# meudnaes/VoronoiRT

Hardware: AMD Instinct MI355X
Metric: formal-solve cell-updates/sec (higher is better)
Workload: dtype f64

## Files before the change

include/voronoirt.h:

```cpp
#ifndef VORONOIRT_H
#define VORONOIRT_H

#include <stdint.h>

#ifdef __cplusplus
extern "C" {
#endif

#define VRT_OK 0
#define VRT_EINVAL (-1)
#define VRT_EGRID (-2)
#define VRT_ENODEVICE (-3)
#define VRT_ENOMEM (-4)
#define VRT_EIO (-5)

typedef struct vrt_grid vrt_grid;
typedef struct vrt_plan vrt_plan;

#define VRT_ALPHA_SITE 0
#define VRT_ALPHA_SITE_LAM 1
#define VRT_ALPHA_ANGLE_SITE_LAM 2
#define VRT_ALPHA_ANGLE_NATIVE 3
#define VRT_ALPHA_SITE_LAM_NATIVE 4

// ... 25 lines not shown
                       int n_sweeps, vrt_plan **out);
void vrt_plan_destroy(vrt_plan *p);
int64_t vrt_plan_num_levels(const vrt_plan *p);
int64_t vrt_plan_num_nodes(const vrt_plan *p);
int vrt_plan_get_upwind(const vrt_plan *p, int64_t angle, int64_t *up, double *dots, double *w,
                        double *r);

int vrt_plan_execute(vrt_plan *p, int64_t nlam, int64_t ld, const double *S, const double *alpha,
                     int alpha_mode, const double *I0_up, const double *I0_down,
                     const double *weights, double *J, double *I_out);
int vrt_plan_execute_dev(vrt_plan *p, int64_t nlam, int64_t ld, const double *dS,
                         const double *dalpha, int alpha_mode, const double *dI0_up,
                         const double *dI0_down, const double *weights_host, double *dJ,
                         double *dI_out, void *stream);
int vrt_grid_get_storage_order(const vrt_grid *g, int dir, int64_t *out);
int64_t vrt_plan_native_alpha_count(const vrt_plan *p, int64_t nlam);
int vrt_plan_native_pair_block(const vrt_plan *p);
int vrt_plan_native_pair_block_f32(const vrt_plan *p);
int vrt_plan_alpha_to_native_dev(vrt_plan *p, int64_t nlam, int64_t ld, const double *dalpha,
                                 double *dalpha_native, void *stream);
int vrt_plan_alpha_to_native_dev_f32(vrt_plan *p, int64_t nlam, int64_t ld, const float *dalpha,
                                     float *dalpha_native, void *stream);

int64_t vrt_plan_native_plane_count(const vrt_plan *p, int64_t nlam);
int vrt_plan_to_native_dev(vrt_plan *p, int64_t nlam, int64_t ld, const double *d_in, double *d_up, double *d_down,
                           void *stream);
int vrt_plan_from_native_dev(vrt_plan *p, int dir, int64_t nlam, int64_t ld, const double *d_native, double *d_out,
                             void *stream);
int vrt_plan_j_from_native_dev(vrt_plan *p, int64_t nlam, int64_t ld, const double *dJ_up, const double *dJ_down,
                               double *dJ, void *stream);
int vrt_plan_execute_native_dev(vrt_plan *p, int64_t nlam, const double *dS_up, const double *dS_down,
                                const double *dalpha, int alpha_mode, const double *dI0_up, const double *dI0_down,
                                const double *weights_host, double *dJ_up, double *dJ_down, void *stream);
int vrt_plan_to_native_dev_f32(vrt_plan *p, int64_t nlam, int64_t ld, const float *d_in, float *d_up, float *d_down,
                               void *stream);
int vrt_plan_from_native_dev_f32(vrt_plan *p, int dir, int64_t nlam, int64_t ld, const float *d_native, float *d_out,
                                 void *stream);
int vrt_plan_j_from_native_dev_f32(vrt_plan *p, int64_t nlam, int64_t ld, const float *dJ_up, const float *dJ_down,
                                   float *dJ, void *stream);
int vrt_plan_execute_native_dev_f32(vrt_plan *p, int64_t nlam, const float *dS_up, const float *dS_down,
                                    const float *dalpha, int alpha_mode, const float *dI0_up, const float *dI0_down,
                                    const double *weights_host, float *dJ_up, float *dJ_down, void *stream);

int vrt_lambda_update_native_dev(vrt_grid *g, int64_t nlam, const double *dJ_up, const double *dJ_down,
                                 const double *dB_up, const double *deps, double *dS_up, double *dS_down,
                                 double *max_rel_change, void *stream);
int vrt_rates_populations_native_dev(vrt_grid *g, int64_t nlam, const double *lambda, const int64_t blocks[6],
                                     const double *dJ_up, const double *dJ_down, const double *planck2,
                                     double lambda0, double c0, const double *d_doppler_width, const double *d_gamma,
                                     double sigma_bb_const, const double *sigma_bf1, const double *sigma_bf2,
                                     const double *d_temperature, const double *d_lte_populations, double hc_over_kB,
                                     double pref_ij, double pref_ji, const double *d_C, const double *d_atom_density,
                                     double *d_R, double *d_populations, void *stream);

int vrt_plan_execute_dev_f32(vrt_plan *p, int64_t nlam, int64_t ld, const float *dS,
                             const float *dalpha, int alpha_mode, const float *dI0_up,
                             const float *dI0_down, const double *weights_host, float *dJ,
                             float *dI_out, void *stream);
int vrt_plan_last_sweep_timing(const vrt_plan *p, double *ms, int64_t *launches);
int vrt_plan_check(vrt_plan *p);
int vrt_plan_last_path(const vrt_plan *p);
int vrt_plan_set_option(vrt_plan *p, const char *name, const char *value);
int vrt_grid_set_option(vrt_grid *g, const char *name, const char *value);

typedef struct vrt_schedule vrt_schedule;
int vrt_schedule_build(const vrt_grid *g, int dir, const int64_t *up, int n_sweeps, vrt_schedule **out);
int64_t vrt_schedule_num_nodes(const vrt_schedule *s);
int64_t vrt_schedule_num_levels(const vrt_schedule *s);
int vrt_schedule_get(const vrt_schedule *s, int64_t *site, int32_t *zflags, int64_t *level_off);
void vrt_schedule_destroy(vrt_schedule *s);
int vrt_layer_schedule(const vrt_grid *g, int dir, const int64_t *up, int n_sweeps, uint32_t *vis,
                       int32_t *nlev, int64_t *n_visits);
int vrt_layer_sorted_slots(const vrt_grid *g, int dir, const uint32_t *vis, int64_t *store, int64_t *self);

typedef struct vrt_patch_schedule vrt_patch_schedule;
int vrt_patch_schedule_build(const vrt_grid *g, int dir, const int64_t *up, int n_sweeps, int own_target,
                             int entry_cap, vrt_patch_schedule **out, int64_t counts[6]);
int vrt_patch_schedule_get(const vrt_patch_schedule *s, int32_t *layer_patch_off, int32_t *patch_own_lo,
                           int32_t *patch_own_cnt, int32_t *patch_nlev, int64_t *patch_ent_off,
                           int32_t *entry_pos, uint32_t *entry_vis, uint32_t *entry_loc);
int vrt_patch_schedule_get_deps(const vrt_patch_schedule *s, int64_t *dep_off, int32_t *dep_list);
int vrt_patch_schedule_get_layers(const vrt_patch_schedule *s, uint32_t *vis, int32_t *nlev, int64_t *n_visits);
void vrt_patch_schedule_destroy(vrt_patch_schedule *s);

int vrt_delaunay_up(vrt_grid *g, const double k[3], const double *S, const double *I0,
                    int64_t nI0, const double *alpha, int n_sweeps, double *I_out);
int vrt_delaunay_down(vrt_grid *g, const double k[3], const double *S, const double *I0,
                      int64_t nI0, const double *alpha, int n_sweeps, double *I_out);

#define VRT_METRIC_EUCLIDEAN   0
#define VRT_METRIC_PERIODIC_XY 1
#define VRT_RASTER_NEAREST     1
#define VRT_RASTER_INV_DIST2   2
int vrt_grid_nearest(vrt_grid *g, int64_t nq, const double *q_zxy, int metric, int k, int64_t *idx, double *dist);
int vrt_grid_to_raster_dev(vrt_grid *g, int64_t nz, int64_t nx, int64_t ny, const double *z, const double *x,
                           const double *y, int metric, int mode, int64_t nf, int64_t ld, const double *d_fields,
                           double *d_raster, void *stream);
int vrt_raster_to_grid_dev(vrt_grid *g, int64_t nz, int64_t nx, int64_t ny, const double *z, const double *x,
                           const double *y, int64_t nf, const double *d_raster, int64_t ld, double *d_fields,
                           void *stream);
int vrt_grid_to_raster(vrt_grid *g, int64_t nz, int64_t nx, int64_t ny, const double *z, const double *x,
                       const double *y, int metric, int mode, int64_t nf, int64_t ld, const double *fields,
                       double *raster);
int vrt_raster_to_grid(vrt_grid *g, int64_t nz, int64_t nx, int64_t ny, const double *z, const double *x,
                       const double *y, int64_t nf, const double *raster, int64_t ld, double *fields);
int vrt_grid_raster_stats(const vrt_grid *g, double *nearest_ms, double *gather_ms, int64_t *queries,
                          int64_t *walk_steps, int64_t *fallbacks);

int vrt_sample_sites(int device, int64_t nz, int64_t nx, int64_t ny, const double *z, const double *x, const double *y,
                     const double *quantity, int64_t n_sites, uint64_t seed, int64_t batch, int64_t max_proposals,
                     double *pos_zxy, int64_t *proposals_used);
int vrt_sample_sites_dev(int device, int64_t nz, int64_t nx, int64_t ny, const double *z, const double *x,
                         const double *y, const double *d_quantity, int64_t n_sites, uint64_t seed, int64_t batch,
                         int64_t max_proposals, double *d_pos_zxy, int64_t *proposals_used, void *stream);

int vrt_lambda_update_dev(vrt_grid *g, int64_t nlam, int64_t ld, const double *dJ, const double *dB,
                          const double *deps, const double *dS_old, double *dS_new,
                          double *max_rel_change, void *stream);

int vrt_line_opacity_dev(vrt_plan *p, int64_t nlam, const double *lambda, double lambda0, double c0,
                         const double *d_velocity, const double *d_doppler_width, const double *d_gamma,
                         const double *d_line_strength, const double *d_alpha_cont, double *d_alpha_native,
                         void *stream);
int vrt_line_opacity_dev_f32(vrt_plan *p, int64_t nlam, const double *lambda, double lambda0, double c0,
                             const double *d_velocity, const double *d_doppler_width, const double *d_gamma,
                             const double *d_line_strength, const double *d_alpha_cont, float *d_alpha_native,
                             void *stream);

int vrt_plan_execute_line(vrt_plan *p, int64_t nlam, int64_t ld, const double *lambda, double lambda0, double c0,
                          const double *velocity, const double *doppler_width, const double *gamma,
                          const double *line_strength, const double *alpha_cont, const double *S, const double *I0_up,
                          const double *I0_down, const double *weights, double *J);

int vrt_line_terms_dev(vrt_grid *g, const double *d_gamma_static, const double *d_gamma_unsold,
                       const double *d_populations, double strength_const, double Bij, double Bji, double *d_gamma,
                       double *d_line_strength, void *stream);

typedef struct vrt_lambda vrt_lambda;
typedef struct vrt_line_case {
    int64_t nlam;
    const double *lambda;
    int64_t blocks[6];
    double lambda0, c0;
    const double *velocity;
    const double *doppler_width;
    const double *gamma_static;
    const double *gamma_unsold;
    const double *alpha_cont;
    const double *eps;
    const double *temperature;
    const double *atom_density;
    const double *B0;
    const double *lte_populations;
    const double *C;
    const double *planck2;
    const double *sigma_bf1, *sigma_bf2;
    double strength_const, Bij, Bji;
    double sigma_bb_const, hc_over_kB, pref_ij, pref_ji;
} vrt_line_case;
int vrt_lambda_create(vrt_plan *p, const vrt_line_case *lc, const double *weights, vrt_lambda **out);
int vrt_lambda_iterate(vrt_lambda *s, double *max_rel_change);
int vrt_lambda_get(vrt_lambda *s, double *J, double *S, double *populations, double *R, double *gamma);
void vrt_lambda_destroy(vrt_lambda *s);

typedef struct vrt_multi vrt_multi;
int vrt_multi_create(int n_devices, const int *devices, int64_t n, const double *pos_zxy, const int64_t *nbr, int64_t D1,
// ... 134 lines not shown
```

voronoirt_amd/_lib.py:

```python
from __future__ import annotations

import ctypes
import os

HERE = os.path.dirname(os.path.abspath(__file__))
LIB_PATH = os.path.join(HERE, "libvrt_hip.so")
if os.environ.get("VRT_LIB_PATH"):
    LIB_PATH = os.environ["VRT_LIB_PATH"]

c_i64 = ctypes.c_int64
c_dbl = ctypes.c_double
p_i64 = ctypes.POINTER(ctypes.c_int64)
p_i32 = ctypes.POINTER(ctypes.c_int32)
p_dbl = ctypes.POINTER(ctypes.c_double)
p_int = ctypes.POINTER(ctypes.c_int)
vp = ctypes.c_void_p

VRT_OK, VRT_EINVAL, VRT_EGRID, VRT_ENODEVICE, VRT_ENOMEM, VRT_EIO = 0, -1, -2, -3, -4, -5
ALPHA_SITE, ALPHA_SITE_LAM, ALPHA_ANGLE_SITE_LAM, ALPHA_ANGLE_NATIVE, ALPHA_SITE_LAM_NATIVE = 0, 1, 2, 3, 4
METRIC_EUCLIDEAN, METRIC_PERIODIC_XY = 0, 1
RASTER_NEAREST, RASTER_INV_DIST2 = 1, 2

class LineCaseStruct(ctypes.Structure):
    _fields_ = [("nlam", c_i64), ("lambda_", p_dbl), ("blocks", c_i64 * 6), ("lambda0", c_dbl), ("c0", c_dbl),
# ... 24 lines not shown
    "vrt_grid_num_layer_offsets": (c_i64, [vp, ctypes.c_int]),
    "vrt_grid_get_layers": (ctypes.c_int, [vp, ctypes.c_int, p_i64]),
    "vrt_grid_get_perm": (ctypes.c_int, [vp, ctypes.c_int, p_i64]),
    "vrt_grid_get_delaunay_lines": (ctypes.c_int, [vp, p_dbl]),
    "vrt_direction": (None, [c_dbl, c_dbl, p_dbl]),
    "vrt_plan_create": (ctypes.c_int, [vp, c_i64, p_dbl, ctypes.c_int, ctypes.POINTER(vp)]),
    "vrt_plan_create_ex": (ctypes.c_int, [vp, c_i64, p_dbl, p_int, ctypes.c_int,
                                          ctypes.POINTER(vp)]),
    "vrt_plan_destroy": (None, [vp]),
    "vrt_plan_num_levels": (c_i64, [vp]),
    "vrt_plan_num_nodes": (c_i64, [vp]),
    "vrt_plan_get_upwind": (ctypes.c_int, [vp, c_i64, p_i64, p_dbl, p_dbl, p_dbl]),
    "vrt_plan_execute": (ctypes.c_int, [vp, c_i64, c_i64, p_dbl, p_dbl, ctypes.c_int, p_dbl, p_dbl,
                                        p_dbl, p_dbl, p_dbl]),
    "vrt_plan_execute_dev": (ctypes.c_int, [vp, c_i64, c_i64, vp, vp, ctypes.c_int, vp, vp, p_dbl,
                                            vp, vp, vp]),
    "vrt_plan_execute_dev_f32": (ctypes.c_int, [vp, c_i64, c_i64, vp, vp, ctypes.c_int, vp, vp, p_dbl,
                                                vp, vp, vp]),
    "vrt_plan_native_plane_count": (c_i64, [vp, c_i64]),
    "vrt_plan_to_native_dev": (ctypes.c_int, [vp, c_i64, c_i64, vp, vp, vp, vp]),
    "vrt_plan_from_native_dev": (ctypes.c_int, [vp, ctypes.c_int, c_i64, c_i64, vp, vp, vp]),
    "vrt_plan_j_from_native_dev": (ctypes.c_int, [vp, c_i64, c_i64, vp, vp, vp, vp]),
    "vrt_plan_execute_native_dev": (ctypes.c_int, [vp, c_i64, vp, vp, vp, ctypes.c_int, vp, vp, p_dbl, vp, vp, vp]),
    "vrt_plan_to_native_dev_f32": (ctypes.c_int, [vp, c_i64, c_i64, vp, vp, vp, vp]),
    "vrt_plan_from_native_dev_f32": (ctypes.c_int, [vp, ctypes.c_int, c_i64, c_i64, vp, vp, vp]),
    "vrt_plan_j_from_native_dev_f32": (ctypes.c_int, [vp, c_i64, c_i64, vp, vp, vp, vp]),
    "vrt_plan_execute_native_dev_f32": (ctypes.c_int, [vp, c_i64, vp, vp, vp, ctypes.c_int, vp, vp, p_dbl, vp, vp, vp]),
    "vrt_plan_check": (ctypes.c_int, [vp]),
    "vrt_lambda_update_native_dev": (ctypes.c_int, [vp, c_i64, vp, vp, vp, vp, vp, vp, p_dbl, vp]),
    "vrt_rates_populations_native_dev": (ctypes.c_int, [vp, c_i64, p_dbl, p_i64, vp, vp, p_dbl, c_dbl, c_dbl, vp, vp,
                                                        c_dbl, p_dbl, p_dbl, vp, vp, c_dbl, c_dbl, c_dbl, vp, vp, vp,
                                                        vp, vp]),
    "vrt_grid_get_storage_order": (ctypes.c_int, [vp, ctypes.c_int, p_i64]),
    "vrt_plan_native_alpha_count": (c_i64, [vp, c_i64]),
    "vrt_plan_native_pair_block": (ctypes.c_int, [vp]),
    "vrt_plan_native_pair_block_f32": (ctypes.c_int, [vp]),
    "vrt_plan_alpha_to_native_dev": (ctypes.c_int, [vp, c_i64, c_i64, vp, vp, vp]),
    "vrt_line_opacity_dev": (ctypes.c_int, [vp, c_i64, p_dbl, c_dbl, c_dbl, vp, vp, vp, vp, vp, vp, vp]),
    "vrt_line_opacity_dev_f32": (ctypes.c_int, [vp, c_i64, p_dbl, c_dbl, c_dbl, vp, vp, vp, vp, vp, vp, vp]),
    "vrt_plan_alpha_to_native_dev_f32": (ctypes.c_int, [vp, c_i64, c_i64, vp, vp, vp]),
    "vrt_plan_execute_line": (ctypes.c_int, [vp, c_i64, c_i64, p_dbl, c_dbl, c_dbl, p_dbl, p_dbl, p_dbl, p_dbl, p_dbl,
                                             p_dbl, p_dbl, p_dbl, p_dbl, p_dbl]),
    "vrt_line_terms_dev": (ctypes.c_int, [vp, vp, vp, vp, c_dbl, c_dbl, c_dbl, vp, vp, vp]),
    "vrt_lambda_create": (ctypes.c_int, [vp, ctypes.POINTER(LineCaseStruct), p_dbl, ctypes.POINTER(vp)]),
    "vrt_lambda_iterate": (ctypes.c_int, [vp, p_dbl]),
    "vrt_lambda_get": (ctypes.c_int, [vp, p_dbl, p_dbl, p_dbl, p_dbl, p_dbl]),
    "vrt_lambda_destroy": (None, [vp]),
    "vrt_multi_create": (ctypes.c_int, [ctypes.c_int, p_int, c_i64, p_dbl, p_i64, c_i64, p_dbl, c_i64, p_dbl, p_int,
                                        ctypes.c_int, ctypes.POINTER(vp)]),
    "vrt_multi_execute": (ctypes.c_int, [vp, c_i64, c_i64, p_dbl, p_dbl, ctypes.c_int, p_dbl, p_dbl, p_dbl, p_dbl]),
    "vrt_multi_set_shard": (ctypes.c_int, [vp, ctypes.c_char_p]),
    "vrt_multi_last_shard": (ctypes.c_int, [vp]),
    "vrt_multi_uses_rccl": (ctypes.c_int, [vp]),
    "vrt_multi_destroy": (None, [vp]),
    "vrt_multi_execute_line": (ctypes.c_int, [vp, c_i64, c_i64, p_dbl, c_dbl, c_dbl, p_dbl, p_dbl, p_dbl, p_dbl, p_dbl, p_dbl,
                                              p_dbl, p_dbl, p_dbl, p_dbl]),
    "vrt_multi_lambda_create": (ctypes.c_int, [vp, ctypes.POINTER(LineCaseStruct), p_dbl, ctypes.POINTER(vp)]),
    "vrt_multi_lambda_iterate": (ctypes.c_int, [vp, p_dbl]),
    "vrt_multi_lambda_get": (ctypes.c_int, [vp, p_dbl, p_dbl, p_dbl, p_dbl, p_dbl]),
    "vrt_multi_lambda_destroy": (None, [vp]),
    "vrt_rates_populations_dev": (ctypes.c_int, [vp, c_i64, c_i64, p_dbl, p_i64, vp, p_dbl, c_dbl, c_dbl, vp, vp,
                                                 c_dbl, p_dbl, p_dbl, vp, vp, c_dbl, c_dbl, c_dbl, vp, vp, vp,
                                                 vp, vp]),
    "vrt_plan_last_sweep_timing": (ctypes.c_int, [vp, p_dbl, p_i64]),
    "vrt_plan_last_path": (ctypes.c_int, [vp]),
    "vrt_plan_set_option": (ctypes.c_int, [vp, ctypes.c_char_p, ctypes.c_char_p]),
    "vrt_grid_set_option": (ctypes.c_int, [vp, ctypes.c_char_p, ctypes.c_char_p]),
    "vrt_schedule_build": (ctypes.c_int, [vp, ctypes.c_int, p_i64, ctypes.c_int,
                                          ctypes.POINTER(vp)]),
    "vrt_schedule_num_nodes": (c_i64, [vp]),
    "vrt_schedule_num_levels": (c_i64, [vp]),
    "vrt_schedule_get": (ctypes.c_int, [vp, p_i64, p_i32, p_i64]),
    "vrt_schedule_destroy": (None, [vp]),
    "vrt_layer_schedule": (ctypes.c_int, [vp, ctypes.c_int, p_i64, ctypes.c_int,
                                          ctypes.POINTER(ctypes.c_uint32), p_i32, p_i64]),
    "vrt_layer_sorted_slots": (ctypes.c_int, [vp, ctypes.c_int, ctypes.POINTER(ctypes.c_uint32), p_i64, p_i64]),
    "vrt_patch_schedule_build": (ctypes.c_int, [vp, ctypes.c_int, p_i64, ctypes.c_int, ctypes.c_int, ctypes.c_int,
                                                ctypes.POINTER(vp), p_i64]),
    "vrt_patch_schedule_get": (ctypes.c_int, [vp, p_i32, p_i32, p_i32, p_i32, p_i64, p_i32,
                                              ctypes.POINTER(ctypes.c_uint32), ctypes.POINTER(ctypes.c_uint32)]),
    "vrt_patch_schedule_get_deps": (ctypes.c_int, [vp, p_i64, p_i32]),
    "vrt_patch_schedule_get_layers": (ctypes.c_int, [vp, ctypes.POINTER(ctypes.c_uint32), p_i32, p_i64]),
    "vrt_patch_schedule_destroy": (None, [vp]),
    "vrt_lambda_update_dev": (ctypes.c_int, [vp, c_i64, c_i64, vp, vp, vp, vp, vp, p_dbl, vp]),
    "vrt_short_characteristics": (ctypes.c_int, [c_i64, c_i64, c_i64, p_dbl, p_dbl, p_dbl, c_i64, p_dbl,
                                                 p_int, p_dbl, c_i64, p_dbl, c_i64, p_dbl, ctypes.c_int,
                                                 ctypes.c_int, p_dbl]),
    "vrt_regular_create": (ctypes.c_int, [c_i64, c_i64, c_i64, p_dbl, p_dbl, p_dbl, ctypes.c_int,
                                          ctypes.POINTER(vp)]),
    "vrt_regular_destroy": (None, [vp]),
    "vrt_regular_execute_dev": (ctypes.c_int, [vp, c_i64, p_dbl, p_int, vp, c_i64, vp, c_i64, c_i64, vp,
                                               ctypes.c_int, vp, vp]),
    "vrt_regular_last_solve_ms": (ctypes.c_int, [vp, p_dbl]),
    "vrt_regular_execute_line": (ctypes.c_int, [vp, c_i64, p_dbl, p_int, p_dbl, c_i64, p_dbl, c_dbl, c_dbl, p_dbl, p_dbl,
                                                p_dbl, p_dbl, p_dbl, p_dbl, p_dbl, ctypes.c_int, p_dbl]),
    "vrt_regular_lambda_create": (ctypes.c_int, [vp, c_i64, p_dbl, p_int, p_dbl, ctypes.POINTER(LineCaseStruct), ctypes.c_int,
                                                 ctypes.POINTER(vp)]),
    "vrt_regular_lambda_iterate": (ctypes.c_int, [vp, p_dbl]),
    "vrt_regular_lambda_get": (ctypes.c_int, [vp, p_dbl, p_dbl, p_dbl, p_dbl, p_dbl]),
    "vrt_regular_lambda_destroy": (None, [vp]),
    "vrt_synth_opacity_dev": (ctypes.c_int, [c_i64, c_i64, c_i64, p_dbl, c_i64, p_dbl, p_dbl, c_dbl, c_dbl, c_dbl, c_dbl,
                                             c_dbl, c_dbl, c_dbl, c_dbl, vp, vp, vp, vp, vp, vp, vp, vp, vp, vp]),
    "vrt_synth_opacity": (ctypes.c_int, [ctypes.c_int, c_i64, c_i64, c_i64, p_dbl, c_i64, p_dbl, p_dbl, c_dbl, c_dbl,
                                         c_dbl, c_dbl, c_dbl, c_dbl, c_dbl, c_dbl, p_dbl, p_dbl, p_dbl, p_dbl, p_dbl,
                                         p_dbl, p_dbl, p_dbl, p_dbl]),
    "vrt_regular_emergent_dev": (ctypes.c_int, [vp, p_dbl, c_i64, vp, vp, ctypes.c_int, vp, vp]),
    "vrt_top_intensity": (ctypes.c_int, [c_i64, c_i64, c_i64, p_dbl, p_dbl, p_dbl, p_dbl, c_i64, p_dbl, p_dbl,
                                         ctypes.c_int, ctypes.c_int, p_dbl]),
    "vrt_tau_unity_dev": (ctypes.c_int, [c_i64, c_i64, c_i64, p_dbl, p_dbl, p_dbl, p_dbl, c_i64, vp, vp, vp]),
    "vrt_tau_unity": (ctypes.c_int, [c_i64, c_i64, c_i64, p_dbl, p_dbl, p_dbl, p_dbl, c_i64, p_dbl, ctypes.c_int,
                                     p_dbl]),
    "vrt_grid_nearest": (ctypes.c_int, [vp, c_i64, p_dbl, ctypes.c_int, ctypes.c_int, p_i64, p_dbl]),
    "vrt_grid_to_raster_dev": (ctypes.c_int, [vp, c_i64, c_i64, c_i64, p_dbl, p_dbl, p_dbl, ctypes.c_int, ctypes.c_int,
                                              c_i64, c_i64, vp, vp, vp]),
    "vrt_raster_to_grid_dev": (ctypes.c_int, [vp, c_i64, c_i64, c_i64, p_dbl, p_dbl, p_dbl, c_i64, vp, c_i64, vp, vp]),
    "vrt_grid_to_raster": (ctypes.c_int, [vp, c_i64, c_i64, c_i64, p_dbl, p_dbl, p_dbl, ctypes.c_int, ctypes.c_int,
                                          c_i64, c_i64, p_dbl, p_dbl]),
    "vrt_raster_to_grid": (ctypes.c_int, [vp, c_i64, c_i64, c_i64, p_dbl, p_dbl, p_dbl, c_i64, p_dbl, c_i64, p_dbl]),
    "vrt_grid_raster_stats": (ctypes.c_int, [vp, p_dbl, p_dbl, p_i64, p_i64, p_i64]),
    "vrt_sample_sites": (ctypes.c_int, [ctypes.c_int, c_i64, c_i64, c_i64, p_dbl, p_dbl, p_dbl, p_dbl, c_i64,
                                        ctypes.c_uint64, c_i64, c_i64, p_dbl, p_i64]),
    "vrt_sample_sites_dev": (ctypes.c_int, [ctypes.c_int, c_i64, c_i64, c_i64, p_dbl, p_dbl, p_dbl, vp, c_i64,
                                            ctypes.c_uint64, c_i64, c_i64, vp, p_i64, vp]),
    "vrt_ng_accelerate_dev": (ctypes.c_int, [c_i64, vp, vp, vp, vp, vp, p_dbl, p_dbl, p_int, vp]),
    "vrt_ng_sums_dev": (ctypes.c_int, [c_i64, vp, vp, vp, vp, p_dbl, vp]),
    "vrt_ng_coefficients": (ctypes.c_int, [p_dbl, p_dbl]),
    "vrt_ng_apply_dev": (ctypes.c_int, [c_i64, c_dbl, c_dbl, vp, vp, vp, vp, p_int, vp]),
    "vrt_lambda_set_acceleration": (ctypes.c_int, [vp, ctypes.c_int, ctypes.c_int, ctypes.c_int]),
    "vrt_regular_lambda_set_acceleration": (ctypes.c_int, [vp, ctypes.c_int, ctypes.c_int, ctypes.c_int]),
    "vrt_lambda_last_acceleration": (ctypes.c_int, [vp, p_int, p_dbl, p_dbl]),
    "vrt_regular_lambda_last_acceleration": (ctypes.c_int, [vp, p_int, p_dbl, p_dbl]),
    "vrt_continuum_case_check": (ctypes.c_int, [ctypes.POINTER(ContinuumCaseStruct), c_i64]),
    "vrt_continuum_create": (ctypes.c_int, [vp, ctypes.POINTER(ContinuumCaseStruct), p_dbl, ctypes.POINTER(vp)]),
    "vrt_continuum_iterate": (ctypes.c_int, [vp, p_dbl]),
    "vrt_continuum_get": (ctypes.c_int, [vp, p_dbl, p_dbl]),
    "vrt_continuum_set_source": (ctypes.c_int, [vp, p_dbl]),
    "vrt_continuum_set_acceleration": (ctypes.c_int, [vp, ctypes.c_int, ctypes.c_int, ctypes.c_int]),
    "vrt_continuum_last_acceleration": (ctypes.c_int, [vp, p_int, p_dbl, p_dbl]),
    "vrt_continuum_destroy": (None, [vp]),
    "vrt_regular_continuum_create": (ctypes.c_int, [vp, c_i64, p_dbl, p_int, p_dbl, ctypes.POINTER(ContinuumCaseStruct),
                                                    ctypes.c_int, ctypes.POINTER(vp)]),
    "vrt_regular_continuum_iterate": (ctypes.c_int, [vp, p_dbl]),
    "vrt_regular_continuum_get": (ctypes.c_int, [vp, p_dbl, p_dbl]),
    "vrt_regular_continuum_set_source": (ctypes.c_int, [vp, p_dbl]),
    "vrt_regular_continuum_set_acceleration": (ctypes.c_int, [vp, ctypes.c_int, ctypes.c_int, ctypes.c_int]),
    "vrt_regular_continuum_last_acceleration": (ctypes.c_int, [vp, p_int, p_dbl, p_dbl]),
    "vrt_regular_continuum_destroy": (None, [vp]),
    "vrt_continuum_update_dev": (ctypes.c_int, [vp, c_i64, c_i64, vp, vp, vp, c_dbl, vp, vp, p_dbl, p_i64, vp]),
    "vrt_plan_lambda_diagonal_dev": (ctypes.c_int, [vp, c_i64, c_i64, vp, p_dbl, vp, vp]),
    "vrt_plan_lambda_diagonal": (ctypes.c_int, [vp, c_i64, c_i64, p_dbl, p_dbl, p_dbl]),
    "vrt_continuum_ali_update_dev": (ctypes.c_int, [vp, c_i64, c_i64, vp, vp, vp, vp, c_dbl, vp, vp, p_dbl, p_i64, vp]),
    "vrt_continuum_set_operator": (ctypes.c_int, [vp, ctypes.c_int]),
    "vrt_continuum_get_operator": (ctypes.c_int, [vp, p_int, p_dbl]),
    "vrt_delaunay_up": (ctypes.c_int, [vp, p_dbl, p_dbl, p_dbl, c_i64, p_dbl, ctypes.c_int, p_dbl]),
    "vrt_delaunay_down": (ctypes.c_int, [vp, p_dbl, p_dbl, p_dbl, c_i64, p_dbl, ctypes.c_int, p_dbl]),
}


class VrtError(RuntimeError):
    def __init__(self, code: int, message: str):
        super().__init__(f"libvrt_hip error {code}: {message}")
        self.code = code
        self.message = message


_lib = None
# ... 33 lines not shown
```

voronoirt_amd/csrc/vrt_api.cpp:

```cpp
#include <algorithm>
#include <atomic>
#include <chrono>
#include <cmath>
#include <cstdio>
#include <cstdlib>
#include <cstring>
#include <memory>
#include <new>
#include <thread>

#include "vrt_internal.h"

namespace vrt {

static thread_local std::string g_err;

void set_error(const std::string &msg) { g_err = msg; }
int fail(int code, const std::string &msg)
{
    g_err = msg;
    return code;
}

void tuning_from_env(Tuning &t)
{
    static const char *names[] = {"VRT_PATH", "VRT_STEP_K", "VRT_STEP_SINGLE", "VRT_STEP_PAIRS", "VRT_STEP_XCD",
                                  "VRT_STEP_STREAMS", "VRT_STEP_LEVEL_MAP", "VRT_STEP_GROUP_DIR", "VRT_TILE_WIDE",
                                  "VRT_TILE_PRE", "VRT_PATCH_K", "VRT_PATCH_NT", "VRT_PATCH_OWN",
                                  "VRT_PATCH_Q", "VRT_PATCH_TARGET", "VRT_PATCH_SPLIT", "VRT_PAIR_BLOCK", "VRT_PATCH_QUAD", "VRT_PATCH_LEAN", "VRT_PATCH_CHAIN", "VRT_CHAIN_PAIRS", "VRT_CHAIN_SPIN", "VRT_CHAIN_DATAFLAG", "VRT_CHAIN_STATIC", "VRT_LAMBDA_NATIVE", "VRT_DEBUG_FLAGS", "VRT_DEBUG_SKIP_LEVELS",
                                  "VRT_TILE_DEBUG"};
    for (const char *nm : names) {
        const char *e = std::getenv(nm);
        if (e && *e && tuning_set(t, nm, e, false) != VRT_OK) {
            static std::mutex mu;
            static std::vector<std::string> said;
            std::lock_guard<std::mutex> lock(mu);
            if (std::find(said.begin(), said.end(), std::string(nm)) == said.end()) {
                said.push_back(nm);
                std::fprintf(stderr, "[libvrt_hip] ignoring %s=%s: %s\n", nm, e, g_err.c_str());
            }
        }
    }
}

int tuning_set(Tuning &t, const char *name, const char *value, bool created)
{
    if (!name || !value) return fail(VRT_EINVAL, "NULL option name or value");
    const std::string nm(name), v(value);
    if (nm == "VRT_PATH") {
        static const char *paths[] = {"auto", "levels", "tiles", "steps", "patches"};
        for (int i = 0; i < 5; i++)
            if (v == paths[i]) { t.path = i; return VRT_OK; }
        if (v.empty()) { t.path = 0; return VRT_OK; }
        return fail(VRT_EINVAL, "VRT_PATH must be auto, levels, tiles, steps or patches");
    }
    char *end = nullptr;
    const long x = std::strtol(value, &end, 10);
    if (end == value || *end != 0) return fail(VRT_EINVAL, "option " + nm + " needs an integer value");
    struct { const char *name; int *field; long lo, hi; bool creation_only; } tab[] = {
        {"VRT_STEP_K", &t.step_K, 0, 18, false}, {"VRT_STEP_SINGLE", &t.step_single, 0, 1, false},
        {"VRT_STEP_PAIRS", &t.step_pairs, 0, 64, false}, {"VRT_STEP_XCD", &t.step_xcd, 0, 2, false},
        {"VRT_STEP_STREAMS", &t.step_streams, 1, 4, false}, {"VRT_STEP_LEVEL_MAP", &t.step_level_map, 0, 1, false},
        {"VRT_STEP_GROUP_DIR", &t.step_group_dir, 0, 1, false}, {"VRT_TILE_WIDE", &t.tile_wide, 0, 1, false},
        {"VRT_TILE_PRE", &t.tile_pre, 0, 1, false},
        {"VRT_PATCH_K", &t.patch_K, 1, 8, true}, {"VRT_PATCH_NT", &t.patch_NT, 64, 1024, true},
        {"VRT_PATCH_OWN", &t.patch_own, 0, 65535, true}, {"VRT_PATCH_Q", &t.patch_Q, 1, 4, false},
        {"VRT_PATCH_TARGET", &t.patch_target, 0, 1 << 20, false}, {"VRT_PATCH_SPLIT", &t.patch_split, 0, 4096, false}, {"VRT_PAIR_BLOCK", &t.pair_block, 1, 16, true},
        {"VRT_PATCH_QUAD", &t.patch_quad, 0, 1, true}, {"VRT_PATCH_LEAN", &t.patch_lean, 0, 1, false},
        {"VRT_PATCH_CHAIN", &t.patch_chain, 0, 2, false}, {"VRT_CHAIN_PAIRS", &t.chain_pairs, 1, 256, false},
        {"VRT_CHAIN_SPIN", &t.chain_spin, 1, 1 << 20, false}, {"VRT_CHAIN_DATAFLAG", &t.chain_dataflag, 0, 2, false},
        {"VRT_LAMBDA_NATIVE", &t.lambda_native, 0, 1, false}, {"VRT_CHAIN_STATIC", &t.chain_static, 0, 1, false}, {"VRT_DEBUG_FLAGS", &t.debug_flags, 0, 1 << 20, false},
        {"VRT_DEBUG_SKIP_LEVELS", &t.debug_skip_levels, 0, 1, false}, {"VRT_TILE_DEBUG", &t.tile_debug, 0, 1, false},
    };
    for (auto &o : tab)
        if (nm == o.name) {
            if (o.creation_only && created)
                return fail(VRT_EINVAL, "option " + nm + " shapes what plan creation builds: preset it in the environment");
            if (x < o.lo || x > o.hi) return fail(VRT_EINVAL, "option " + nm + " out of range");
            *o.field = (int)x;
            return VRT_OK;
        }
    return fail(VRT_EINVAL, "unknown option " + nm);
}

int use_device(int device)
{
    if (device < 0)
        return fail(VRT_ENODEVICE, "host-only grid handle (device < 0): no compute without a HIP device");
    int cnt = 0;
    hipError_t e = hipGetDeviceCount(&cnt);
    if (e != hipSuccess || cnt <= 0)
        return fail(VRT_ENODEVICE, "no HIP device available (libvrt_hip has no CPU fallback)");
    if (device < 0 || device >= cnt) return fail(VRT_EINVAL, "device ordinal out of range");
    VRT_HIP_TRY(hipSetDevice(device));
    (void)hipGetLastError();
    return VRT_OK;
}

int use_current_device()
{
    int cnt = 0;
    if (hipGetDeviceCount(&cnt) != hipSuccess || cnt <= 0)
        return fail(VRT_ENODEVICE, "no HIP device available (libvrt_hip has no CPU fallback)");
    (void)hipGetLastError();
    return VRT_OK;
}

static void free_grid(vrt_grid *g)
{
    if (!g) return;
    for (PlanCacheEntry *c : g->cache) {
        vrt_plan_destroy(c->plan);
        delete c;
    }
    g->cache.clear();
    raster_locator_free(g);
    dev_free(g->d_pos);
    dev_free(g->d_rowptr);
    dev_free(g->d_col);
    dev_free(g->d_lz);
    dev_free(g->d_lx);
    dev_free(g->d_ly);
    dev_free(g->up.d_order);
    dev_free(g->down.d_order);
    dev_free(g->up.d_rank);
    dev_free(g->down.d_rank);
    dev_free(g->up.d_lay);
    dev_free(g->down.d_lay);
    dev_free(g->d_scalars);
    dev_free(g->d_small);
    if (g->small_ev) (void)hipEventDestroy(g->small_ev);
    if (g->small_copy_ev) (void)hipEventDestroy(g->small_copy_ev);
    if (g->h_small) (void)hipHostFree(g->h_small);
    dev_free(g->up.d_store);
    dev_free(g->down.d_store);
    dev_free(g->up.d_srank);
    dev_free(g->down.d_srank);
    if (g->stream) (void)hipStreamDestroy(g->stream);
    delete g;
}

static int upload_grid(vrt_grid *g)
{
    const int64_t n = g->n;
    const size_t nnz = g->col.size();
    int rc;
    if ((rc = dev_alloc(&g->d_pos, (size_t)3 * n))) return rc;
    if ((rc = dev_alloc(&g->d_rowptr, (size_t)n + 1))) return rc;
    if ((rc = dev_alloc(&g->d_col, nnz))) return rc;
    if ((rc = dev_alloc(&g->d_lz, nnz))) return rc;
// ... 9 lines not shown
        std::vector<int32_t> order((size_t)n);
        for (int64_t i = 0; i < n; i++) order[(size_t)i] = (int32_t)(dir.perm[(size_t)i] - 1);
        if ((rc = dev_alloc(&dir.d_order, (size_t)n))) return rc;
        VRT_HIP_TRY(hipMemcpy(dir.d_order, order.data(), sizeof(int32_t) * n, hipMemcpyHostToDevice));
        std::vector<int32_t> rank((size_t)n);
        for (int64_t i = 0; i < n; i++) rank[(size_t)order[(size_t)i]] = (int32_t)i;
        if ((rc = dev_alloc(&dir.d_rank, (size_t)n))) return rc;
        VRT_HIP_TRY(hipMemcpy(dir.d_rank, rank.data(), sizeof(int32_t) * n, hipMemcpyHostToDevice));
        std::vector<int32_t> srank((size_t)n);
        for (int64_t i = 0; i < n; i++) srank[(size_t)dir.store[(size_t)i]] = (int32_t)i;
        if ((rc = dev_alloc(&dir.d_store, (size_t)n))) return rc;
        if ((rc = dev_alloc(&dir.d_srank, (size_t)n))) return rc;
        VRT_HIP_TRY(hipMemcpy(dir.d_store, dir.store.data(), sizeof(int32_t) * n, hipMemcpyHostToDevice));
        VRT_HIP_TRY(hipMemcpy(dir.d_srank, srank.data(), sizeof(int32_t) * n, hipMemcpyHostToDevice));
        std::vector<int32_t> lay(dir.reduced.size());
        for (size_t j = 0; j < lay.size(); j++) lay[j] = (int32_t)(dir.reduced[j] - 1);
        if ((rc = dev_alloc(&dir.d_lay, lay.size()))) return rc;
        VRT_HIP_TRY(hipMemcpy(dir.d_lay, lay.data(), sizeof(int32_t) * lay.size(), hipMemcpyHostToDevice));
    }
    if ((rc = launch_delaunay_lines(g))) return rc;
    VRT_HIP_TRY(hipStreamSynchronize(g->stream));
    return VRT_OK;
}

static int grid_create_impl(int64_t n, const double *pos, const int64_t *nbr, int64_t D1,
                            const double bounds[6], int device, vrt_grid **out)
{
    if (!out) return fail(VRT_EINVAL, "out is NULL");
    *out = nullptr;
    if (!pos || !nbr || !bounds) return fail(VRT_EINVAL, "NULL argument");
    int rc = device >= 0 ? use_device(device) : VRT_OK;
    if (rc) return rc;
    vrt_grid *g = new (std::nothrow) vrt_grid();
    if (!g) return fail(VRT_ENOMEM, "out of host memory");
    g->device = device;
    rc = build_grid_host(g, n, pos, nbr, D1, bounds);
    if (!rc && device >= 0) rc = upload_grid(g);
    if (rc) {
        free_grid(g);
        return rc;
    }
    *out = g;
    return VRT_OK;
}

static const Direction &direction_of(const vrt_grid *g, int dir) { return dir > 0 ? g->up : g->down; }

static void free_plan(vrt_plan *p)
{
    if (!p) return;
    dev_free(p->d_up1);
    dev_free(p->d_up2);
    dev_free(p->d_d1);
    dev_free(p->d_d2);
    dev_free(p->d_w1);
    dev_free(p->d_w2);
    dev_free(p->d_r1);
    dev_free(p->d_r2);
    dev_free(p->d_node_site);
    dev_free(p->d_node_meta);
    dev_free(p->d_node_u1);
    dev_free(p->d_node_u2);
    dev_free(p->d_angles_up);
    dev_free(p->d_angles_down);
    dev_free(p->d_I);
    for (int i = 0; i < 6; i++) dev_free(p->d_stage[i]);
    dev_free(p->t_u1); dev_free(p->t_u2);
    dev_free(p->t_w1); dev_free(p->t_w2); dev_free(p->t_r1); dev_free(p->t_r2);
    dev_free(p->t_vis);
    dev_free(p->t_loc);
    dev_free(p->t_self);
    dev_free(p->t_vis_s);
    dev_free(p->t_loc_s);
    dev_free(p->t_gpos);
    dev_free(p->t_rank_s);
    dev_free(p->t_loc_ss);
    dev_free(p->t_code_ss);
    dev_free(p->d_nlev); dev_free(p->d_angle_dir); dev_free(p->d_task_map);
    for (int d = 0; d < 2; d++) { dev_free(p->ws_S[d]); dev_free(p->ws_A[d]); dev_free(p->ws_J[d]); }
    dev_free(p->ws_AA);
    for (int i = 0; i < 2; i++) dev_free(p->ws_cg[i]);
    dev_free(p->d_step_angles);
    dev_free(p->d_level_map);
    dev_free(p->d_patch_work);
    dev_free(p->d_chain_items); dev_free(p->d_chain_deps); dev_free(p->d_chain_progress); dev_free(p->d_chain_ctrl);
    for (auto &cs : p->chain_cache) { dev_free(cs.items); dev_free(cs.deps); }
    p->chain_cache.clear();
    if (p->h_chain_status) { (void)hipHostFree(p->h_chain_status); p->h_chain_status = nullptr; }
    if (p->d_chain_dev) { (void)hipFree(p->d_chain_dev); p->d_chain_dev = nullptr; }
    if (p->h_chain_dev_pinned) { (void)hipHostFree(p->h_chain_dev_pinned); p->h_chain_dev_pinned = nullptr; }
    if (p->chain_dev_ev) (void)hipEventDestroy(p->chain_dev_ev);
    dev_free(p->e_pos); dev_free(p->e_u1); dev_free(p->e_u2); dev_free(p->e_vis); dev_free(p->e_loc);
    dev_free(p->e_w1); dev_free(p->e_w2); dev_free(p->e_r1); dev_free(p->e_r2);
    if (p->step_fork) (void)hipEventDestroy(p->step_fork);
    for (int i = 0; i < 4; i++) {
        if (p->step_join[i]) (void)hipEventDestroy(p->step_join[i]);
        if (p->step_stream[i]) (void)hipStreamDestroy(p->step_stream[i]);
    }
    for (CopyLane &l : p->copy_lanes) {
        for (int b = 0; b < 2; b++) {
            if (l.pin[b]) (void)hipHostFree(l.pin[b]);
            if (l.ev[b]) (void)hipEventDestroy(l.ev[b]);
        }
        if (l.st) (void)hipStreamDestroy(l.st);
    }
    if (p->copy_done) (void)hipEventDestroy(p->copy_done);
    if (p->ev0) (void)hipEventDestroy(p->ev0);
    if (p->ev1) (void)hipEventDestroy(p->ev1);
    delete p;
}

static int ensure_level_schedule(vrt_plan *p)
{
    if (p->level_ready) return VRT_OK;
    vrt_grid *g = p->g;
    const int64_t n = g->n;
    const int A = p->A;
    const int n_sweeps = p->n_sweeps;
    std::vector<AngleSchedule> sched((size_t)A);
    {
        unsigned hw = std::thread::hardware_concurrency();
        int nthr = (int)std::min<unsigned>(hw ? hw : 4, 16);
        nthr = std::max(1, std::min(nthr, std::max(A, 1)));
        if (!run_workers(nthr, [&](int t) {
                for (int a = t; a < A; a += nthr) {
                    const bool up = p->dir_of_active[(size_t)a] > 0;
                    build_angle_schedule(up ? g->up : g->down, up, n, n_sweeps,
                                         p->h_up1.data() + (size_t)a * n, p->h_up2.data() + (size_t)a * n,
                                         sched[(size_t)a]);
                }
            }))
            return fail(VRT_ENOMEM, "out of host memory while building the level schedule");
    }
    int64_t max_levels = 0, total = 0;
    for (int a = 0; a < A; a++) {
        if (sched[(size_t)a].bad_site >= 0) return fail(VRT_EGRID, "site without an upwind neighbour");
        max_levels = std::max<int64_t>(max_levels, (int64_t)sched[(size_t)a].level_off.size() - 1);
        total += (int64_t)sched[(size_t)a].site.size();
    }
    std::vector<int32_t> srank_up((size_t)n);
    for (int64_t i = 0; i < n; i++) srank_up[(size_t)g->up.store[(size_t)i]] = (int32_t)i;
    std::vector<uint32_t> node_site((size_t)total), node_meta((size_t)total);
    std::vector<int32_t> node_u1((size_t)total), node_u2((size_t)total);
    p->level_off.assign((size_t)max_levels + 1, 0);
    int64_t at = 0;
    for (int64_t t = 0; t < max_levels; t++) {
        p->level_off[(size_t)t] = at;
        for (int a = 0; a < A; a++) {
            const AngleSchedule &s = sched[(size_t)a];
            if (t + 1 >= (int64_t)s.level_off.size()) continue;
            const int64_t x0 = s.level_off[(size_t)t], x1 = s.level_off[(size_t)t + 1];
            std::vector<std::pair<int32_t, int64_t>> keyed((size_t)(x1 - x0));
            for (int64_t x = x0; x < x1; x++)
                keyed[(size_t)(x - x0)] = {srank_up[(size_t)s.site[(size_t)x]], x};
            std::sort(keyed.begin(), keyed.end());
            for (const auto &kv : keyed) {
                const int64_t x = kv.second;
                node_site[(size_t)at] = s.site[(size_t)x];
                node_meta[(size_t)at] = (uint32_t)a | ((uint32_t)s.zflags[(size_t)x] << 8);
                node_u1[(size_t)at] = p->h_up1[(size_t)a * (size_t)n + s.site[(size_t)x]];
                node_u2[(size_t)at] = p->h_up2[(size_t)a * (size_t)n + s.site[(size_t)x]];
                at++;
            }
        }
    }
    p->level_off[(size_t)max_levels] = at;
    p->n_nodes = total;
// ... 773 lines not shown
        return VRT_OK;
    });
}

struct vrt_patch_schedule {
    vrt::PatchSchedule s;
    vrt::LayerSchedule layers;
};

int vrt_patch_schedule_build(const vrt_grid *g, int dir, const int64_t *up, int n_sweeps, int own_target,
                             int entry_cap, vrt_patch_schedule **out, int64_t counts[6])
{
    if (!g || !up || !out || !counts) return fail(VRT_EINVAL, "NULL argument");
    if (n_sweeps < 1 || own_target < 1 || entry_cap < 1 || entry_cap > 65535)
        return fail(VRT_EINVAL, "need n_sweeps >= 1, own_target >= 1 and 1 <= entry_cap <= 65535");
    *out = nullptr;
    return guarded([&] {
        const int64_t n = g->n;
        std::vector<int32_t> u1((size_t)n), u2((size_t)n);
        for (int64_t i = 0; i < n; i++) {
            const int64_t a = up[2 * i], b = up[2 * i + 1];
            if (a > n || b > n) return fail(VRT_EINVAL, "upwind id out of range");
            u1[(size_t)i] = a >= 1 ? (int32_t)(a - 1) : kNoUpwind;
            u2[(size_t)i] = b >= 1 ? (int32_t)(b - 1) : kNoUpwind;
        }
        std::unique_ptr<vrt_patch_schedule> ps(new vrt_patch_schedule());
        int threads = (int)std::max(1u, std::min(8u, std::thread::hardware_concurrency()));
        if (const char *e = std::getenv("VRT_HOST_THREADS")) threads = std::max(1, std::min(64, std::atoi(e)));
        build_patch_schedule(direction_of(g, dir), dir > 0, n, n_sweeps, u1.data(), u2.data(), own_target, entry_cap,
                             ps->s, threads, &ps->layers);
        if (ps->s.bad_site >= 0)
            return fail(VRT_EGRID, "site " + std::to_string(ps->s.bad_site + 1) + " has no upwind neighbour");
        if (!ps->s.ok) return fail(VRT_EINVAL, "schedule does not fit the packed patch encoding");
        counts[0] = (int64_t)ps->s.patch_own_lo.size();
        counts[1] = (int64_t)ps->s.entry_pos.size();
        counts[2] = ps->s.n_visits;
        counts[3] = ps->s.n_live;
        counts[4] = ps->s.max_entries;
        counts[5] = (int64_t)ps->s.layer_patch_off.size();
        *out = ps.release();
        return VRT_OK;
    });
}

int vrt_patch_schedule_get(const vrt_patch_schedule *s, int32_t *layer_patch_off, int32_t *patch_own_lo,
                           int32_t *patch_own_cnt, int32_t *patch_nlev, int64_t *patch_ent_off,
                           int32_t *entry_pos, uint32_t *entry_vis, uint32_t *entry_loc)
{
    if (!s) return fail(VRT_EINVAL, "NULL schedule");
    const PatchSchedule &p = s->s;
    if (layer_patch_off) std::copy(p.layer_patch_off.begin(), p.layer_patch_off.end(), layer_patch_off);
    if (patch_own_lo) std::copy(p.patch_own_lo.begin(), p.patch_own_lo.end(), patch_own_lo);
    if (patch_own_cnt) std::copy(p.patch_own_cnt.begin(), p.patch_own_cnt.end(), patch_own_cnt);
    if (patch_nlev) std::copy(p.patch_nlev.begin(), p.patch_nlev.end(), patch_nlev);
    if (patch_ent_off) std::copy(p.patch_ent_off.begin(), p.patch_ent_off.end(), patch_ent_off);
    if (entry_pos) std::copy(p.entry_pos.begin(), p.entry_pos.end(), entry_pos);
    if (entry_vis) std::copy(p.entry_vis.begin(), p.entry_vis.end(), entry_vis);
    if (entry_loc) std::copy(p.entry_loc.begin(), p.entry_loc.end(), entry_loc);
    return VRT_OK;
}

int vrt_patch_schedule_get_deps(const vrt_patch_schedule *s, int64_t *dep_off, int32_t *dep_list)
{
    if (!s) return fail(VRT_EINVAL, "NULL schedule");
    const PatchSchedule &p = s->s;
    if (dep_off) std::copy(p.dep_off.begin(), p.dep_off.end(), dep_off);
    if (dep_list) std::copy(p.dep_list.begin(), p.dep_list.end(), dep_list);
    return VRT_OK;
}

int vrt_patch_schedule_get_layers(const vrt_patch_schedule *s, uint32_t *vis, int32_t *nlev, int64_t *n_visits)
{
    if (!s) return fail(VRT_EINVAL, "NULL schedule");
    const LayerSchedule &ls = s->layers;
    if (!ls.ok) return fail(VRT_EINVAL, "schedule does not fit the packed layer-tile encoding");
    if (vis) std::copy(ls.vis.begin(), ls.vis.end(), vis);
    if (nlev) std::copy(ls.nlev.begin(), ls.nlev.end(), nlev);
    if (n_visits) *n_visits = ls.n_visits;
    return VRT_OK;
}

void vrt_patch_schedule_destroy(vrt_patch_schedule *s) { delete s; }

int vrt_grid_get_storage_order(const vrt_grid *g, int dir, int64_t *out)
{
    if (!g || !out) return fail(VRT_EINVAL, "NULL argument");
    const Direction &d = direction_of(g, dir);
    for (int64_t i = 0; i < g->n; i++) out[i] = (int64_t)d.store[(size_t)i] + 1;
    return VRT_OK;
}

int vrt_plan_native_pair_block(const vrt_plan *p) { return p ? 1 << native_lg(p, false) : 0; }
int vrt_plan_native_pair_block_f32(const vrt_plan *p) { return p ? 1 << native_lg(p, true) : 0; }

int64_t vrt_plan_native_alpha_count(const vrt_plan *p, int64_t nlam)
{
    if (!p || nlam < 1) return 0;
    return (int64_t)p->A * ((nlam + 1) / 2 * 2) * p->g->n;
}

static int alpha_native_call(vrt_plan *p, int64_t nlam, int64_t ld, const void *dalpha, void *dalpha_native, void *stream,
                             bool f32)
{
    return guarded([&] {
        if (!p || !dalpha || !dalpha_native) return fail(VRT_EINVAL, "NULL argument");
        if (nlam < 1 || ld < nlam) return fail(VRT_EINVAL, "need nlam >= 1 and ld >= nlam");
        if (p->A != (int)p->n_angles_user)
            return fail(VRT_EINVAL, "per-angle alpha needs every angle active (no θ = 90 direction)");
        std::lock_guard<std::mutex> lock(p->mu);
        int rc = use_device(p->g->device);
        return rc ? rc : alpha_to_native(p, nlam, ld, dalpha, dalpha_native, (hipStream_t)stream, f32);
    });
}

int vrt_plan_alpha_to_native_dev(vrt_plan *p, int64_t nlam, int64_t ld, const double *dalpha,
                                 double *dalpha_native, void *stream)
{
    return alpha_native_call(p, nlam, ld, dalpha, dalpha_native, stream, false);
}

int vrt_plan_alpha_to_native_dev_f32(vrt_plan *p, int64_t nlam, int64_t ld, const float *dalpha, float *dalpha_native,
                                     void *stream)
{
    return alpha_native_call(p, nlam, ld, dalpha, dalpha_native, stream, true);
}

int vrt_plan_execute_dev(vrt_plan *p, int64_t nlam, int64_t ld, const double *dS,
                         const double *dalpha, int alpha_mode, const double *dI0_up,
                         const double *dI0_down, const double *weights_host, double *dJ,
                         double *dI_out, void *stream)
{
    return execute_call(p, caller_args(nlam, ld, dS, dalpha, alpha_mode, dI0_up, dI0_down, weights_host, dJ, dI_out,
                                       (hipStream_t)stream, false));
}

int64_t vrt_plan_native_plane_count(const vrt_plan *p, int64_t nlam)
{
    if (!p || nlam < 1) return 0;
    return ((nlam + 1) / 2 * 2) * p->g->n;
}

int vrt_plan_to_native_dev(vrt_plan *p, int64_t nlam, int64_t ld, const double *d_in, double *d_up, double *d_down, void *stream)
{
    return native_call(p, nlam, ld, d_in && (d_up || d_down), false,
                       [&] { return planes_to_native(p, nlam, ld, d_in, d_up, d_down, (hipStream_t)stream); });
}

int vrt_plan_from_native_dev(vrt_plan *p, int dir, int64_t nlam, int64_t ld, const double *d_native, double *d_out, void *stream)
{
    return native_call(p, nlam, ld, d_native && d_out, false,
                       [&] { return plane_from_native(p, dir > 0 ? 0 : 1, nlam, ld, d_native, d_out, (hipStream_t)stream); });
}

int vrt_plan_j_from_native_dev(vrt_plan *p, int64_t nlam, int64_t ld, const double *dJ_up, const double *dJ_down, double *dJ,
                               void *stream)
{
    return native_call(p, nlam, ld, dJ && (dJ_up || dJ_down), false,
                       [&] { return J_from_native(p, nlam, ld, dJ_up, dJ_down, dJ, (hipStream_t)stream); });
}

int vrt_plan_execute_native_dev(vrt_plan *p, int64_t nlam, const double *dS_up, const double *dS_down, const double *dalpha,
                                int alpha_mode, const double *dI0_up, const double *dI0_down, const double *weights_host,
                                double *dJ_up, double *dJ_down, void *stream)
{
    return execute_call(p, native_args(nlam, dS_up, dS_down, dalpha, alpha_mode, dI0_up, dI0_down, weights_host, dJ_up,
                                       dJ_down, (hipStream_t)stream, false));
// ... 384 lines not shown
```

voronoirt_amd/csrc/vrt_internal.h:

```cpp
#pragma once

#include <hip/hip_runtime.h>

#include <algorithm>
#include <cstdint>
#include <mutex>
#include <new>
#include <string>
#include <thread>
#include <vector>

#include "voronoirt.h"

namespace vrt {

void set_error(const std::string &msg);
int fail(int code, const std::string &msg);

#define VRT_HIP_TRY(expr)                                                                  \
    do {                                                                                   \
        hipError_t _e = (expr);                                                            \
        if (_e != hipSuccess)                                                              \
            return ::vrt::fail(VRT_ENODEVICE, std::string(#expr) + ": " + hipGetErrorString(_e)); \
    } while (0)
// ... 65 lines not shown
    ~DevBuf() { dev_free(p); }
    int alloc(size_t count) { dev_free(p); return dev_alloc(&p, count); }
    operator T *() const { return p; }
};

template <typename Body>
inline bool run_workers(int count, Body body)
{
    std::vector<char> threw((size_t)std::max(count, 1), 0);
    auto guarded = [&](int t) {
        try {
            body(t);
        } catch (...) {
            threw[(size_t)t] = 1;
        }
    };
    std::vector<std::thread> pool;
    try {
        pool.reserve((size_t)std::max(count, 1));
    } catch (...) {
    }
    for (int t = 0; t < count; t++) {
        try {
            pool.emplace_back(guarded, t);
        } catch (...) {
            guarded(t);
        }
    }
    for (auto &th : pool) th.join();
    for (int t = 0; t < count; t++)
        if (threw[(size_t)t]) return false;
    return true;
}

constexpr int kMaxAngles = 64;
constexpr int64_t kMaxGuess = 70;
constexpr int32_t kNoUpwind = -1;

struct Direction {
    std::vector<int32_t> layer_of;
    std::vector<int64_t> perm;
    std::vector<int64_t> reduced;
    int64_t n1 = 0;
    int32_t *d_order = nullptr;
    int32_t *d_rank = nullptr;
    int32_t *d_lay = nullptr;
    std::vector<int32_t> store;
    int32_t *d_store = nullptr;
    int32_t *d_srank = nullptr;
};

struct PlanCacheEntry;

struct CopyLane {
    hipStream_t st = nullptr;
    void *pin[2] = {nullptr, nullptr};
    hipEvent_t ev[2] = {nullptr, nullptr};
};
constexpr size_t kCopyChunk = (size_t)8 << 20;

struct Tuning {
    int path = 0;
    int step_K = 0;
    int step_single = 0;
    int step_pairs = 0;
    int step_xcd = 2;
    int step_streams = 2;
    int step_level_map = 1;
    int step_group_dir = 1;
    int tile_wide = 1;
    int tile_pre = 1;
    int patch_K = 1, patch_NT = 512;
    int patch_own = 0;
    int patch_Q = 1;
    int pair_block = 1;
    int patch_quad = 1;
    int patch_lean = 1;
    int patch_chain = 2;
    int chain_pairs = 9;
    int chain_spin = 2048;
    int chain_dataflag = 2;
    int patch_split = 0;
    int patch_target = 0;
    int chain_static = 1;
    int lambda_native = 1;
    int debug_flags = 0, debug_skip_levels = 0, tile_debug = 0;
};
void tuning_from_env(Tuning &t);
int tuning_set(Tuning &t, const char *name, const char *value, bool created);

struct ExecArgs {
    int64_t nlam = 0, ld = 0;
    const void *S = nullptr;
    const void *S_nat[2] = {nullptr, nullptr};
    const void *alpha = nullptr;
    int alpha_mode = 0;
    const void *I0[2] = {nullptr, nullptr};
    const double *weights = nullptr;
    void *J = nullptr;
    void *J_nat[2] = {nullptr, nullptr};
    void *I_out = nullptr;
    bool native = false;
    bool f32 = false;
    hipStream_t st = nullptr;
    bool wants_J() const { return native ? J_nat[0] != nullptr : J != nullptr; }
};
inline ExecArgs caller_args(int64_t nlam, int64_t ld, const void *S, const void *alpha, int alpha_mode, const void *I0_up,
                            const void *I0_down, const double *weights, void *J, void *I_out, hipStream_t st, bool f32)
{
    ExecArgs x;
    x.nlam = nlam; x.ld = ld;
    x.S = S;
    x.alpha = alpha; x.alpha_mode = alpha_mode;
    x.I0[0] = I0_up; x.I0[1] = I0_down;
    x.weights = weights;
    x.J = J; x.I_out = I_out;
    x.f32 = f32;
    x.st = st;
    return x;
}
inline ExecArgs native_args(int64_t nlam, const void *S_up, const void *S_down, const void *alpha, int alpha_mode,
                            const void *I0_up, const void *I0_down, const double *weights, void *J_up, void *J_down,
                            hipStream_t st, bool f32)
{
    ExecArgs x = caller_args(nlam, (nlam + 1) / 2 * 2, nullptr, alpha, alpha_mode, I0_up, I0_down, weights, nullptr, nullptr,
                             st, f32);
    x.S_nat[0] = S_up; x.S_nat[1] = S_down;
    x.J_nat[0] = J_up; x.J_nat[1] = J_down;
    x.native = true;
    return x;
}

}

namespace vrt {
struct RasterLocator;
void raster_locator_free(vrt_grid *g);
}

struct vrt_grid {
    int device = 0;
    int64_t n = 0;
    int64_t D = 0;
    double bounds[6] = {0, 0, 0, 0, 0, 0};
    std::vector<double> pos;
    std::vector<int32_t> rowptr;
    std::vector<int32_t> col;
    vrt::Direction up, down;
    double *d_pos = nullptr;
    int32_t *d_rowptr = nullptr;
    int32_t *d_col = nullptr;
    double *d_lz = nullptr, *d_lx = nullptr, *d_ly = nullptr;
    hipStream_t stream = nullptr;
    unsigned long long *d_scalars = nullptr;
    double *d_small = nullptr;
    size_t small_cap = 0;
    double *h_small = nullptr;
    hipEvent_t small_ev = nullptr;
    bool small_ev_valid = false;
    hipEvent_t small_copy_ev = nullptr;
    bool small_copy_valid = false;
    std::vector<std::pair<std::string, std::string>> options;
    std::mutex mu;
    std::vector<vrt::PlanCacheEntry *> cache;
    vrt::RasterLocator *locator = nullptr;
    int64_t nearest_cells = 0;
};

struct vrt_plan {
    vrt_grid *g = nullptr;
    vrt::Tuning tune;
    int n_sweeps = 3;
    int64_t n_angles_user = 0;
    int A = 0;
    std::vector<int> user_of_active;
    std::vector<int> dir_of_active;
    std::vector<double> k;
    int32_t *d_up1 = nullptr, *d_up2 = nullptr;
    double *d_d1 = nullptr, *d_d2 = nullptr;
    double *d_w1 = nullptr, *d_w2 = nullptr;
    double *d_r1 = nullptr, *d_r2 = nullptr;
    uint32_t *d_node_site = nullptr;
    uint32_t *d_node_meta = nullptr;
    int32_t *d_node_u1 = nullptr, *d_node_u2 = nullptr;
    std::vector<int64_t> level_off;
    bool level_ready = false;
    std::vector<int32_t> h_up1, h_up2;
    int64_t n_nodes = 0;
    int32_t *d_angles_up = nullptr, *d_angles_down = nullptr;
    int n_up = 0, n_down = 0;
    std::vector<int64_t> skip_site;
    double *d_I = nullptr;
    size_t I_cap = 0;
    int64_t I_ld = 0;
    double *d_stage[6] = {nullptr, nullptr, nullptr, nullptr, nullptr, nullptr};
    size_t stage_cap[6] = {0, 0, 0, 0, 0, 0};
    bool tile_ok = false;
    bool step_tables_ready = false;
    int tile_K = 8;
    int tile_max_layers = 0;
    int64_t tile_max_layer_size = 0;
    int64_t tile_visits = 0;
    int32_t *t_u1 = nullptr, *t_u2 = nullptr;
    double *t_w1 = nullptr, *t_w2 = nullptr, *t_r1 = nullptr, *t_r2 = nullptr;
    uint32_t *t_vis = nullptr, *t_loc = nullptr;
    int32_t *t_self = nullptr;
    uint32_t *t_vis_s = nullptr, *t_loc_s = nullptr;
    uint32_t *t_gpos = nullptr;
    int32_t *t_rank_s = nullptr;
    uint32_t *t_loc_ss = nullptr;
    uint32_t *t_code_ss = nullptr;
    int32_t *d_nlev = nullptr, *d_angle_dir = nullptr;
    std::vector<int64_t> angle_visits;
    std::vector<int32_t> h_task_map;
    int32_t *d_task_map = nullptr;
    size_t task_map_cap = 0;
    int task_map_nlam = -1;
    double *ws_S[2] = {nullptr, nullptr}, *ws_A[2] = {nullptr, nullptr}, *ws_J[2] = {nullptr, nullptr};
    size_t ws_S_cap[2] = {0, 0}, ws_A_cap[2] = {0, 0}, ws_J_cap[2] = {0, 0};
    double *ws_AA = nullptr;
    size_t ws_AA_cap = 0;
    double *ws_cg[2] = {nullptr, nullptr};
    size_t ws_cg_cap[2] = {0, 0};
    int step_groups = 0;
    int32_t *d_step_angles = nullptr;
    std::vector<int> step_group_off;
    std::vector<double> angle_mean_levels;
    int32_t *d_level_map = nullptr;
    std::vector<int> level_map_off;
    int level_map_units = 0, level_map_groups = 0;
    std::vector<int32_t> h_step_angles;
    bool patch_ok = false;
    int lg_pair_block = 0;
    int patch_cap = 0, patch_K = 0, patch_NT = 0;
    int64_t n_patches = 0, n_patch_entries = 0, n_patch_visits = 0;
    std::vector<int32_t> h_patch_first;
    std::vector<int4> h_patch_rec;
    int32_t *e_pos = nullptr, *e_u1 = nullptr, *e_u2 = nullptr;
    uint32_t *e_vis = nullptr, *e_loc = nullptr;
    double *e_w1 = nullptr, *e_w2 = nullptr, *e_r1 = nullptr, *e_r2 = nullptr;
    std::vector<int2> h_patch_rec2;
    std::vector<int64_t> h_patch_dep_off;
    std::vector<int32_t> h_patch_deps;
    int4 *d_chain_items = nullptr;
    int32_t *d_chain_deps = nullptr;
    uint32_t *d_chain_progress = nullptr, *d_chain_ctrl = nullptr;
    uint32_t *h_chain_status = nullptr, *d_chain_status = nullptr;
    void *d_chain_dev = nullptr, *h_chain_dev_pinned = nullptr;
    std::vector<char> h_chain_dev;
    hipEvent_t chain_dev_ev = nullptr;
    bool chain_dev_ev_valid = false;
    size_t chain_progress_cap = 0;
    bool chain_progress_fresh = false;
    int chain_q_off[9] = {0, 0, 0, 0, 0, 0, 0, 0, 0};
    int chain_npair = -1, chain_lgB = -1, chain_nsplit = -1, chain_reduce = -1;
    int64_t chain_items = 0;
    struct ChainSet {
        int npair = -1, lgB = -1, nsplit = -1, reduce = -1;
        int4 *items = nullptr;
        int32_t *deps = nullptr;
        int q_off[9] = {0, 0, 0, 0, 0, 0, 0, 0, 0};
        int64_t n_items = 0;
    };
    std::vector<ChainSet> chain_cache;
    uint32_t chain_epoch = 0;
    int4 *d_patch_work = nullptr;
    std::vector<int64_t> patch_work_off;
    int patch_work_groups = 0;
    hipStream_t step_stream[4] = {nullptr, nullptr, nullptr, nullptr};
    hipEvent_t step_fork = nullptr, step_join[4] = {nullptr, nullptr, nullptr, nullptr};
    int last_path = 0;
    hipEvent_t ev0 = nullptr, ev1 = nullptr;
    bool ev_valid = false;
    std::vector<vrt::CopyLane> copy_lanes;
    hipEvent_t copy_done = nullptr;
    int64_t last_launches = 0;
    std::mutex mu;
};

namespace vrt {

struct PlanCacheEntry {
    double k[3];
    int n_sweeps;
    vrt_plan *plan;
    int users;
};

int parse_neighbour_file(const char *path, int64_t n, std::vector<int64_t> &matrix, int64_t &D1);
int build_grid_host(vrt_grid *g, int64_t n, const double *pos, const int64_t *nbr, int64_t D1,
                    const double bounds[6]);

int tessellate_host(int64_t n, const double *pos, const double bounds[6], int64_t D1, int64_t *nbr_out,
                    int64_t *max_count, int nthreads);

struct AngleSchedule {
    std::vector<uint32_t> site;
    std::vector<uint8_t> zflags;
    std::vector<int64_t> level_off;
    int64_t bad_site = -1;
};
void build_angle_schedule(const Direction &dir, bool ascending, int64_t n, int n_sweeps,
                          const int32_t *up1, const int32_t *up2, AngleSchedule &out);
struct LayerSchedule {
    std::vector<uint32_t> vis;
    std::vector<int32_t> nlev;
    int64_t n_visits = 0;
    int64_t max_layer_size = 0;
    int64_t bad_site = -1;
    bool ok = false;
};
void build_layer_schedule(const Direction &dir, bool ascending, int64_t n, int n_sweeps,
                          const int32_t *up1, const int32_t *up2, LayerSchedule &out);
void build_sorted_slots(const Direction &dir, int64_t n, const std::vector<uint32_t> &vis_site,
                        std::vector<int32_t> &self);
struct PatchSchedule {
    std::vector<int32_t> layer_patch_off;
    std::vector<int32_t> patch_own_lo;
    std::vector<int32_t> patch_own_cnt;
    std::vector<int32_t> patch_nlev;
    std::vector<int64_t> patch_ent_off;
    std::vector<int32_t> entry_pos;
    std::vector<uint32_t> entry_vis;
    std::vector<uint32_t> entry_loc;
    std::vector<int64_t> dep_off;
    std::vector<int32_t> dep_list;
    int64_t n_visits = 0;
    int64_t n_live = 0;
    int64_t max_entries = 0;
    int64_t bad_site = -1;
    bool ok = false;
};
void build_patch_schedule(const Direction &dir, bool ascending, int64_t n, int n_sweeps, const int32_t *up1,
                          const int32_t *up2, int own_target, int entry_cap, PatchSchedule &out, int threads = 1,
                          LayerSchedule *layers = nullptr);

int launch_delaunay_lines(vrt_grid *g);
int launch_upwind_table(vrt_plan *p, int a);
struct SweepArgs {
    int64_t n, nlam, ldS, ldA, ldI;
    const void *S, *alpha;
    int alpha_mode;
    void *I;
    bool f32 = false;
};
int launch_boundary(vrt_plan *p, const SweepArgs &sa, const void *dI0_up, const void *dI0_down,
                    hipStream_t st);
int launch_sweep_levels(vrt_plan *p, const SweepArgs &sa, hipStream_t st, int64_t *launches);
int launch_reduce_J(vrt_plan *p, const SweepArgs &sa, const double *weights_active, void *dJ,
                    int64_t ldJ, hipStream_t st);
int launch_copy_I_out(vrt_plan *p, const SweepArgs &sa, void *dI_out, int64_t ldO, hipStream_t st);

constexpr size_t kUpdateWords = 3;
int launch_axpy(size_t count, const double *d_src, double *d_dst, hipStream_t st);
int launch_gather_rows(int64_t rows, int64_t nlam, int64_t ld, const int32_t *d_order, const double *d_src, double *d_dst,
                       hipStream_t st);
int launch_lambda_update(int64_t n, int64_t nlam, int64_t ld, const double *dJ, const double *dB,
                         const double *deps, const double *dS_old, double *dS_new,
                         unsigned long long *d_result, hipStream_t st);
int launch_lambda_update_native(vrt_grid *g, int64_t nlam, const double *dJ_up, const double *dJ_down, const double *dB_up,
                                const double *deps, double *dS_up, double *dS_down, unsigned long long *d_result, hipStream_t st);

int launch_line_opacity(vrt_plan *p, int64_t nlam, const double *d_lambda, double lambda0, double c0,
                        const double *d_velocity, const double *d_doppler, const double *d_gamma,
                        const double *d_strength, const double *d_alpha_cont, void *d_out, hipStream_t st,
                        bool f32_out = false);
int launch_line_terms(int64_t n, const double *d_gamma_static, const double *d_gamma_unsold, const double *d_pops,
                      double strength_const, double Bij, double Bji, double *d_gamma, double *d_strength, hipStream_t st);
int launch_rates_populations(vrt_grid *g, int64_t nlam, int64_t ld, const int64_t blocks[6],
                             const double *d_small, const double *dJ, double lambda0, double c0,
                             const double *d_doppler, const double *d_gamma, double sigma_bb_const,
                             const double *d_temperature, const double *d_lte, double hc_over_kB,
                             double pref_ij, double pref_ji, const double *d_C, const double *d_atom_density,
                             double *d_R, double *d_populations, hipStream_t st,
                             const double *dJ_up = nullptr, const double *dJ_down = nullptr);
int launch_rates_populations(int64_t n, int64_t nlam, int64_t ld, const int64_t blocks[6], const double *d_small,
                             const double *dJ, double lambda0, double c0, const double *d_doppler, const double *d_gamma,
                             double sigma_bb_const, const double *d_temperature, const double *d_lte, double hc_over_kB,
                             double pref_ij, double pref_ji, const double *d_C, const double *d_atom_density, double *d_R,
                             double *d_populations, hipStream_t st);

int launch_rates_partial(vrt_grid *g, int64_t nlam, int64_t l0, int64_t l1, int64_t ld, const int64_t blocks[6],
                         const double *d_small, const double *dJ, double lambda0, double c0, const double *d_doppler,
                         const double *d_gamma, double sigma_bb_const, const double *d_temperature, const double *d_lte,
                         double hc_over_kB, double pref_ij, double pref_ji, double *d_shares, hipStream_t st,
                         const double *dJ_up = nullptr, const double *dJ_down = nullptr);
int launch_populations_from_shares(vrt_grid *g, const double *d_shares, const double *d_C, const double *d_atom_density,
                                   double *d_R, double *d_populations, hipStream_t st);

int execute_locked(vrt_plan *p, const ExecArgs &x);

int ensure_step_tables(vrt_plan *p);
int launch_permute_table(vrt_plan *p, int a, const uint32_t *d_vis_site);
int launch_sorted_tables(vrt_plan *p, int a);
int launch_gpos(vrt_plan *p, int a);
inline int native_lg(const vrt_plan *p, bool f32)
{
    if (!p->patch_ok) return 0;
    return f32 && p->tune.patch_quad != 0 && p->patch_K == 1 ? std::max(p->lg_pair_block, 1) : p->lg_pair_block;
}
int alpha_to_native(vrt_plan *p, int64_t nlam, int64_t ld, const void *dalpha, void *out, hipStream_t st, bool f32);
int native_planes_ok(const vrt_plan *p, bool f32 = false);
int planes_to_native_f32(vrt_plan *p, int64_t nlam, int64_t ld, const float *din, float *out_up, float *out_down, hipStream_t st);
int plane_from_native_f32(vrt_plan *p, int dir_index, int64_t nlam, int64_t ld, const float *din, float *dout, hipStream_t st);
int J_from_native_f32(vrt_plan *p, int64_t nlam, int64_t ld, const float *dJ_up, const float *dJ_down, float *dJ, hipStream_t st);
int planes_to_native(vrt_plan *p, int64_t nlam, int64_t ld, const double *din, double *out_up, double *out_down, hipStream_t st);
int plane_from_native(vrt_plan *p, int dir_index, int64_t nlam, int64_t ld, const double *din, double *dout, hipStream_t st);
int J_from_native(vrt_plan *p, int64_t nlam, int64_t ld, const double *dJ_up, const double *dJ_down, double *dJ, hipStream_t st);
int execute_layers(vrt_plan *p, const ExecArgs &x, int path);
int64_t steps_max_layer(bool f32);

struct TileArgs;
struct PatchReduce;
bool patch_shape_exists(int K, int Q, int NT);
int launch_patch_entries(vrt_plan *p, int a, int64_t first, int64_t count);
int ensure_patch_work(vrt_plan *p, int G, const std::vector<int32_t> &group_angles, const std::vector<int> &group_off);
int launch_patch_layer(vrt_plan *p, const TileArgs &ta, int npair, int layer, int group, int Q, hipStream_t st,
                       bool f32, const PatchReduce *reduce);
bool patch_chain_possible(const vrt_plan *p, int npair, bool f32);
bool patch_chain_dataflag(const vrt_plan *p, int npair, bool f32);
int launch_patch_chain(vrt_plan *p, const TileArgs &ta, int npair, hipStream_t st, bool f32, const PatchReduce *reduce,
                       bool dataflag, bool ctrl_zeroed = false);
int chain_ctrl_words();
int patch_chain_check(vrt_plan *p);

struct NgRange {
    int64_t dense = 0, tail = 0, tstride = 1;
};
struct NgState {
    int order = 0, start = 0, period = 0;
    double *hist[3] = {nullptr, nullptr, nullptr};
    unsigned have = 0;
    double *d_ws = nullptr;
    int last_applied = 0;
    double last_sums[5] = {0, 0, 0, 0, 0}, last_coeffs[2] = {0, 0};
};
int ng_check_settings(int order, int start, int period);
int ng_configure(NgState &ng, int order, int start, int period, size_t alloc_count);
void ng_release(NgState &ng);
int ng_after_iterate(NgState &ng, int64_t iterate, double *&S, size_t alloc_count, const NgRange &rg, hipStream_t st);
int ng_report(const NgState &ng, int *applied, double sums[5], double coeffs[2]);
int launch_ng_mirror(vrt_grid *g, int64_t nlam, const double *dS_up, double *dS_down, hipStream_t st);

}
```

voronoirt_amd/csrc/vrt_layers.hip:

```cpp
#include <hip/hip_runtime.h>

#include <algorithm>
#include <cmath>
#include <cstdio>
#include <cstdlib>
#include <cstring>

#include "vrt_device.h"
#include "vrt_internal.h"

#include "vrt_layout_kernels.h"
#include "vrt_step_kernels.h"
#include "vrt_tile_kernels.h"

namespace vrt {

static int build_task_map(vrt_plan *p, int nlam, hipStream_t st)
{
    const int A = p->A;
    if (p->task_map_nlam == nlam && p->d_task_map) return VRT_OK;
    const int ntask = A * nlam;
    struct Group { int a, l0, l1; double cost; };
    std::vector<Group> groups;
    const int halves = nlam >= 2 ? 2 : 1;
// ... 86 lines not shown
int plane_from_native_f32(vrt_plan *p, int dir_index, int64_t nlam, int64_t ld, const float *din, float *dout, hipStream_t st)
{
    vrt_grid *g = p->g;
    const int64_t n = g->n;
    const dim3 tgrid((unsigned)((n + 63) / 64), (unsigned)((nlam + 63) / 64));
    const Direction &dir = dir_index == 0 ? g->up : g->down;
    hipLaunchKernelGGL(k_from_sweep_order<float>, tgrid, dim3(256), 0, st, n, (int)nlam, ld, 2 << native_lg(p, true), dir.d_store, din, dout);
    VRT_HIP_TRY(hipGetLastError());
    return VRT_OK;
}
int J_from_native_f32(vrt_plan *p, int64_t nlam, int64_t ld, const float *dJ_up, const float *dJ_down, float *dJ, hipStream_t st)
{
    vrt_grid *g = p->g;
    const int64_t n = g->n;
    const dim3 tgrid((unsigned)((n + 63) / 64), (unsigned)((nlam + 63) / 64));
    hipLaunchKernelGGL(k_combine_J<float>, tgrid, dim3(256), 0, st, n, (int)nlam, ld, 2 << native_lg(p, true), g->up.d_store, g->down.d_srank, dJ_up, dJ_down, dJ);
    VRT_HIP_TRY(hipGetLastError());
    return VRT_OK;
}

int planes_to_native(vrt_plan *p, int64_t nlam, int64_t ld, const double *din, double *out_up, double *out_down, hipStream_t st)
{
    vrt_grid *g = p->g;
    const int64_t n = g->n;
    const dim3 tgrid((unsigned)((n + 63) / 64), (unsigned)((nlam + 63) / 64));
    for (int d = 0; d < 2; d++) {
        double *out = d == 0 ? out_up : out_down;
        if (!out) continue;
        const Direction &dir = d == 0 ? g->up : g->down;
        hipLaunchKernelGGL(k_to_sweep_order<double>, tgrid, dim3(256), 0, st, n, (int)nlam, ld, 2, dir.d_store, din, out,
                           (const double *)nullptr, (double *)nullptr);
    }
    VRT_HIP_TRY(hipGetLastError());
    return VRT_OK;
}

int plane_from_native(vrt_plan *p, int dir_index, int64_t nlam, int64_t ld, const double *din, double *dout, hipStream_t st)
{
    vrt_grid *g = p->g;
    const int64_t n = g->n;
    const dim3 tgrid((unsigned)((n + 63) / 64), (unsigned)((nlam + 63) / 64));
    const Direction &dir = dir_index == 0 ? g->up : g->down;
    hipLaunchKernelGGL(k_from_sweep_order<double>, tgrid, dim3(256), 0, st, n, (int)nlam, ld, 2, dir.d_store, din, dout);
    VRT_HIP_TRY(hipGetLastError());
    return VRT_OK;
}

int J_from_native(vrt_plan *p, int64_t nlam, int64_t ld, const double *dJ_up, const double *dJ_down, double *dJ, hipStream_t st)
{
    vrt_grid *g = p->g;
    const int64_t n = g->n;
    const dim3 tgrid((unsigned)((n + 63) / 64), (unsigned)((nlam + 63) / 64));
    hipLaunchKernelGGL(k_combine_J<double>, tgrid, dim3(256), 0, st, n, (int)nlam, ld, 2, g->up.d_store, g->down.d_srank, dJ_up, dJ_down, dJ);
    VRT_HIP_TRY(hipGetLastError());
    return VRT_OK;
}

static int ensure_step_streams(vrt_plan *p, int G)
{
    if (p->step_groups == G && p->d_step_angles) return VRT_OK;
    const int A = p->A;
    std::vector<int32_t> order((size_t)A);
    for (int a = 0; a < A; a++) order[(size_t)a] = a;
    std::stable_sort(order.begin(), order.end(), [&](int32_t x, int32_t y) {
        return p->angle_visits[(size_t)x] > p->angle_visits[(size_t)y];
    });
    std::vector<int32_t> list;
    p->step_group_off.assign((size_t)G + 1, 0);
    const bool by_dir = G == 2 && p->n_up > 0 && std::abs(p->n_up - p->n_down) <= 1 &&
                        p->tune.step_group_dir != 0;
    for (int gi = 0; gi < G; gi++) {
        p->step_group_off[(size_t)gi] = (int)list.size();
        if (by_dir) {
            for (int j = 0; j < A; j++)
                if ((p->dir_of_active[(size_t)order[(size_t)j]] > 0) == (gi == 0)) list.push_back(order[(size_t)j]);
        } else
        for (int j = gi; j < A; j += G) list.push_back(order[(size_t)j]);
    }
    p->step_group_off[(size_t)G] = (int)list.size();
    int rc;
    if (!p->d_step_angles && (rc = dev_alloc(&p->d_step_angles, (size_t)A))) return rc;
    VRT_HIP_TRY(hipMemcpy(p->d_step_angles, list.data(), sizeof(int32_t) * list.size(), hipMemcpyHostToDevice));
    p->h_step_angles = list;
    dev_free(p->d_patch_work);
    if (!p->step_fork) VRT_HIP_TRY(hipEventCreateWithFlags(&p->step_fork, hipEventDisableTiming));
    for (int gi = 0; gi < 4; gi++) {
        if (gi >= 1 && gi < G && !p->step_stream[gi]) {
            VRT_HIP_TRY(hipStreamCreateWithFlags(&p->step_stream[gi], hipStreamNonBlocking));
            VRT_HIP_TRY(hipEventCreateWithFlags(&p->step_join[gi], hipEventDisableTiming));
        }
    }
    p->step_groups = G;
    return VRT_OK;
}

static int build_level_map(vrt_plan *p, int G, int units)
{
    if (p->d_level_map && p->level_map_groups == G && p->level_map_units == units) return VRT_OK;
    dev_free(p->d_level_map);
    double mean_all = 0.0;
    for (double v : p->angle_mean_levels) mean_all += v;
    mean_all = p->angle_mean_levels.empty() ? 1.0 : std::max(1.0, mean_all / (double)p->angle_mean_levels.size());
    std::vector<int32_t> h_angles((size_t)p->A);
    VRT_HIP_TRY(hipMemcpy(h_angles.data(), p->d_step_angles, sizeof(int32_t) * (size_t)p->A, hipMemcpyDeviceToHost));
    std::vector<int32_t> map;
    p->level_map_off.assign((size_t)G + 1, 0);
    for (int gi = 0; gi < G; gi++) {
        p->level_map_off[(size_t)gi] = (int)map.size();
        const int j0 = p->step_group_off[(size_t)gi], n_list = p->step_group_off[(size_t)gi + 1] - j0;
        const int ntask = n_list * units;
        if (ntask == 0) continue;
        std::vector<double> w((size_t)n_list);
        double W = 0.0;
        for (int j = 0; j < n_list; j++) {
            const int a = h_angles[(size_t)(j0 + j)];
            const double lv = (size_t)a < p->angle_mean_levels.size() ? p->angle_mean_levels[(size_t)a] : mean_all;
            w[(size_t)j] = 1.7 * mean_all + lv;
            W += w[(size_t)j] * units;
        }
        std::vector<std::vector<int32_t>> runs(8);
        double cum = 0.0;
        for (int t = 0; t < ntask; t++) {
            const double wt = w[(size_t)(t / units)];
            const int x = std::min(7, (int)((cum + 0.5 * wt) * 8.0 / W));
            runs[(size_t)x].push_back(t);
            cum += wt;
        }
        size_t per = 0;
        for (const auto &r : runs) per = std::max(per, r.size());
        for (size_t j = 0; j < per; j++)
            for (int x = 0; x < 8; x++) map.push_back(j < runs[(size_t)x].size() ? runs[(size_t)x][j] : -1);
    }
    p->level_map_off[(size_t)G] = (int)map.size();
    if (int rc = dev_alloc(&p->d_level_map, map.size())) return rc;
    VRT_HIP_TRY(hipMemcpy(p->d_level_map, map.data(), sizeof(int32_t) * map.size(), hipMemcpyHostToDevice));
    p->level_map_groups = G;
    p->level_map_units = units;
    return VRT_OK;
}

constexpr int kSingleMaxK64 = 12, kSingleMaxK32 = 18;

template <typename T, int K>
static void launch_levels1(dim3 grid, size_t lds, hipStream_t sg, const StepArgs &sa)
{
    hipLaunchKernelGGL((k_step_levels1<T, K>), grid, dim3(1024), lds, sg, sa);
}

template <typename T>
static void launch_levels1_K(int K, dim3 grid, size_t lds, hipStream_t sg, const StepArgs &sa)
{
    switch ((K + 1) / 2 * 2) {
    case 2: launch_levels1<T, 2>(grid, lds, sg, sa); break;
    case 4: launch_levels1<T, 4>(grid, lds, sg, sa); break;
    case 6: launch_levels1<T, 6>(grid, lds, sg, sa); break;
    case 8: launch_levels1<T, 8>(grid, lds, sg, sa); break;
    case 10: launch_levels1<T, 10>(grid, lds, sg, sa); break;
    case 12: launch_levels1<T, 12>(grid, lds, sg, sa); break;
    default:
        if (sizeof(T) == 4) {
            switch ((K + 1) / 2 * 2) {
            case 14: launch_levels1<float, 14>(grid, lds, sg, sa); break;
            case 16: launch_levels1<float, 16>(grid, lds, sg, sa); break;
            default: launch_levels1<float, 18>(grid, lds, sg, sa); break;
            }
        }
        break;
// ... 327 lines not shown
            if (single) {
                hipLaunchKernelGGL((k_step_coeffs<T, true>), g1, dim3(256), 0, sg, sa);
                const int K1 = std::max(need_K, std::min(force_K, kF32 ? kSingleMaxK32 : kSingleMaxK64));
                launch_levels1_K<T>(std::max(K1, 1), dim3((unsigned)lblocks),
                                    (size_t)(cnt_l + 1) * sizeof(T), sg, sa);
                r.launches += 2;
                continue;
            }
            if constexpr (!kF32) {
                const size_t lds = (size_t)(cnt_l + 1) * sizeof(double2);
                const dim3 g2((unsigned)lblocks);
                hipLaunchKernelGGL((k_step_coeffs<double, false>), g1, dim3(256), 0, sg, sa);
                switch (step_K) {
                case 1: hipLaunchKernelGGL(k_step_levels<1>, g2, dim3(1024), lds, sg, sa); break;
                case 2: hipLaunchKernelGGL(k_step_levels<2>, g2, dim3(1024), lds, sg, sa); break;
                case 3: hipLaunchKernelGGL(k_step_levels<3>, g2, dim3(1024), lds, sg, sa); break;
                case 4: hipLaunchKernelGGL(k_step_levels<4>, g2, dim3(1024), lds, sg, sa); break;
                case 5: hipLaunchKernelGGL(k_step_levels<5>, g2, dim3(1024), lds, sg, sa); break;
                case 6: hipLaunchKernelGGL(k_step_levels<6>, g2, dim3(1024), lds, sg, sa); break;
                case 7: hipLaunchKernelGGL(k_step_levels<7>, g2, dim3(1024), lds, sg, sa); break;
                default: hipLaunchKernelGGL(k_step_levels<8>, g2, dim3(1024), lds, sg, sa); break;
                }
            }
            r.launches += 2;
        }
    }
    return join_streams(p, st, G);
}

template <typename T>
static int patch_reduce_template(vrt_plan *p, const ExecArgs &x, const LayerRun &r, PatchReduce &red)
{
    int rc;
    for (int a = 0; a < p->A; a++) red.w[a] = x.weights[p->user_of_active[(size_t)a]];
    for (int d = 0; d < 2; d++)
        if (r.use_dir[d] && !x.native && (rc = dev_grow(p->ws_J[d], p->ws_J_cap[d], dcount<T>(r.plane)))) return rc;
    return VRT_OK;
}

template <typename T>
static int run_patch_layers(vrt_plan *p, const ExecArgs &x, LayerRun &r)
{
    constexpr bool kF32 = sizeof(T) == 4;
    vrt_grid *g = p->g;
    const int64_t n = g->n;
    const int A = p->A, G = r.G, npair = r.npair;
    const hipStream_t st = x.st;
    int rc;
    if ((rc = ensure_patch_work(p, G, p->h_step_angles, p->step_group_off))) return rc;
    PatchReduce red_tmpl{};
    int owner_of_dir[2] = {-1, -1};
    int64_t reduced_upto[2] = {0, 0};
    if (x.wants_J()) {
        if ((rc = patch_reduce_template<T>(p, x, r, red_tmpl))) return rc;
        for (int d = 0; d < 2; d++)
            for (int gi = 0; gi < G && r.use_dir[d]; gi++)
                if (group_holds_dir(p, gi, d)) owner_of_dir[d] = gi;
    }
    r.fused_dir[0] = owner_of_dir[0] >= 0;
    r.fused_dir[1] = owner_of_dir[1] >= 0;
    auto make_reduce = [&](int gi, int layer_done, bool final, PatchReduce &red) -> bool {
        red = red_tmpl;
        int k = 0;
        for (int d = 0; d < 2; d++) {
            if (owner_of_dir[d] != gi) continue;
            const Direction &dir = d == 0 ? g->up : g->down;
            const int Ld = (int)dir.reduced.size() - 1;
            int64_t upto = reduced_upto[d];
            if (final) upto = n;
            else if (layer_done >= 1 && layer_done <= Ld) upto = dir.reduced[(size_t)layer_done] - 1;
            if (upto <= reduced_upto[d]) continue;
            red.lo[k] = (int)reduced_upto[d];
            red.hi[k] = (int)upto;
            red.Jd[k] = J_planes(p, x, d);
            red.count[k] = 0;
            for (int a = 0; a < A; a++)
                if ((p->dir_of_active[(size_t)a] > 0) == (d == 0)) red.angles[k][red.count[k]++] = a;
            reduced_upto[d] = upto;
            k++;
        }
        return k > 0;
    };
    const int Lmax = deepest_layer(r);
    if ((rc = fork_streams(p, st, G))) return rc;
    r.launches = 0;
    for (int layer = 2; layer <= Lmax; layer++)
        for (int gi = 0; gi < G; gi++) {
            hipStream_t sg = gi == 0 ? st : p->step_stream[gi];
            if (p->step_group_off[gi + 1] == p->step_group_off[gi]) continue;
            int Q = p->tune.patch_Q;
            if (!patch_shape_exists(p->patch_K, Q, p->patch_NT) || (npair % Q != 0 && npair < 2 * Q)) Q = 1;
            PatchReduce red;
            const bool have_red = make_reduce(gi, layer - 1, false, red);
            if ((rc = launch_patch_layer(p, r.ta, npair, layer, gi, Q, sg, kF32, have_red ? &red : nullptr))) return rc;
            r.launches += 1;
        }
    for (int gi = 0; gi < G; gi++) {
        PatchReduce red;
        if (!make_reduce(gi, 0, true, red)) continue;
        if ((rc = launch_patch_layer(p, r.ta, npair, p->tile_max_layers + 1, gi, 1, gi == 0 ? st : p->step_stream[gi], kF32, &red)))
            return rc;
        r.launches += 1;
    }
    return join_streams(p, st, G);
}

template <typename T>
static int run_patch_chain(vrt_plan *p, const ExecArgs &x, LayerRun &r)
{
    constexpr bool kF32 = sizeof(T) == 4;
    const int A = p->A;
    const hipStream_t st = x.st;
    int rc;
    if ((rc = ensure_patch_work(p, r.G, p->h_step_angles, p->step_group_off))) return rc;
    PatchReduce red{};
    if (x.wants_J() && (rc = patch_reduce_template<T>(p, x, r, red))) return rc;
    for (int d = 0; d < 2; d++)
        for (int gi = 1; gi < r.G; gi++)
            if (r.use_dir[d] && r.dir_st[d] == p->step_stream[gi]) {
                VRT_HIP_TRY(hipEventRecord(p->step_join[gi], p->step_stream[gi]));
                VRT_HIP_TRY(hipStreamWaitEvent(st, p->step_join[gi], 0));
            }
    VRT_HIP_TRY(hipEventRecord(p->ev0, st));
    if (x.wants_J())
        for (int d = 0; d < 2; d++) {
            red.count[d] = 0;
            red.Jd[d] = r.use_dir[d] ? J_planes(p, x, d) : nullptr;
            for (int a = 0; a < A; a++)
                if ((p->dir_of_active[(size_t)a] > 0) == (d == 0)) red.angles[d][red.count[d]++] = a;
            r.fused_dir[d] = r.use_dir[d];
        }
    if ((rc = launch_patch_chain(p, r.ta, r.npair, st, kF32, x.wants_J() ? &red : nullptr, r.chain_df, r.prep_ctrl))) return rc;
    r.launches = 1;
    VRT_HIP_TRY(hipEventRecord(p->ev1, st));
    return VRT_OK;
}

template <typename T>
static int finish_outputs(vrt_plan *p, const ExecArgs &x, const LayerRun &r)
{
    vrt_grid *g = p->g;
    const int64_t n = g->n, nlam = x.nlam, ld = x.ld;
    const int A = p->A;
    const hipStream_t st = x.st;
    const T *wI = reinterpret_cast<const T *>(p->d_I);
    int rc;
    if (x.wants_J()) {
        T *Jd[2] = {nullptr, nullptr};
        for (int d = 0; d < 2; d++) {
            if (!r.use_dir[d]) {
                if (x.native && x.J_nat[d]) VRT_HIP_TRY(hipMemsetAsync(x.J_nat[d], 0, r.plane * sizeof(T), st));
                continue;
            }
            if (!x.native && (rc = dev_grow(p->ws_J[d], p->ws_J_cap[d], dcount<T>(r.plane)))) return rc;
            DirWeights dw;
            dw.count = 0;
            for (int a = 0; a < A; a++)
                if ((p->dir_of_active[(size_t)a] > 0) == (d == 0)) {
                    dw.w[dw.count] = x.weights[p->user_of_active[(size_t)a]];
                    dw.idx[dw.count] = a;
                    dw.count++;
                }
            Jd[d] = reinterpret_cast<T *>(J_planes(p, x, d));
            if (r.fused_dir[d]) continue;
            hipLaunchKernelGGL(k_reduce_dir<T>, dim3((unsigned)((r.plane + 255) / 256)), dim3(256), 0, st,
                               (int64_t)r.plane, (int64_t)r.plane, dw, wI, Jd[d]);
// ... 73 lines not shown
```

voronoirt_amd/csrc/vrt_patch.cpp:

```cpp
#include <algorithm>
#include <atomic>
#include <new>

#include "vrt_internal.h"

namespace vrt {

namespace {

struct LayerPatches {
    std::vector<int32_t> own_lo, own_cnt, nlev;
    std::vector<int64_t> ent_off;
    std::vector<int32_t> entry_pos;
    std::vector<uint32_t> entry_vis, entry_loc;
    std::vector<uint32_t> vis;
    int32_t layer_nlev = 0;
    int64_t n_visits = 0, n_live = 0, max_entries = 0, bad_site = -1;
    bool ok = true;
    bool levels_ok = false;
};

void build_layer_patches(const Direction &dir, bool ascending, int n_sweeps, const int32_t *up1, const int32_t *up2,
                         int own_target, int entry_cap, int64_t layer, const int32_t *pos_of, LayerPatches &out)
{
    const std::vector<int64_t> &r = dir.reduced;
    const int32_t lo = (int32_t)(r[(size_t)layer - 1] - 1), hi = (int32_t)(r[(size_t)layer] - 1);
    const int32_t m = hi - lo;
    out.ent_off.push_back(0);
    if (m <= 0) return;
    auto local = [&](int32_t site) -> int32_t {
        const int32_t q = pos_of[(size_t)site];
        return dir.layer_of[(size_t)site] == layer && q >= lo && q < hi ? q - lo : -1;
    };
    std::vector<int32_t> l1((size_t)m), l2((size_t)m);
    for (int32_t p = lo; p < hi; p++) {
        const int32_t i = dir.store[(size_t)p];
        const int32_t u1 = up1[i], u2 = up2[i];
        if (u1 < 0 || u2 < 0) {
            if (out.bad_site < 0 || i < out.bad_site) out.bad_site = i;
            l1[(size_t)(p - lo)] = l2[(size_t)(p - lo)] = -1;
            continue;
        }
        l1[(size_t)(p - lo)] = local(u1);
        l2[(size_t)(p - lo)] = local(u2);
    }
    if (out.bad_site >= 0) {
        out.ok = false;
        return;
    }
    std::vector<uint32_t> t_site;
    std::vector<int32_t> t_src1, t_src2;
    t_site.reserve((size_t)m * 2);
    t_src1.reserve((size_t)m * 2);
    t_src2.reserve((size_t)m * 2);
    std::vector<uint32_t> ver((size_t)m, 0), seen1((size_t)m, UINT32_MAX), seen2((size_t)m, UINT32_MAX);
    std::vector<int32_t> lastw((size_t)m, -1);
    for (int sweep = 0; sweep < n_sweeps; sweep++)
        for (int32_t t = 0; t < m; t++) {
            const int64_t posn = ascending ? (int64_t)lo + t : (int64_t)hi - 1 - t;
            const int32_t i = (int32_t)(dir.perm[(size_t)posn] - 1);
            const int32_t li = pos_of[(size_t)i] - lo;
            const int32_t a = l1[(size_t)li], b = l2[(size_t)li];
            const uint32_t v1 = a >= 0 ? ver[(size_t)a] : 0u, v2 = b >= 0 ? ver[(size_t)b] : 0u;
            if (seen1[(size_t)li] == v1 && seen2[(size_t)li] == v2) continue;
            seen1[(size_t)li] = v1;
            seen2[(size_t)li] = v2;
            ver[(size_t)li]++;
            t_src1.push_back(a >= 0 ? lastw[(size_t)a] : -1);
            t_src2.push_back(b >= 0 ? lastw[(size_t)b] : -1);
            lastw[(size_t)li] = (int32_t)t_site.size();
            t_site.push_back((uint32_t)li);
        }
    const size_t T = t_site.size();
    std::vector<uint8_t> live(T, 0);
    {
        std::vector<uint8_t> needed((size_t)m, 1);
        for (size_t x = T; x-- > 0;) {
            const uint32_t li = t_site[x];
            if (!needed[li]) continue;
            live[x] = 1;
            needed[li] = 0;
            if (t_src1[x] >= 0) needed[(size_t)l1[li]] = 1;
            if (t_src2[x] >= 0) needed[(size_t)l2[li]] = 1;
        }
    }
    {
// ... 175 lines not shown
            ls.max_layer_size = std::max(ls.max_layer_size, r[(size_t)layer] - r[(size_t)layer - 1]);
        if (all) {
            ls.vis.assign((size_t)n, 0u);
            for (int64_t j = 0; j < count; j++) {
                const LayerPatches &l = lp[(size_t)j];
                const int64_t lo = r[(size_t)(first + j) - 1] - 1;
                for (size_t li = 0; li < l.vis.size(); li++) ls.vis[(size_t)dir.store[(size_t)lo + li]] = l.vis[li];
                ls.nlev[(size_t)(first + j)] = l.layer_nlev;
                ls.n_visits += l.n_live;
            }
            ls.ok = true;
        }
    }
    if (out.bad_site >= 0) {
        out.ok = false;
        return;
    }
    for (int64_t j = 0; j < count; j++)
        if (!lp[(size_t)j].ok) {
            out.ok = false;
            return;
        }
    int32_t patch_id = 0;
    for (int64_t j = 0; j < count; j++) {
        LayerPatches &l = lp[(size_t)j];
        out.layer_patch_off[(size_t)(first + j)] = patch_id;
        const int64_t e_base = (int64_t)out.entry_pos.size();
        for (size_t q = 0; q < l.own_lo.size(); q++) {
            out.patch_own_lo.push_back(l.own_lo[q]);
            out.patch_own_cnt.push_back(l.own_cnt[q]);
            out.patch_nlev.push_back(l.nlev[q]);
            out.patch_ent_off.push_back(e_base + l.ent_off[q]);
            patch_id++;
        }
        out.entry_pos.insert(out.entry_pos.end(), l.entry_pos.begin(), l.entry_pos.end());
        out.entry_vis.insert(out.entry_vis.end(), l.entry_vis.begin(), l.entry_vis.end());
        out.entry_loc.insert(out.entry_loc.end(), l.entry_loc.begin(), l.entry_loc.end());
        out.n_visits += l.n_visits;
        out.n_live += l.n_live;
        out.max_entries = std::max(out.max_entries, l.max_entries);
        l = LayerPatches();
    }
    for (int64_t layer = std::max<int64_t>(nl, 2); layer <= nl; layer++) out.layer_patch_off[(size_t)layer] = patch_id;
    out.patch_ent_off.push_back((int64_t)out.entry_pos.size());

    std::vector<int32_t> owner((size_t)n, -1);
    for (int32_t q = 0; q < patch_id; q++)
        for (int32_t j = 0; j < out.patch_own_cnt[(size_t)q]; j++) owner[(size_t)(out.patch_own_lo[(size_t)q] + j)] = q;
    const int dthr = (int)std::max<int64_t>(1, std::min<int64_t>(threads, patch_id / 256 + 1));
    std::vector<std::vector<int32_t>> part_list((size_t)dthr);
    std::vector<std::vector<int32_t>> part_cnt((size_t)dthr);
    auto dep_worker = [&](int t) {
        const int32_t q0 = (int32_t)((int64_t)patch_id * t / dthr), q1 = (int32_t)((int64_t)patch_id * (t + 1) / dthr);
        std::vector<int32_t> deps;
        std::vector<int32_t> &list = part_list[(size_t)t], &cnt = part_cnt[(size_t)t];
        cnt.reserve((size_t)(q1 - q0));
        int64_t layer = first;
        for (int32_t q = q0; q < q1; q++) {
            while (layer < last && q >= out.layer_patch_off[(size_t)layer + 1]) layer++;
            deps.clear();
            for (int64_t e = out.patch_ent_off[(size_t)q]; e < out.patch_ent_off[(size_t)q + 1]; e++) {
                const int32_t i = dir.store[(size_t)out.entry_pos[(size_t)e]];
                for (int qq = 0; qq < 2; qq++) {
                    const int32_t u = qq == 0 ? up1[i] : up2[i];
                    if (dir.layer_of[(size_t)u] < layer && owner[(size_t)pos_of[(size_t)u]] >= 0) deps.push_back(owner[(size_t)pos_of[(size_t)u]]);
                }
            }
            std::sort(deps.begin(), deps.end());
            deps.erase(std::unique(deps.begin(), deps.end()), deps.end());
            list.insert(list.end(), deps.begin(), deps.end());
            cnt.push_back((int32_t)deps.size());
        }
    };
    if (dthr <= 1) dep_worker(0);
    else if (!run_workers(dthr, dep_worker)) throw std::bad_alloc();
    out.dep_off.reserve((size_t)patch_id + 1);
    out.dep_off.push_back(0);
    for (int t = 0; t < dthr; t++) {
        for (int32_t c : part_cnt[(size_t)t]) out.dep_off.push_back(out.dep_off.back() + c);
        out.dep_list.insert(out.dep_list.end(), part_list[(size_t)t].begin(), part_list[(size_t)t].end());
    }
}

}
```

voronoirt_amd/csrc/vrt_patch.hip:

```cpp
#include <hip/hip_runtime.h>

#include <algorithm>
#include <cmath>
#include <cstdio>
#include <cstdlib>
#include <cstring>
#include <type_traits>

#include "vrt_device.h"
#include "vrt_internal.h"

namespace vrt {

enum : int {
    kDiagNoLevels = 1, kDiagCentreGathers = 2, kDiagNoWeights = 4, kDiagNoStores = 8, kDiagNoGatherI = 16, kDiagNoGatherAlpha = 32,
    kDiagNoGatherS = 64, kDiagNoReduce = 128, kDiagNoWait = 256, kDiagPlainLoadI = 512, kDiagPlainStoreI = 1024, kDiagNoPairLoop = 2048,
};
__host__ __device__ __forceinline__ constexpr bool diag(int dbg, int flag) { return kDiag && (dbg & flag) != 0; }

struct PatchArgs {
    TileArgs ta;
    int npair;
    int layer;
    int ngrp;
    int nsplit, Q;
    int lgB;
    int stride;
    int cap;
    int quad;
    int lean;
    int dbg;
    PatchReduce red;
    const int4 *wrec;
    const int32_t *e_pos, *e_u1, *e_u2;
    const uint32_t *e_vis, *e_loc;
    const double *e_w1, *e_w2, *e_r1, *e_r2;
};

__global__ void __launch_bounds__(256)
k_patch_entries(int64_t count, const int32_t *__restrict__ e_pos, const int32_t *__restrict__ t_u1,
                const int32_t *__restrict__ t_u2, const double *__restrict__ t_w1, const double *__restrict__ t_w2,
                const double *__restrict__ t_r1, const double *__restrict__ t_r2, int32_t *__restrict__ e_u1,
                int32_t *__restrict__ e_u2, double *__restrict__ e_w1, double *__restrict__ e_w2,
                double *__restrict__ e_r1, double *__restrict__ e_r2)
{
    const int64_t e = (int64_t)blockIdx.x * blockDim.x + threadIdx.x;
    if (e >= count) return;
    const int p = e_pos[e];
    e_u1[e] = t_u1[p]; e_u2[e] = t_u2[p];
    e_w1[e] = t_w1[p]; e_w2[e] = t_w2[p];
    e_r1[e] = t_r1[p]; e_r2[e] = t_r2[p];
}

int launch_patch_entries(vrt_plan *p, int a, int64_t first, int64_t count)
{
    if (count <= 0) return VRT_OK;
    const size_t o = (size_t)a * (size_t)p->g->n;
    hipLaunchKernelGGL(k_patch_entries, dim3((unsigned)((count + 255) / 256)), dim3(256), 0, p->g->stream, count,
                       p->e_pos + first, p->t_u1 + o, p->t_u2 + o, p->t_w1 + o, p->t_w2 + o, p->t_r1 + o,
                       p->t_r2 + o, p->e_u1 + first, p->e_u2 + first, p->e_w1 + first, p->e_w2 + first,
                       p->e_r1 + first, p->e_r2 + first);
    VRT_HIP_TRY(hipGetLastError());
    return VRT_OK;
}


template <typename T2>
__device__ __forceinline__ double2 ldpair(const T2 *base, int idx, int sh)
{
    const unsigned off = (unsigned)idx << sh;
    return to_d2(*reinterpret_cast<const T2 *>(reinterpret_cast<const char *>(base) + off));
}
template <typename T2> struct Log2Size;
template <> struct Log2Size<double2> { static constexpr int value = 4; };
template <> struct Log2Size<float2> { static constexpr int value = 3; };

__host__ __device__ __forceinline__ void split_blocks(const PatchArgs &pa, int split, int nblock, int &b0, int &b1)
{
    const int nstep = (nblock + pa.Q - 1) / pa.Q;
    const int base = nstep / pa.nsplit, rem = nstep - base * pa.nsplit;
    const int s0 = split * base + (split < rem ? split : rem), s1 = s0 + base + (split < rem ? 1 : 0);
    b0 = s0 * pa.Q;
    b1 = nblock < s1 * pa.Q ? nblock : s1 * pa.Q;
}

#ifndef VRT_REDUCE_LAST
#define VRT_REDUCE_LAST 1
#endif
__device__ __forceinline__ int reduce_block_index(const PatchArgs &pa)
{
    return VRT_REDUCE_LAST ? (int)blockIdx.x - ((int)gridDim.x - pa.red.nred) : ((int)blockIdx.x < pa.red.nred ? (int)blockIdx.x : -1);
}
__device__ __forceinline__ int patch_block_index(const PatchArgs &pa)
{
    return VRT_REDUCE_LAST ? (int)blockIdx.x : (int)blockIdx.x - pa.red.nred;
}
template <typename T, int NT>
__device__ __forceinline__ void patch_reduce_role(const PatchArgs &pa)
{
    typedef typename Pair<T>::type T2;
    const TileArgs &ta = pa.ta;
    const int tid = threadIdx.x;
    int b = reduce_block_index(pa), r = 0;
    if (b >= pa.red.nblk[0]) { b -= pa.red.nblk[0]; r = 1; }
    if (b >= pa.red.nblk[r]) return;
    if (diag(pa.dbg, kDiagNoReduce)) return;
    const int len = pa.red.hi[r] - pa.red.lo[r];
    const int per = NT * pa.red.ppb;
    const int nblock = pair_block_count(pa.npair, pa.lgB);
    int k0 = 0, lw = 0;
    for (int k = 0; k < nblock; k++) {
        pair_block_of(k, pa.npair, pa.lgB, k0, lw);
        const int cnt = (int)((((int64_t)len << lw) + per - 1) / per);
        if (b < cnt) break;
        b -= cnt;
    }
    const int64_t nn = ta.n;
    const size_t run = (size_t)len << lw;
    const size_t base = (size_t)k0 * (size_t)nn + ((size_t)pa.red.lo[r] << lw);
    T2 *Jd = reinterpret_cast<T2 *>(pa.red.Jd[r]);
    const T2 *I0 = reinterpret_cast<const T2 *>(ta.I);
    const size_t plane = (size_t)pa.npair * (size_t)nn;
    if (pa.red.ppb == 4) {
        const size_t f0 = (size_t)b * 4 * NT + tid;
        const unsigned left = f0 < run ? (unsigned)min((size_t)(run - f0 + NT - 1) / NT, (size_t)4) : 0u;
        const size_t e0 = base + (left ? f0 : 0);
        double ax[4], ay[4];
#pragma unroll
        for (int i = 0; i < 4; i++) { ax[i] = 0.0; ay[i] = 0.0; }
        for (int j = 0; j < pa.red.count[r]; j++) {
            const int a = pa.red.angles[r][j];
            const T2 *Ia = I0 + (size_t)a * plane + e0;
            double2 v[4];
#pragma unroll
            for (int i = 0; i < 4; i++) v[i] = to_d2(Ia[(unsigned)i < left ? i * NT : 0]);
#pragma unroll
            for (int i = 0; i < 4; i++) {
                ax[i] += pa.red.w[a] * v[i].x;
                ay[i] += pa.red.w[a] * v[i].y;
            }
        }
#pragma unroll
        for (int i = 0; i < 4; i++)
            if ((unsigned)i < left) Jd[e0 + (size_t)i * NT] = from_d2<T>(make_double2(ax[i], ay[i]));
        return;
    }
    for (int i = 0; i < pa.red.ppb; i++) {
        const size_t f = ((size_t)b * pa.red.ppb + i) * NT + tid;
        if (f >= run) break;
        const size_t e = base + f;
        double ax = 0.0, ay = 0.0;
        for (int j = 0; j < pa.red.count[r]; j++) {
            const int a = pa.red.angles[r][j];
            const double2 v = to_d2(I0[(size_t)a * plane + e]);
            ax += pa.red.w[a] * v.x;
            ay += pa.red.w[a] * v.y;
        }
        Jd[e] = from_d2<T>(make_double2(ax, ay));
    }
}

#ifdef VRT_PATCH_WPE
#define VRT_WPE_ATTR __attribute__((amdgpu_waves_per_eu(VRT_PATCH_WPE, VRT_PATCH_WPE)))
#else
#define VRT_WPE_ATTR
#endif
template <typename T, int AM, int K, int Q, int NT>
__global__ void __launch_bounds__(NT) VRT_WPE_ATTR
k_patch_solve(PatchArgs pa)
{
    typedef typename Pair<T>::type T2;
    extern __shared__ __attribute__((aligned(16))) double2 ptile[];
    const TileArgs &ta = pa.ta;
    const int tid = threadIdx.x;
    if (reduce_block_index(pa) >= 0) {
        patch_reduce_role<T, NT>(pa);
        return;
    }
    const int bid = patch_block_index(pa);
    const int x = bid & 7, rr = bid >> 3;
    const int grp = rr % pa.ngrp, sj = rr / pa.ngrp;
    const int4 rec = pa.wrec[2 * (sj * 8 + x)], rec2 = pa.wrec[2 * (sj * 8 + x) + 1];
    if (rec.y <= 0) return;
    const int sib = grp & ((1 << pa.lgB) - 1);
    const int nblock = pair_block_count(pa.npair, pa.lgB);
    int b0, b1;
    split_blocks(pa, grp >> pa.lgB, nblock, b0, b1);
    if (b0 >= b1) return;
    {
        int k0, lw;
        pair_block_of(b0, pa.npair, pa.lgB, k0, lw);
        if (sib >= (1 << lw)) return;
    }
    const int ent_off = rec.x, n_ent = rec.y, own_lo = rec.z, own_cnt = rec.w;
    const int dbg = kDiag ? pa.dbg : 0;
    const int nlev = diag(dbg, kDiagNoLevels) ? 0 : rec2.x, a = rec2.y & 0xFFFF;
    const int d = rec2.y >> 16;
    const int lo = rec2.z, hi = rec2.w;
    const int64_t n = ta.n;
    const int stride = pa.stride;

    double *s_w1 = reinterpret_cast<double *>(ptile + Q * stride);
    double *s_w2 = s_w1 + pa.cap, *s_r1 = s_w2 + pa.cap, *s_r2 = s_r1 + pa.cap;
    int *s_pos = reinterpret_cast<int *>(s_r2 + pa.cap);
    int *s_u1 = s_pos + pa.cap, *s_u2 = s_u1 + pa.cap;
    uint32_t *s_vis = reinterpret_cast<uint32_t *>(s_u2 + pa.cap), *s_loc = s_vis + pa.cap;
#pragma unroll
    for (int k = 0; k < K; k++) {
        const int i = tid + k * NT;
        const bool ok = i < n_ent;
        const int e = ent_off + (ok ? i : n_ent - 1);
        s_pos[i] = pa.e_pos[e];
        s_u1[i] = pa.e_u1[e];
        s_u2[i] = pa.e_u2[e];
        s_vis[i] = ok ? pa.e_vis[e] : 0u;
        const uint32_t lc = pa.e_loc[e], l1 = lc & 0xFFFFu, l2 = lc >> 16;
        s_loc[i] = (l1 == 0xFFFFu ? (uint32_t)n_ent : l1) | ((l2 == 0xFFFFu ? (uint32_t)n_ent : l2) << 16);
        s_w1[i] = pa.e_w1[e]; s_w2[i] = pa.e_w2[e]; s_r1[i] = pa.e_r1[e]; s_r2[i] = pa.e_r2[e];
    }
    if (tid == 0) {
#pragma unroll
        for (int qi = 0; qi < Q; qi++) ptile[qi * stride + n_ent] = make_double2(0.0, 0.0);
    }
    exp2_table_fill();
    __syncthreads();
    constexpr int lgT2 = Log2Size<T2>::value;
    for (int bk = b0; bk < b1; bk += Q) {
        size_t qbase[Q];
        int qsh[Q];
        bool qok[Q];
#pragma unroll
        for (int qi = 0; qi < Q; qi++) {
            int k0, lw;
            pair_block_of(min(bk + qi, b1 - 1), pa.npair, pa.lgB, k0, lw);
            qok[qi] = bk + qi < b1 && sib < (1 << lw);
            if (!qok[qi] && qi > 0) { qbase[qi] = qbase[qi - 1]; qsh[qi] = qsh[qi - 1]; continue; }
            qbase[qi] = (size_t)k0 * (size_t)n + (size_t)sib;
            qsh[qi] = lw + lgT2;
        }
        if (!qok[0]) break;
        double2 c[K][Q], g1[K][Q], g2[K][Q];
#pragma unroll
        for (int k = 0; k < K; k++) {
            const int i = tid + k * NT;
            const int p = s_pos[i];
            int v1 = s_u1[i], v2 = s_u2[i];
            if (diag(dbg, kDiagCentreGathers)) { v1 = p; v2 = p; }
            int i1 = v1 < lo ? v1 : (int)n - 1, i2 = v2 < lo ? v2 : (int)n - 1;
            if (diag(dbg, kDiagNoGatherI)) { i1 = (int)n - 1; i2 = (int)n - 1; }
            const int av1 = diag(dbg, kDiagNoGatherAlpha) ? p : v1, av2 = diag(dbg, kDiagNoGatherAlpha) ? p : v2;
            const int sv1 = diag(dbg, kDiagNoGatherS) ? p : v1, sv2 = diag(dbg, kDiagNoGatherS) ? p : v2;
            const bool in1 = (v1 >= lo) & (v1 < hi), in2 = (v2 >= lo) & (v2 < hi);
#pragma unroll
            for (int qi = 0; qi < Q; qi++) {
                const int sh = qsh[qi];
                const T2 *__restrict__ S = reinterpret_cast<const T2 *>(ta.S[d]) + qbase[qi];
                const T2 *__restrict__ I = reinterpret_cast<const T2 *>(ta.I) + (size_t)a * pa.npair * (size_t)n + qbase[qi];
                double2 a_c, a_1, a_2;
                if constexpr (AM == VRT_ALPHA_SITE) {
                    const T *__restrict__ Al = reinterpret_cast<const T *>(ta.alpha[d]);
                    const double c0 = Al[p], c1 = Al[av1], c2 = Al[av2];
                    (void)sh;
                    a_c = make_double2(c0, c0); a_1 = make_double2(c1, c1); a_2 = make_double2(c2, c2);
                } else {
                    const T2 *__restrict__ Al =
                        AM == VRT_ALPHA_SITE_LAM
                            ? reinterpret_cast<const T2 *>(ta.alpha[d]) + qbase[qi]
                            : reinterpret_cast<const T2 *>(ta.alpha_angle) + (size_t)a * pa.npair * (size_t)n + qbase[qi];
                    a_c = ldpair(Al, p, sh); a_1 = ldpair(Al, av1, sh); a_2 = ldpair(Al, av2, sh);
                }
                const double2 S_c = ldpair(S, p, sh), S_1 = ldpair(S, sv1, sh), S_2 = ldpair(S, sv2, sh);
                const double2 I_1 = ldpair(I, i1, sh), I_2 = ldpair(I, i2, sh);
                const double w1 = s_w1[i], w2 = s_w2[i], r1 = s_r1[i], r2 = s_r2[i];
                const double wg1 = in1 ? w1 : 0.0, wg2 = in2 ? w2 : 0.0;
                const double rh1 = 0.5 * r1, rh2 = 0.5 * r2;
                if (diag(dbg, kDiagNoWeights)) {
                    c[k][qi] = make_double2(a_c.x + S_c.x + I_1.x + a_1.x + S_1.x, a_c.y + S_c.y + I_2.y + a_2.y + S_2.y);
                    g1[k][qi] = make_double2(w1, w2); g2[k][qi] = make_double2(r1, r2);
                    continue;
                }
                entry_lambda(rh1, rh2, w1, w2, wg1, wg2, a_c.x, a_1.x, a_2.x, S_c.x, S_1.x, S_2.x, I_1.x, I_2.x,
                             c[k][qi].x, g1[k][qi].x, g2[k][qi].x);
                entry_lambda(rh1, rh2, w1, w2, wg1, wg2, a_c.y, a_1.y, a_2.y, S_c.y, S_1.y, S_2.y, I_1.y, I_2.y,
                             c[k][qi].y, g1[k][qi].y, g2[k][qi].y);
            }
        }
        uint32_t vis[K], loc[K];
#pragma unroll
        for (int k = 0; k < K; k++) {
            vis[k] = s_vis[tid + k * NT];
            loc[k] = s_loc[tid + k * NT];
            if (tid + k * NT < n_ent) {
#pragma unroll
                for (int qi = 0; qi < Q; qi++) ptile[qi * stride + tid + k * NT] = make_double2(0.0, 0.0);
            }
        }
        __syncthreads();
        for (int t = 1; t <= nlev; t++) {
#pragma unroll
            for (int k = 0; k < K; k++) {
                if ((vis[k] & 0xFFu) == (uint32_t)t) {
                    const uint32_t l1 = loc[k] & 0xFFFFu, l2 = loc[k] >> 16;
#pragma unroll
                    for (int qi = 0; qi < Q; qi++) {
                        const double2 xv = ptile[qi * stride + l1], yv = ptile[qi * stride + l2];
                        double2 r;
                        r.x = fma(g2[k][qi].x, yv.x, fma(g1[k][qi].x, xv.x, c[k][qi].x));
                        r.y = fma(g2[k][qi].y, yv.y, fma(g1[k][qi].y, xv.y, c[k][qi].y));
                        ptile[qi * stride + tid + k * NT] = r;
                    }
                    vis[k] >>= 8;
                }
            }
            __syncthreads();
        }
#pragma unroll
        for (int k = 0; k < K; k++) {
            const int i = tid + k * NT;
            if (i < own_cnt) {
#pragma unroll
                for (int qi = 0; qi < Q; qi++) {
                    if (qok[qi] && !(diag(dbg, kDiagNoStores) && ptile[qi * stride + i].x != 1.2345e300)) {
                        T2 *I = reinterpret_cast<T2 *>(ta.I) + (size_t)a * pa.npair * (size_t)n + qbase[qi];
                        const unsigned off = (unsigned)(own_lo + i) << qsh[qi];
                        *reinterpret_cast<T2 *>(reinterpret_cast<char *>(I) + off) = from_d2<T>(ptile[qi * stride + i]);
                    }
                }
            }
        }
    }
}


struct PatchItem {
    int sib, b0, b1;
    int ent_off, n_ent, own_lo, own_cnt, nlev, a, d, lo, hi;
};
__device__ __forceinline__ bool patch_item(const PatchArgs &pa, int lgS, PatchItem &it)
{
    const int bid = patch_block_index(pa);
    const int x = bid & 7, rr = bid >> 3;
    const int grp = rr % pa.ngrp, sj = rr / pa.ngrp;
    const int4 rec = pa.wrec[2 * (sj * 8 + x)], rec2 = pa.wrec[2 * (sj * 8 + x) + 1];
    if (rec.y <= 0) return false;
    it.sib = grp & ((1 << lgS) - 1);
    split_blocks(pa, grp >> lgS, pair_block_count(pa.npair, pa.lgB), it.b0, it.b1);
    if (it.b0 >= it.b1) return false;
    it.ent_off = rec.x; it.n_ent = rec.y; it.own_lo = rec.z; it.own_cnt = rec.w;
    it.nlev = rec2.x; it.a = rec2.y & 0xFFFF;
    it.d = rec2.y >> 16;
    it.lo = rec2.z;
    it.hi = rec2.w;
    return true;
}
template <int CAP>
struct EntryTable {
    double *w1, *w2, *r1, *r2;
    int *pos, *u1, *u2;
    uint32_t *vis, *loc;
    __device__ __forceinline__ EntryTable(double2 *tiles, int planes)
    {
        w1 = reinterpret_cast<double *>(tiles + planes * (CAP + 1));
        w2 = w1 + CAP; r1 = w2 + CAP; r2 = r1 + CAP;
        pos = reinterpret_cast<int *>(r2 + CAP);
        u1 = pos + CAP; u2 = u1 + CAP;
        vis = reinterpret_cast<uint32_t *>(u2 + CAP);
        loc = vis + CAP;
    }
    template <typename Tables>
    __device__ __forceinline__ void park(const Tables &pa, const PatchItem &it, int tid) const
    {
        const bool ok = tid < it.n_ent;
        const int e = it.ent_off + (ok ? tid : it.n_ent - 1);
        pos[tid] = pa.e_pos[e];
        u1[tid] = pa.e_u1[e];
        u2[tid] = pa.e_u2[e];
        vis[tid] = ok ? pa.e_vis[e] : 0u;
        const uint32_t lc = pa.e_loc[e], l1 = lc & 0xFFFFu, l2 = lc >> 16;
        loc[tid] = (l1 == 0xFFFFu ? (uint32_t)it.n_ent : l1) | ((l2 == 0xFFFFu ? (uint32_t)it.n_ent : l2) << 16);
        w1[tid] = pa.e_w1[e]; w2[tid] = pa.e_w2[e]; r1[tid] = pa.e_r1[e]; r2[tid] = pa.e_r2[e];
    }
};

struct PairIO {
    int n;
    int npair, lgB, dbg;
    const void *S;
    const void *alpha;
    void *I;
};
template <int AM>
__device__ __forceinline__ PairIO pair_io(const PatchArgs &pa, int d)
{
    PairIO io;
    io.n = (int)pa.ta.n; io.npair = pa.npair; io.lgB = pa.lgB; io.dbg = kDiag ? pa.dbg : 0;
    io.S = pa.ta.S[d];
    io.alpha = AM == VRT_ALPHA_ANGLE_SITE_LAM ? (const void *)pa.ta.alpha_angle : (const void *)pa.ta.alpha[d];
    io.I = pa.ta.I;
    return io;
}

typedef unsigned int vrt_u32x2 __attribute__((ext_vector_type(2)));
typedef unsigned int vrt_u32x4 __attribute__((ext_vector_type(4)));
#ifndef VRT_CHAIN_AUX
#define VRT_CHAIN_AUX 17
#endif
constexpr int kAuxSc1 = VRT_CHAIN_AUX;
constexpr int kChainDepLds = 128;
constexpr int kChainHeadStride = 32;
constexpr int kChainAbortWord = 8 * kChainHeadStride;

struct ChainDev;
constexpr int kCtlItem = 0, kCtlSelf = 1, kCtlNdep = 2, kCtlDepOff = 3, kCtlArgsLo = 4, kCtlArgsHi = 5, kCtlProgLo = 6, kCtlProgHi = 7,
              kCtlBase = 8, kCtlGaveUp = 9, kCtlWords = 12;
template <int CAP>
__device__ __forceinline__ uint32_t *chain_ctl_slots(const EntryTable<CAP> &tab) { return tab.loc + CAP; }
template <int CAP>
__device__ __forceinline__ int32_t *chain_dep_slots(const EntryTable<CAP> &tab) { return reinterpret_cast<int32_t *>(tab.loc + CAP + kCtlWords); }

__device__ __forceinline__ uint32_t ld_agent(const uint32_t *p)
{
    return __hip_atomic_load(p, __ATOMIC_RELAXED, __HIP_MEMORY_SCOPE_AGENT);
}
__device__ __forceinline__ void st_agent(uint32_t *p, uint32_t v)
{
    __hip_atomic_store(p, v, __ATOMIC_RELAXED, __HIP_MEMORY_SCOPE_AGENT);
}
__device__ __forceinline__ uint32_t *chain_progress(const uint32_t *ctl)
{
    return reinterpret_cast<uint32_t *>(((uint64_t)ctl[kCtlProgHi] << 32) | (uint64_t)ctl[kCtlProgLo]);
}
__device__ __forceinline__ uint32_t chain_peek(const int32_t *s_dep, int step)
{
// ... 222 lines not shown
                    rI_1 = BufSc1<T2>::load(rsI, (unsigned)i1 << sh);
                    rI_2 = BufSc1<T2>::load(rsI, (unsigned)i2 << sh);
                }
                if constexpr (CHAIN == 2) {
                    const bool in1 = (v1 >= it.lo) & (v1 < it.hi), in2 = (v2 >= it.lo) & (v2 < it.hi);
                    if (!diag(dbg, kDiagNoWeights)) {
                        LateTerms Lx, Ly;
                        late_lambda(d1x, d2x, (double)rS_1.x, (double)rS_2.x, Lx, d1y);
                        double sink = 0.0;
                        late_lambda(d1y, d2y, (double)rS_1.y, (double)rS_2.y, Ly, sink);
                        if (!diag(dbg, kDiagNoWait)) chain_data_wait<T2>(rsI, (unsigned)i1 << sh, (unsigned)i2 << sh, rI_1, rI_2, s_dep);
                        late_apply(Lx, tab.w1 + tid, tab.w2 + tid, in1, in2, (double)rS_c.x, (double)rI_1.x, (double)rI_2.x, c.x, g1.x, g2.x);
                        late_apply(Ly, tab.w1 + tid, tab.w2 + tid, in1, in2, (double)rS_c.y, (double)rI_1.y, (double)rI_2.y, c.y, g1.y, g2.y);
                    } else {
                        if (!diag(dbg, kDiagNoWait)) chain_data_wait<T2>(rsI, (unsigned)i1 << sh, (unsigned)i2 << sh, rI_1, rI_2, s_dep);
                        c = make_double2(d1x + (double)rS_c.x + (double)rS_1.x + (double)rI_1.x, d2y + (double)rS_c.y + (double)rS_2.y + (double)rI_2.y);
                        g1 = make_double2(in1 ? d2x : 0.0, in1 ? d1y : 0.0);
                        g2 = make_double2(in2 ? d1x : 0.0, in2 ? d2y : 0.0);
                    }
                }
            } else {
                rI_1 = at(Ia + qb, (unsigned)i1 << sh);
                rI_2 = at(Ia + qb, (unsigned)i2 << sh);
            }
            const bool in1 = (v1 >= it.lo) & (v1 < it.hi), in2 = (v2 >= it.lo) & (v2 < it.hi);
            if constexpr (CHAIN == 2) {
            } else if (diag(dbg, kDiagNoWeights)) {
                c = make_double2(d1x + (double)rS_c.x + (double)rS_1.x + (double)rI_1.x, d2y + (double)rS_c.y + (double)rS_2.y + (double)rI_2.y);
                g1 = make_double2(in1 ? d2x : 0.0, in1 ? d1y : 0.0);
                g2 = make_double2(in2 ? d1x : 0.0, in2 ? d2y : 0.0);
            } else {
                entry_lambda_seq(d1x, d2x, tab.w1 + tid, tab.w2 + tid, in1, in2, (double)rS_c.x, (double)rS_1.x, (double)rS_2.x,
                                 (double)rI_1.x, (double)rI_2.x, c.x, g1.x, g2.x, d1y);
                double sink = 0.0;
                entry_lambda_seq(d1y, d2y, tab.w1 + tid, tab.w2 + tid, in1, in2, (double)rS_c.y, (double)rS_1.y, (double)rS_2.y,
                                 (double)rI_1.y, (double)rI_2.y, c.y, g1.y, g2.y, sink);
            }
        }
        uint32_t vis = tab.vis[tid];
        const uint32_t loc = tab.loc[tid];
        {
            double z;
            asm volatile("v_mov_b64 %0, 0" : "=v"(z));
            if (tid < it.n_ent) ptile[tid] = make_double2(z, z);
        }
        if constexpr (CHAIN == 1) asm volatile("s_waitcnt vmcnt(0)" ::: "memory");
        __syncthreads();
        if constexpr (CHAIN == 1) {
            if (bk > it.b0 && tid == 0) chain_publish(s_dep, bk - it.b0);
        }
        const int nlev = diag(dbg, kDiagNoLevels) ? 0 : it.nlev;
        __builtin_amdgcn_s_setprio(VRT_LEVEL_PRIO);
        for (int t = 1; t <= nlev; t++) {
            if ((vis & 0xFFu) == (uint32_t)t) {
                const double2 xv = ptile[loc & 0xFFFFu], yv = ptile[loc >> 16];
                double2 r;
                r.x = fma(g2.x, yv.x, fma(g1.x, xv.x, c.x));
                r.y = fma(g2.y, yv.y, fma(g1.y, xv.y, c.y));
                ptile[tid] = r;
                vis >>= 8;
            }
            __syncthreads();
        }
        __builtin_amdgcn_s_setprio(0);
        if (tid < it.own_cnt && !(diag(dbg, kDiagNoStores) && ptile[tid].x != 1.2345e300)) {
            if (CHAIN && !diag(dbg, kDiagPlainStoreI)) {
                const __amdgpu_buffer_rsrc_t rsI = plane_rsrc(Ia + qb, n << sh);
                BufSc1<T2>::store(rsI, (unsigned)(it.own_lo + tid) << sh, from_d2<T>(ptile[tid]));
            } else {
                T2 *I = reinterpret_cast<T2 *>(pa.I) + (size_t)it.a * pa.npair * (size_t)n + qb;
                *reinterpret_cast<T2 *>(reinterpret_cast<char *>(I) + ((unsigned)(it.own_lo + tid) << sh)) = from_d2<T>(ptile[tid]);
            }
        }
        __syncthreads();
    }
}

template <typename T, int AM, int NT>
__global__ void __launch_bounds__(NT) VRT_LEAN_ATTR
k_patch_lean(PatchArgs pa)
{
    extern __shared__ __attribute__((aligned(16))) double2 ptile[];
    const int tid = threadIdx.x;
    if (reduce_block_index(pa) >= 0) {
        patch_reduce_role<T, NT>(pa);
        return;
    }
    PatchItem it;
    if (!patch_item(pa, pa.lgB, it)) return;
    if (diag(pa.dbg, kDiagNoPairLoop)) it.b1 = it.b0;
    const EntryTable<NT> tab(ptile, 1);
    tab.park(pa, it, tid);
    if (tid == 0) ptile[it.n_ent] = make_double2(0.0, 0.0);
    exp2_table_fill();
    __syncthreads();
    lean_pairs<T, AM, NT, 0>(pair_io<AM>(pa, it.d), it, tab, ptile);
}


template <int AM, int NT, bool CHAIN>
__device__ __forceinline__ void quad_pairs(const PairIO &pa, const PatchItem &it, const EntryTable<NT> &tab,
                                           double2 *ptile)
{
    const int tid = threadIdx.x;
    const int sib2 = it.sib, b0 = it.b0, b1 = it.b1;
    const unsigned n = (unsigned)pa.n;
    const int n_ent = it.n_ent, own_lo = it.own_lo, own_cnt = it.own_cnt, nlev = it.nlev, a = it.a;
    const int lo = it.lo, hi = it.hi;
    constexpr int CAP = NT;
    double2 *tileA = ptile, *tileB = ptile + (CAP + 1);
    double *const s_r1 = tab.r1, *const s_r2 = tab.r2, *const s_w1 = tab.w1, *const s_w2 = tab.w2;
    int *const s_pos = tab.pos, *const s_u1 = tab.u1, *const s_u2 = tab.u2;
    uint32_t *const s_vis = tab.vis, *const s_loc = tab.loc;
    const float2 *Sd = reinterpret_cast<const float2 *>(pa.S);
    const float2 *Ia = reinterpret_cast<const float2 *>(pa.I) + (size_t)a * pa.npair * (size_t)n;
    auto at4 = [](const float2 *base, unsigned off) { return *reinterpret_cast<const float4 *>(reinterpret_cast<const char *>(base) + off); };
    const int32_t *s_dep = chain_dep_slots(tab);
    for (int bk = b0; bk < b1; bk++) {
        int k0, lw;
        if constexpr (CHAIN) { k0 = 2 * bk; lw = 1; }
        else {
            pair_block_of(bk, pa.npair, pa.lgB, k0, lw);
            if (2 * sib2 >= (1 << lw)) break;
        }
        const size_t qb = (size_t)k0 * (size_t)n + (size_t)(CHAIN ? 0 : 2 * sib2);
        const int sh = lw + 3;
        uint32_t seen = 0;
        if constexpr (CHAIN) seen = chain_peek(s_dep, bk - b0 + 1);
        const int p = s_pos[tid], v1 = s_u1[tid], v2 = s_u2[tid];
        double d1x, d2x, d1y, d2y, d1z, d2z, d1w, d2w;
        {
            float4 a_c, a_1, a_2;
            if constexpr (AM == VRT_ALPHA_SITE) {
                const float *__restrict__ A1 = reinterpret_cast<const float *>(pa.alpha);
                const float c0 = A1[p], c1 = A1[v1], c2 = A1[v2];
                a_c = make_float4(c0, c0, c0, c0); a_1 = make_float4(c1, c1, c1, c1); a_2 = make_float4(c2, c2, c2, c2);
            } else {
                const float2 *Al = AM == VRT_ALPHA_SITE_LAM ? reinterpret_cast<const float2 *>(pa.alpha) + qb
                                                            : reinterpret_cast<const float2 *>(pa.alpha) + (size_t)a * pa.npair * (size_t)n + qb;
                a_c = at4(Al, (unsigned)p << sh); a_1 = at4(Al, (unsigned)v1 << sh); a_2 = at4(Al, (unsigned)v2 << sh);
            }
            const double rh1 = 0.5 * s_r1[tid], rh2 = 0.5 * s_r2[tid];
            d1x = rh1 * ((double)a_c.x + (double)a_1.x); d2x = rh2 * ((double)a_c.x + (double)a_2.x);
            d1y = rh1 * ((double)a_c.y + (double)a_1.y); d2y = rh2 * ((double)a_c.y + (double)a_2.y);
            d1z = rh1 * ((double)a_c.z + (double)a_1.z); d2z = rh2 * ((double)a_c.z + (double)a_2.z);
            d1w = rh1 * ((double)a_c.w + (double)a_1.w); d2w = rh2 * ((double)a_c.w + (double)a_2.w);
        }
        asm volatile("" : "+v"(d1x), "+v"(d2x), "+v"(d1y), "+v"(d2y), "+v"(d1z), "+v"(d2z), "+v"(d1w), "+v"(d2w) : : "memory");
        double2 cA, g1A, g2A, cB, g1B, g2B;
        {
            const int i1 = v1 < lo ? v1 : (int)n - 1, i2 = v2 < lo ? v2 : (int)n - 1;
            const bool in1 = (v1 >= lo) & (v1 < hi), in2 = (v2 >= lo) & (v2 < hi);
            const float4 S_c = at4(Sd + qb, (unsigned)p << sh), S_1 = at4(Sd + qb, (unsigned)v1 << sh), S_2 = at4(Sd + qb, (unsigned)v2 << sh);
            float4 I_1, I_2;
            if constexpr (CHAIN) {
                chain_wait(s_dep, bk - b0 + 1, seen);
                const __amdgpu_buffer_rsrc_t rsI = plane_rsrc(Ia + qb, n << sh);
                I_1 = BufSc1<float4>::load(rsI, (unsigned)i1 << sh);
                I_2 = BufSc1<float4>::load(rsI, (unsigned)i2 << sh);
            } else {
                I_1 = at4(Ia + qb, (unsigned)i1 << sh);
                I_2 = at4(Ia + qb, (unsigned)i2 << sh);
            }
            entry_lambda_seq(d1x, d2x, s_w1 + tid, s_w2 + tid, in1, in2, (double)S_c.x, (double)S_1.x, (double)S_2.x,
                             (double)I_1.x, (double)I_2.x, cA.x, g1A.x, g2A.x, d1y);
            entry_lambda_seq(d1y, d2y, s_w1 + tid, s_w2 + tid, in1, in2, (double)S_c.y, (double)S_1.y, (double)S_2.y,
                             (double)I_1.y, (double)I_2.y, cA.y, g1A.y, g2A.y, d1z);
            entry_lambda_seq(d1z, d2z, s_w1 + tid, s_w2 + tid, in1, in2, (double)S_c.z, (double)S_1.z, (double)S_2.z,
                             (double)I_1.z, (double)I_2.z, cB.x, g1B.x, g2B.x, d1w);
            double sink = 0.0;
            entry_lambda_seq(d1w, d2w, s_w1 + tid, s_w2 + tid, in1, in2, (double)S_c.w, (double)S_1.w, (double)S_2.w,
                             (double)I_1.w, (double)I_2.w, cB.y, g1B.y, g2B.y, sink);
        }
        uint32_t vis = s_vis[tid];
        const uint32_t loc = s_loc[tid];
        {
            double z;
            asm volatile("v_mov_b64 %0, 0" : "=v"(z));
            if (tid < n_ent) {
                tileA[tid] = make_double2(z, z);
                tileB[tid] = make_double2(z, z);
            }
        }
        if constexpr (CHAIN) asm volatile("s_waitcnt vmcnt(0)" ::: "memory");
        __syncthreads();
        if constexpr (CHAIN) {
            if (bk > b0 && tid == 0) chain_publish(s_dep, bk - b0);
        }
        for (int t = 1; t <= nlev; t++) {
            if ((vis & 0xFFu) == (uint32_t)t) {
                const uint32_t l1 = loc & 0xFFFFu, l2 = loc >> 16;
                const double2 xa = tileA[l1], ya = tileA[l2], xb = tileB[l1], yb = tileB[l2];
                double2 ra, rb;
                ra.x = fma(g2A.x, ya.x, fma(g1A.x, xa.x, cA.x));
                ra.y = fma(g2A.y, ya.y, fma(g1A.y, xa.y, cA.y));
                rb.x = fma(g2B.x, yb.x, fma(g1B.x, xb.x, cB.x));
                rb.y = fma(g2B.y, yb.y, fma(g1B.y, xb.y, cB.y));
                tileA[tid] = ra;
                tileB[tid] = rb;
                vis >>= 8;
            }
            __syncthreads();
        }
        if (tid < own_cnt) {
            const double2 ra = tileA[tid], rb = tileB[tid];
            const float4 out = make_float4((float)ra.x, (float)ra.y, (float)rb.x, (float)rb.y);
            if constexpr (CHAIN) {
                const __amdgpu_buffer_rsrc_t rsI = plane_rsrc(Ia + qb, n << sh);
                BufSc1<float4>::store(rsI, (unsigned)(own_lo + tid) << sh, out);
            } else {
                float2 *I = reinterpret_cast<float2 *>(pa.I) + (size_t)a * pa.npair * (size_t)n + qb;
                *reinterpret_cast<float4 *>(reinterpret_cast<char *>(I) + ((unsigned)(own_lo + tid) << sh)) = out;
            }
        }
        __syncthreads();
    }
}

#ifndef VRT_QUAD_ATTR
#define VRT_QUAD_ATTR __attribute__((amdgpu_waves_per_eu(6, 6)))
#endif
template <int AM, int NT>
__global__ void __launch_bounds__(NT) VRT_QUAD_ATTR
k_patch_quad(PatchArgs pa)
{
    extern __shared__ __attribute__((aligned(16))) double2 ptile[];
    const int tid = threadIdx.x;
    if (reduce_block_index(pa) >= 0) {
        patch_reduce_role<float, NT>(pa);
        return;
    }
    PatchItem it;
    if (!patch_item(pa, pa.lgB - 1, it)) return;
    const EntryTable<NT> tab(ptile, 2);
    tab.park(pa, it, tid);
    if (tid == 0) {
        ptile[it.n_ent] = make_double2(0.0, 0.0);
        ptile[NT + 1 + it.n_ent] = make_double2(0.0, 0.0);
    }
    exp2_table_fill();
    __syncthreads();
    quad_pairs<AM, NT, false>(pair_io<AM>(pa, it.d), it, tab, ptile);
}


struct ChainDev {
    TileArgs ta;
    int npair, nsplit, cap;
    const int32_t *e_pos, *e_u1, *e_u2;
    const uint32_t *e_vis, *e_loc;
    const double *e_w1, *e_w2, *e_r1, *e_r2;
    PatchReduce red;
    const int4 *items;
    int q_off[9];
    const int32_t *deps;
    uint32_t *progress;
    uint32_t *ctrl;
    uint32_t *host_status;
    int64_t n_patches;
    uint32_t spin_limit;
    int static_items;
    int dbg;
};

__device__ __forceinline__ const uint32_t *chain_abort_word(const uint32_t *cd_words)
{
    return reinterpret_cast<const ChainDev *>(cd_words)->ctrl + kChainAbortWord;
}

__device__ __forceinline__ int cd_int(const int *p) { return __builtin_amdgcn_readfirstlane(*p); }
template <typename P>
__device__ __forceinline__ P *cd_ptr(P *const *p) { return uniform_ptr(*p); }

__device__ __forceinline__ void chain_wait_slow(const int32_t *s_dep, int step)
{
    const int lane = (int)(threadIdx.x & 63u);
    const uint32_t *ctl = reinterpret_cast<const uint32_t *>(s_dep - kCtlWords);
    const ChainDev *cd = reinterpret_cast<const ChainDev *>(((uint64_t)ctl[kCtlArgsHi] << 32) | (uint64_t)ctl[kCtlArgsLo]);
    uint32_t *abort_word = cd->ctrl + kChainAbortWord;
    const uint32_t *progress = chain_progress(ctl);
    const uint32_t target = ctl[kCtlBase] + (uint32_t)step, limit = cd->spin_limit;
    const int ndep = (int)ctl[kCtlNdep];
    for (int c0 = 0; c0 < ndep; c0 += 64) {
        const int j = c0 + lane;
        const int dep = j < 64 + kChainDepLds ? s_dep[j] : (j < ndep ? (cd->deps + ctl[kCtlDepOff])[j] : (int)ctl[kCtlSelf]);
        const uint32_t *w = progress + dep;
        uint32_t spins = 0;
        for (;;) {
            const uint32_t v = ld_agent(w);
            if (__all(j >= ndep || (int)(v - target) >= 0)) break;
            __builtin_amdgcn_s_sleep(8);
            if ((++spins & 127u) == 1u) {
                if (spins > limit) {
                    st_agent(abort_word, 1u);
                    uint32_t *hs = cd->host_status;
                    __hip_atomic_store(hs + 1, ctl[kCtlItem], __ATOMIC_RELAXED, __HIP_MEMORY_SCOPE_SYSTEM);
                    __hip_atomic_store(hs, 1u, __ATOMIC_RELAXED, __HIP_MEMORY_SCOPE_SYSTEM);
                }
                if (ld_agent(abort_word) != 0u) return;
            }
        }
    }
}

__device__ __forceinline__ void chain_data_give_up_cd(const ChainDev *cd, uint32_t item)
{
    st_agent(cd->ctrl + kChainAbortWord, 1u);
    uint32_t *hs = cd->host_status;
    __hip_atomic_store(hs + 1, item, __ATOMIC_RELAXED, __HIP_MEMORY_SCOPE_SYSTEM);
    __hip_atomic_store(hs, 1u, __ATOMIC_RELAXED, __HIP_MEMORY_SCOPE_SYSTEM);
}

template <typename T, int NT, int LGB, int MODE>
__device__ __forceinline__ void chain_reduce(const ChainDev &cd, const ChainDev *cdp, uint32_t item, int r, int lo, int hi, int b0, int b1)
{
    typedef typename Pair<T>::type T2;
    const int tid = threadIdx.x;
    if (diag(cd.dbg, kDiagNoReduce)) return;
    const int64_t nn = cd.ta.n;
    const int npair = cd.npair;
    const size_t plane = (size_t)npair * (size_t)nn;
    T2 *Jd = reinterpret_cast<T2 *>(cd.red.Jd[r]);
    const T2 *I0 = reinterpret_cast<const T2 *>(cd.ta.I);
    const int count = cd.red.count[r];
    constexpr int lgT2 = Log2Size<T2>::value;
// ... 127 lines not shown
        __syncthreads();
        if (tid == 0 && s_ctl[kCtlGaveUp]) chain_data_give_up_cd(cd, (uint32_t)idx);
    }
    if constexpr (MODE == 1) {
        asm volatile("s_waitcnt vmcnt(0)" ::: "memory");
        __syncthreads();
        if (tid == 0) chain_publish(s_dep, b1 - b0);
    }
}

template <typename T, int AM, int NT>
__global__ void __launch_bounds__(NT) VRT_LEAN_ATTR
k_patch_chain(ChainDev ca, const ChainDev *cd, uint32_t base)
{
    extern __shared__ __attribute__((aligned(16))) double2 ptile[];
    chain_item<T, AM, NT, false, 1>(ca, cd, base, ptile);
}
template <typename T, int AM, int NT>
__global__ void __launch_bounds__(NT) __attribute__((amdgpu_waves_per_eu(6, 6)))
k_patch_chain_df(ChainDev ca, const ChainDev *cd, uint32_t base)
{
    extern __shared__ __attribute__((aligned(16))) double2 ptile[];
    chain_item<T, AM, NT, false, 2>(ca, cd, base, ptile);
}
template <int AM, int NT>
__global__ void __launch_bounds__(NT) VRT_QUAD_ATTR
k_patch_chain_quad(ChainDev ca, const ChainDev *cd, uint32_t base)
{
    extern __shared__ __attribute__((aligned(16))) double2 ptile[];
    chain_item<float, AM, NT, true, 1>(ca, cd, base, ptile);
}

#define VRT_PATCH_SHAPES(X) \
    X(1, 1, 256) X(1, 1, 512) X(1, 1, 1024) X(2, 1, 256) X(2, 1, 512) X(1, 2, 256) X(1, 2, 512) X(1, 2, 1024) X(2, 2, 512)

template <typename T, int AM>
static int launch_shape(int K, int Q, int NT, dim3 grid, size_t lds, hipStream_t st, const PatchArgs &pa)
{
    if constexpr (sizeof(T) == 4) {
        if (pa.quad) {
            switch (NT) {
            case 256: hipLaunchKernelGGL((k_patch_quad<AM, 256>), grid, dim3(256), lds, st, pa); return VRT_OK;
            case 512: hipLaunchKernelGGL((k_patch_quad<AM, 512>), grid, dim3(512), lds, st, pa); return VRT_OK;
            case 1024: hipLaunchKernelGGL((k_patch_quad<AM, 1024>), grid, dim3(1024), lds, st, pa); return VRT_OK;
            default: break;
            }
        }
    }
    if (pa.lean && K == 1 && Q == 1) {
        switch (NT) {
        case 256: hipLaunchKernelGGL((k_patch_lean<T, AM, 256>), grid, dim3(256), lds, st, pa); return VRT_OK;
        case 512: hipLaunchKernelGGL((k_patch_lean<T, AM, 512>), grid, dim3(512), lds, st, pa); return VRT_OK;
        case 1024: hipLaunchKernelGGL((k_patch_lean<T, AM, 1024>), grid, dim3(1024), lds, st, pa); return VRT_OK;
        default: break;
        }
    }
#define VRT_PATCH_CASE(k, q, nt) \
    if (K == k && Q == q && NT == nt) { hipLaunchKernelGGL((k_patch_solve<T, AM, k, q, nt>), grid, dim3(nt), lds, st, pa); return VRT_OK; }
    VRT_PATCH_SHAPES(VRT_PATCH_CASE)
#undef VRT_PATCH_CASE
    return fail(VRT_EINVAL, "no patch kernel for this (entries per thread, pairs, threads) shape");
}

template <typename T>
static int launch_mode(int am, int K, int Q, int NT, dim3 grid, size_t lds, hipStream_t st, const PatchArgs &pa)
{
    switch (am) {
    case VRT_ALPHA_SITE: return launch_shape<T, VRT_ALPHA_SITE>(K, Q, NT, grid, lds, st, pa);
    case VRT_ALPHA_SITE_LAM: return launch_shape<T, VRT_ALPHA_SITE_LAM>(K, Q, NT, grid, lds, st, pa);
    default: return launch_shape<T, VRT_ALPHA_ANGLE_SITE_LAM>(K, Q, NT, grid, lds, st, pa);
    }
}

bool patch_shape_exists(int K, int Q, int NT)
{
#define VRT_PATCH_CASE(k, q, nt) if (K == k && Q == q && NT == nt) return true;
    VRT_PATCH_SHAPES(VRT_PATCH_CASE)
#undef VRT_PATCH_CASE
    return false;
}

int ensure_patch_work(vrt_plan *p, int G, const std::vector<int32_t> &group_angles, const std::vector<int> &group_off)
{
    if (p->d_patch_work && p->patch_work_groups == G) return VRT_OK;
    if (p->d_patch_work) { (void)hipFree(p->d_patch_work); p->d_patch_work = nullptr; }
    const int maxL = p->tile_max_layers;
    std::vector<int4> work;
    p->patch_work_off.assign((size_t)G * (size_t)(maxL + 2) + 1, 0);
    std::vector<std::pair<int64_t, int32_t>> items;
    for (int gi = 0; gi < G; gi++)
        for (int layer = 0; layer <= maxL + 1; layer++) {
            p->patch_work_off[(size_t)gi * (size_t)(maxL + 2) + (size_t)layer] = (int64_t)(work.size() / 2);
            if (layer < 2 || layer > maxL) continue;
            items.clear();
            for (int j = group_off[(size_t)gi]; j < group_off[(size_t)gi + 1]; j++) {
                const int a = group_angles[(size_t)j];
                const int32_t *first = p->h_patch_first.data() + (size_t)a * (size_t)(maxL + 2);
                for (int32_t q = first[layer]; q < first[layer + 1]; q++)
                    items.push_back({(int64_t)p->h_patch_rec[(size_t)q].z * 64 + (j - group_off[(size_t)gi]), q});
            }
            std::sort(items.begin(), items.end());
            const size_t m = items.size();
            if (m == 0) continue;
            const size_t slots = (m + 7) / 8;
            const size_t base = work.size();
            work.resize(base + slots * 8 * 2, make_int4(0, 0, 0, 0));
            for (int x = 0; x < 8; x++) {
                const size_t b0 = m * (size_t)x / 8, b1 = m * (size_t)(x + 1) / 8;
                for (size_t t = b0; t < b1; t++) {
                    const int32_t q = items[t].second;
                    const int2 r2 = p->h_patch_rec2[(size_t)q];
                    const int d = p->dir_of_active[(size_t)r2.y] > 0 ? 0 : 1;
                    const Direction &dir = d == 0 ? p->g->up : p->g->down;
                    const size_t slot = base + 2 * ((t - b0) * 8 + (size_t)x);
                    work[slot] = p->h_patch_rec[(size_t)q];
                    work[slot + 1] = make_int4(r2.x, r2.y | (d << 16), (int)(dir.reduced[(size_t)layer - 1] - 1), (int)(dir.reduced[(size_t)layer] - 1));
                }
            }
        }
    p->patch_work_off.back() = (int64_t)(work.size() / 2);
    if (int rc = dev_alloc(&p->d_patch_work, work.size())) return rc;
    VRT_HIP_TRY(hipMemcpy(p->d_patch_work, work.data(), sizeof(int4) * work.size(), hipMemcpyHostToDevice));
    p->patch_work_groups = G;
    return VRT_OK;
}

static void size_reduce(PatchReduce &red, int npair, int lgB, int NT)
{
    red.nred = 0;
    int64_t total = 0;
    for (int r = 0; r < 2; r++)
        if (red.count[r] > 0 && red.Jd[r]) total += (int64_t)std::max(0, red.hi[r] - red.lo[r]) * npair;
    red.ppb = total <= (int64_t)NT * 1024 ? 1 : 4;
    const int64_t per = (int64_t)NT * red.ppb;
    const int nblock = pair_block_count(npair, lgB);
    for (int r = 0; r < 2; r++) {
        const int64_t len = red.hi[r] - red.lo[r];
        red.nblk[r] = 0;
        if (len > 0 && red.count[r] > 0 && red.Jd[r])
            for (int k = 0; k < nblock; k++) {
                int k0, lw;
                pair_block_of(k, npair, lgB, k0, lw);
                red.nblk[r] += (int)(((len << lw) + per - 1) / per);
            }
        red.nred += red.nblk[r];
    }
    red.nred = (red.nred + 7) / 8 * 8;
}

int launch_patch_layer(vrt_plan *p, const TileArgs &ta, int npair, int layer, int group, int Q, hipStream_t st,
                       bool f32, const PatchReduce *reduce)
{
    const int target_wgs = p->tune.patch_target;
    const int maxL = p->tile_max_layers;
    const size_t wo = (size_t)group * (size_t)(maxL + 2) + (size_t)layer;
    const int64_t w0 = (layer >= 2 && layer <= maxL) ? p->patch_work_off[wo] : 0, w1 = (layer >= 2 && layer <= maxL) ? p->patch_work_off[wo + 1] : 0;
    PatchArgs pa;
    if (reduce) {
        pa.red = *reduce;
        size_reduce(pa.red, npair, native_lg(p, f32), p->patch_NT);
    }
    if (w1 <= w0 && pa.red.nred == 0) return VRT_OK;
    pa.ta = ta;
    pa.npair = npair;
    pa.layer = layer;
    pa.lgB = native_lg(p, f32);
    pa.quad = (f32 && pa.lgB >= 1 && p->patch_K == 1 && p->tune.patch_quad != 0 && (npair & 1) == 0) ? 1 : 0;
    if (pa.quad) Q = 1;
    pa.lean = (p->tune.patch_lean != 0 && p->patch_K == 1 && Q == 1 && !pa.quad && npair >= 2) ? 1 : 0;
    const int lgS = pa.lgB - pa.quad;
    pa.Q = Q;
    pa.nsplit = 1;
    pa.ngrp = 1 << lgS;
    if (w1 > w0) {
        const int64_t items = (w1 - w0) << lgS;
        const int nblock = pair_block_count(npair, pa.lgB);
        const int steps_all = (nblock + Q - 1) / Q;
        int nsplit;
        if (p->tune.patch_split > 0) nsplit = std::min(steps_all, p->tune.patch_split);
        else if (target_wgs > 0) nsplit = (int)std::max<int64_t>(1, std::min<int64_t>(steps_all, (target_wgs + items - 1) / items));
        else {
            const double T = std::min(900.0, 460.0 + 4100.0 / (double)steps_all);
            const int s_min = (int)std::min<int64_t>(steps_all, std::max<int64_t>(1, (512 + items - 1) / items));
            double dmin = 1e300;
            for (int c = steps_all; c >= 1; c--) {
                const int sc = (steps_all + c - 1) / c;
                if (sc >= s_min) dmin = std::min(dmin, std::fabs(std::log((double)items * sc / T)));
            }
            nsplit = s_min;
            for (int c = steps_all; c >= 1; c--) {
                const int sc = (steps_all + c - 1) / c;
                if (sc >= s_min && std::fabs(std::log((double)items * sc / T)) <= dmin + 0.03) nsplit = sc;
            }
        }
        pa.nsplit = nsplit;
        pa.ngrp = nsplit << lgS;
    }
    pa.stride = p->patch_cap + 1;
    pa.cap = p->patch_cap;
    pa.dbg = kDiag ? p->tune.debug_flags : 0;
    pa.wrec = p->d_patch_work + 2 * w0;
    pa.e_pos = p->e_pos; pa.e_u1 = p->e_u1; pa.e_u2 = p->e_u2;
    pa.e_vis = p->e_vis; pa.e_loc = p->e_loc;
    pa.e_w1 = p->e_w1; pa.e_w2 = p->e_w2; pa.e_r1 = p->e_r1; pa.e_r2 = p->e_r2;
    const dim3 grid((unsigned)(pa.red.nred + (w1 - w0) * pa.ngrp));
    const size_t lds = (size_t)(pa.quad ? 2 : Q) * (size_t)pa.stride * sizeof(double2) + (size_t)pa.cap * (4 * sizeof(double) + 5 * sizeof(int32_t));
    const int rc = f32 ? launch_mode<float>(ta.alpha_mode, p->patch_K, Q, p->patch_NT, grid, lds, st, pa)
                       : launch_mode<double>(ta.alpha_mode, p->patch_K, Q, p->patch_NT, grid, lds, st, pa);
    return rc;
}

bool patch_chain_possible(const vrt_plan *p, int npair, bool f32)
{
    if (!p->patch_ok || p->tune.patch_chain == 0 || p->patch_K != 1 || p->patch_NT != 512) return false;
    const int lgB = native_lg(p, f32);
    const bool quad = f32 && lgB >= 1 && p->tune.patch_quad != 0 && (npair & 1) == 0;
    if (lgB - (quad ? 1 : 0) != 0) return false;
    if (!f32 && p->tune.patch_lean == 0) return false;
    if (p->tile_max_layers >= 65535 || p->A > 63) return false;
    if (p->tune.patch_chain == 1) return true;
    if (f32) return false;
    const double per_layer = (double)p->n_patches / (double)std::max(1, p->tile_max_layers);
    return per_layer * (double)pair_block_count(npair, lgB) <= 1400.0;
}

bool patch_chain_dataflag(const vrt_plan *p, int npair, bool f32)
{
    if (f32 || p->tune.chain_dataflag == 0 || native_lg(p, f32) != 0) return false;
    return p->tune.chain_dataflag == 1 || npair <= 2;
}

static int chain_nsplit(const vrt_plan *p, int nblock)
{
    const int per = std::max(1, p->tune.chain_pairs);
    const double per_layer = (double)p->n_patches / (double)std::max(1, p->tile_max_layers);
    const int fill = (int)std::ceil(1024.0 / std::max(1.0, per_layer));
    return std::max(1, std::min({std::max((nblock + per - 1) / per, fill), nblock, 511}));
}

static int ensure_patch_chain(vrt_plan *p, int npair, int lgB, int nsplit, bool with_reduce)
{
    if (p->d_chain_items && p->chain_npair == npair && p->chain_lgB == lgB && p->chain_nsplit == nsplit &&
        p->chain_reduce == (with_reduce ? 1 : 0))
        return VRT_OK;
    {
        auto stash = [&]() {
            if (!p->d_chain_items) return;
            vrt_plan::ChainSet cs;
            cs.npair = p->chain_npair; cs.lgB = p->chain_lgB; cs.nsplit = p->chain_nsplit; cs.reduce = p->chain_reduce;
            cs.items = p->d_chain_items; cs.deps = p->d_chain_deps; cs.n_items = p->chain_items;
            for (int x = 0; x <= 8; x++) cs.q_off[x] = p->chain_q_off[x];
            p->d_chain_items = nullptr; p->d_chain_deps = nullptr;
            p->chain_npair = -1;
            p->chain_cache.push_back(cs);
            if (p->chain_cache.size() > 3) {
                (void)hipFree(p->chain_cache.front().items);
                (void)hipFree(p->chain_cache.front().deps);
                p->chain_cache.erase(p->chain_cache.begin());
            }
        };
        for (size_t c = 0; c < p->chain_cache.size(); c++) {
            const vrt_plan::ChainSet cs = p->chain_cache[c];
            if (cs.npair == npair && cs.lgB == lgB && cs.nsplit == nsplit && cs.reduce == (with_reduce ? 1 : 0)) {
                p->chain_cache.erase(p->chain_cache.begin() + (long)c);
                stash();
                p->d_chain_items = cs.items; p->d_chain_deps = cs.deps; p->chain_items = cs.n_items;
                for (int x = 0; x <= 8; x++) p->chain_q_off[x] = cs.q_off[x];
                p->chain_npair = npair; p->chain_lgB = lgB; p->chain_nsplit = nsplit; p->chain_reduce = with_reduce ? 1 : 0;
                const size_t words = (size_t)nsplit * (size_t)std::max<int64_t>(p->n_patches, 1);
                if (words <= p->chain_progress_cap) return VRT_OK;
                break;
            }
        }
        stash();
    }
    const vrt_grid *g = p->g;
    const int maxL = p->tile_max_layers, A = p->A;
    const int64_t n = g->n, n_patches = p->n_patches;
    const int nblock = pair_block_count(npair, lgB);
    if ((int64_t)nsplit * n_patches >= ((int64_t)1 << 31)) return fail(VRT_EINVAL, "too many (split, patch) progress words");
    PatchArgs sp;
    sp.nsplit = nsplit;
    sp.Q = 1;
    std::vector<int> steps((size_t)nsplit);
    for (int s = 0; s < nsplit; s++) {
        int b0, b1;
        split_blocks(sp, s, nblock, b0, b1);
        steps[(size_t)s] = b1 - b0;
    }
    std::vector<int4> q[8];
    std::vector<int32_t> rdeps;
    const size_t dep_base = p->h_patch_deps.size();
    std::vector<std::pair<int64_t, int32_t>> items;
    std::vector<int> dir_angles[2];
    for (int a = 0; a < A; a++) dir_angles[p->dir_of_active[(size_t)a] > 0 ? 0 : 1].push_back(a);
    std::vector<int32_t> run_start((size_t)(maxL + 2) * 2 * 8, 0);
    auto first_of = [&](int a, int layer) { return p->h_patch_first[(size_t)a * (size_t)(maxL + 2) + (size_t)layer]; };
    auto level_queues = [&]() {
        size_t longest = 0;
        for (int x = 0; x < 8; x++) longest = std::max(longest, q[x].size());
        for (int x = 0; x < 8; x++)
            while (q[x].size() < longest) {
                q[x].push_back(make_int4(0, 0, 0x40000000, 0));
                q[x].push_back(make_int4(0, 0, 0, 0));
                q[x].push_back(make_int4(0, 0, 0, 0));
            }
    };
    auto emit_reduce = [&](int layer) {
        if (!with_reduce) return;
        for (int d = 0; d < 2; d++) {
            const Direction &dir = d == 0 ? g->up : g->down;
            const int Ld = (int)dir.reduced.size() - 1;
            if (dir_angles[d].empty() || layer < 1 || layer > Ld) continue;
            const int64_t lo = dir.reduced[(size_t)layer - 1] - 1;
            const int64_t hi = layer == Ld ? n : dir.reduced[(size_t)layer] - 1;
            const int32_t *rs = run_start.data() + ((size_t)layer * 2 + (size_t)d) * 8;
            constexpr int64_t R = 512;
            for (int64_t clo = lo; clo < hi; clo += R) {
                const int64_t chi = std::min(hi, clo + R);
                int x = 0;
                if (layer >= 2) { while (x < 7 && rs[x + 1] <= clo) x++; }
                else x = (int)std::min<int64_t>(7, 8 * (clo - lo) / std::max<int64_t>(1, hi - lo));
                const size_t d0 = rdeps.size();
                if (layer >= 2)
                    for (int a : dir_angles[d])
                        for (int32_t pq = first_of(a, layer); pq < first_of(a, layer + 1); pq++) {
                            const int4 &rec = p->h_patch_rec[(size_t)pq];
                            if (rec.z < chi && rec.z + rec.w > clo) rdeps.push_back(pq);
                        }
                for (int s = 0; s < nsplit; s++) {
                    q[x].push_back(make_int4((int)clo, (int)chi, (int)0x80000000u, (d << 6) | (s << 7)));
                    q[x].push_back(make_int4((int)(dep_base + d0), (int)(rdeps.size() - d0), 0, steps[(size_t)s]));
                    q[x].push_back(make_int4(0, 0, 0, 0));
                }
            }
        }
    };
    for (int layer = 2; layer <= maxL; layer++) {
        for (int d = 0; d < 2; d++) {
            const Direction &dir = d == 0 ? g->up : g->down;
            if (layer > (int)dir.reduced.size() - 1) continue;
            items.clear();
            for (size_t j = 0; j < dir_angles[d].size(); j++) {
                const int a = dir_angles[d][j];
                for (int32_t pq = first_of(a, layer); pq < first_of(a, layer + 1); pq++)
                    items.push_back({(int64_t)p->h_patch_rec[(size_t)pq].z * 64 + (int64_t)j, pq});
            }
            std::sort(items.begin(), items.end());
            const size_t m = items.size();
            int32_t *rs = run_start.data() + ((size_t)layer * 2 + (size_t)d) * 8;
            for (int x = 0; x < 8; x++) {
                const size_t t0 = m * (size_t)x / 8, t1 = m * (size_t)(x + 1) / 8;
                rs[x] = t0 < m ? p->h_patch_rec[(size_t)items[t0].second].z : INT32_MAX;
                for (size_t t = t0; t < t1; t++) {
                    const int32_t pq = items[t].second;
                    const int4 &rec = p->h_patch_rec[(size_t)pq];
                    const int2 &rec2 = p->h_patch_rec2[(size_t)pq];
                    const int64_t o0 = p->h_patch_dep_off[(size_t)pq], o1 = p->h_patch_dep_off[(size_t)pq + 1];
                    for (int s = 0; s < nsplit; s++) {
                        q[x].push_back(make_int4(rec.x, rec.z, rec.y | (rec.w << 10) | (rec2.x << 20),
                                                 rec2.y | (d << 6) | (s << 7) | (layer << 16)));
                        q[x].push_back(make_int4((int)o0, (int)(o1 - o0), pq, 0));
                        q[x].push_back(make_int4((int)(dir.reduced[(size_t)layer - 1] - 1), (int)(dir.reduced[(size_t)layer] - 1), 0, 0));
                    }
                }
            }
            level_queues();
        }
        emit_reduce(layer - 1);
        level_queues();
// ... 158 lines not shown
```

Baseline: 87.85 billion.

## Build per-item cost-based workgroup records for patch layer launches

Replaces the uniform per-launch split of pair blocks across workgroups with precomputed per-workgroup records. The records are built on the host from a per-item cost model (levels, entries, prologue), cached per split rule, and uploaded to the device, so each workgroup reads its item and block range from a record instead of deriving them from uniform nsplit/ngrp. The aim is to balance load when patch items vary in depth. It also adds a diagnostics-only per-workgroup time log plus query APIs for the records. In exchange it adds host-side record construction, device memory for up to 16 cached record sets, and a device synchronisation when that cache evicts a set.

```diff
diff --git a/include/voronoirt.h b/include/voronoirt.h
--- a/include/voronoirt.h
+++ b/include/voronoirt.h
@@ -131,6 +131,13 @@
 int vrt_patch_schedule_get_deps(const vrt_patch_schedule *s, int64_t *dep_off, int32_t *dep_list);
 int vrt_patch_schedule_get_layers(const vrt_patch_schedule *s, uint32_t *vis, int32_t *nlev, int64_t *n_visits);
 void vrt_patch_schedule_destroy(vrt_patch_schedule *s);
+int vrt_patch_split_records(int64_t n_items, const int32_t *n_ent, const int32_t *nlev, int npair, int pair_block, int quad,
+                            int Q, int cost, int split, int target, int64_t cap, int32_t *records, double *est,
+                            int64_t counts[3]);
+int vrt_plan_patch_records(vrt_plan *p, int npair, int cost, int64_t cap_offsets, int64_t *offsets, int64_t cap_records,
+                           int32_t *records, int64_t counts[2]);
+int vrt_plan_patch_timelog(vrt_plan *p, int64_t cap_launches, int64_t *launches, int64_t cap_rows, uint32_t *rows,
+                           int64_t counts[2]);
 
 int vrt_delaunay_up(vrt_grid *g, const double k[3], const double *S, const double *I0,
                     int64_t nI0, const double *alpha, int n_sweeps, double *I_out);
diff --git a/voronoirt_amd/_lib.py b/voronoirt_amd/_lib.py
--- a/voronoirt_amd/_lib.py
+++ b/voronoirt_amd/_lib.py
@@ -130,6 +130,10 @@
     "vrt_patch_schedule_get_deps": (ctypes.c_int, [vp, p_i64, p_i32]),
     "vrt_patch_schedule_get_layers": (ctypes.c_int, [vp, ctypes.POINTER(ctypes.c_uint32), p_i32, p_i64]),
     "vrt_patch_schedule_destroy": (None, [vp]),
+    "vrt_patch_split_records": (ctypes.c_int, [c_i64, p_i32, p_i32, ctypes.c_int, ctypes.c_int, ctypes.c_int, ctypes.c_int,
+                                               ctypes.c_int, ctypes.c_int, ctypes.c_int, c_i64, p_i32, p_dbl, p_i64]),
+    "vrt_plan_patch_records": (ctypes.c_int, [vp, ctypes.c_int, ctypes.c_int, c_i64, p_i64, c_i64, p_i32, p_i64]),
+    "vrt_plan_patch_timelog": (ctypes.c_int, [vp, c_i64, p_i64, c_i64, ctypes.POINTER(ctypes.c_uint32), p_i64]),
     "vrt_lambda_update_dev": (ctypes.c_int, [vp, c_i64, c_i64, vp, vp, vp, vp, vp, p_dbl, vp]),
     "vrt_short_characteristics": (ctypes.c_int, [c_i64, c_i64, c_i64, p_dbl, p_dbl, p_dbl, c_i64, p_dbl,
                                                  p_int, p_dbl, c_i64, p_dbl, c_i64, p_dbl, ctypes.c_int,
diff --git a/voronoirt_amd/csrc/vrt_api.cpp b/voronoirt_amd/csrc/vrt_api.cpp
--- a/voronoirt_amd/csrc/vrt_api.cpp
+++ b/voronoirt_amd/csrc/vrt_api.cpp
@@ -27,7 +27,7 @@
     static const char *names[] = {"VRT_PATH", "VRT_STEP_K", "VRT_STEP_SINGLE", "VRT_STEP_PAIRS", "VRT_STEP_XCD",
                                   "VRT_STEP_STREAMS", "VRT_STEP_LEVEL_MAP", "VRT_STEP_GROUP_DIR", "VRT_TILE_WIDE",
                                   "VRT_TILE_PRE", "VRT_PATCH_K", "VRT_PATCH_NT", "VRT_PATCH_OWN",
-                                  "VRT_PATCH_Q", "VRT_PATCH_TARGET", "VRT_PATCH_SPLIT", "VRT_PAIR_BLOCK", "VRT_PATCH_QUAD", "VRT_PATCH_LEAN", "VRT_PATCH_CHAIN", "VRT_CHAIN_PAIRS", "VRT_CHAIN_SPIN", "VRT_CHAIN_DATAFLAG", "VRT_CHAIN_STATIC", "VRT_LAMBDA_NATIVE", "VRT_DEBUG_FLAGS", "VRT_DEBUG_SKIP_LEVELS",
+                                  "VRT_PATCH_Q", "VRT_PATCH_TARGET", "VRT_PATCH_SPLIT", "VRT_PATCH_SPLIT_COST", "VRT_PAIR_BLOCK", "VRT_PATCH_QUAD", "VRT_PATCH_LEAN", "VRT_PATCH_CHAIN", "VRT_CHAIN_PAIRS", "VRT_CHAIN_SPIN", "VRT_CHAIN_DATAFLAG", "VRT_CHAIN_STATIC", "VRT_LAMBDA_NATIVE", "VRT_DEBUG_FLAGS", "VRT_DEBUG_SKIP_LEVELS",
                                   "VRT_TILE_DEBUG"};
     for (const char *nm : names) {
         const char *e = std::getenv(nm);
@@ -65,7 +65,7 @@
         {"VRT_TILE_PRE", &t.tile_pre, 0, 1, false},
         {"VRT_PATCH_K", &t.patch_K, 1, 8, true}, {"VRT_PATCH_NT", &t.patch_NT, 64, 1024, true},
         {"VRT_PATCH_OWN", &t.patch_own, 0, 65535, true}, {"VRT_PATCH_Q", &t.patch_Q, 1, 4, false},
-        {"VRT_PATCH_TARGET", &t.patch_target, 0, 1 << 20, false}, {"VRT_PATCH_SPLIT", &t.patch_split, 0, 4096, false}, {"VRT_PAIR_BLOCK", &t.pair_block, 1, 16, true},
+        {"VRT_PATCH_TARGET", &t.patch_target, 0, 1 << 20, false}, {"VRT_PATCH_SPLIT", &t.patch_split, 0, 4096, false}, {"VRT_PATCH_SPLIT_COST", &t.patch_split_cost, 0, 1, false}, {"VRT_PAIR_BLOCK", &t.pair_block, 1, 16, true},
         {"VRT_PATCH_QUAD", &t.patch_quad, 0, 1, true}, {"VRT_PATCH_LEAN", &t.patch_lean, 0, 1, false},
         {"VRT_PATCH_CHAIN", &t.patch_chain, 0, 2, false}, {"VRT_CHAIN_PAIRS", &t.chain_pairs, 1, 256, false},
         {"VRT_CHAIN_SPIN", &t.chain_spin, 1, 1 << 20, false}, {"VRT_CHAIN_DATAFLAG", &t.chain_dataflag, 0, 2, false},
@@ -241,7 +241,8 @@
     for (int i = 0; i < 2; i++) dev_free(p->ws_cg[i]);
     dev_free(p->d_step_angles);
     dev_free(p->d_level_map);
-    dev_free(p->d_patch_work);
+    free_patch_workgroups(p);
+    dev_free(p->d_patch_tlog);
     dev_free(p->d_chain_items); dev_free(p->d_chain_deps); dev_free(p->d_chain_progress); dev_free(p->d_chain_ctrl);
     for (auto &cs : p->chain_cache) { dev_free(cs.items); dev_free(cs.deps); }
     p->chain_cache.clear();
@@ -1181,6 +1182,106 @@
 
 void vrt_patch_schedule_destroy(vrt_patch_schedule *s) { delete s; }
 
+int vrt_patch_split_records(int64_t n_items, const int32_t *n_ent, const int32_t *nlev, int npair, int pair_block, int quad,
+                            int Q, int cost, int split, int target, int64_t cap, int32_t *records, double *est,
+                            int64_t counts[3])
+{
+    if (!n_ent || !nlev || !counts) return fail(VRT_EINVAL, "NULL argument");
+    if (n_items < 1 || n_items > (1 << 24) || npair < 1 || Q < 1 || pair_block < 1 || pair_block > 16 || (pair_block & (pair_block - 1)) ||
+        quad < 0 || quad > 1 || (quad && pair_block < 2))
+        return fail(VRT_EINVAL, "need 1 <= n_items <= 2^24, npair >= 1, Q >= 1, pair_block 1, 2, 4, 8 or 16 (>= 2 with quad)");
+    return guarded([&] {
+        const size_t m = (size_t)n_items, slots = (m + 7) / 8;
+        std::vector<int4> items(slots * 8 * 2, make_int4(0, 0, 0, 0));
+        for (int x = 0; x < 8; x++) {
+            const size_t b0 = m * (size_t)x / 8, b1 = m * (size_t)(x + 1) / 8;
+            for (size_t t = b0; t < b1; t++) {
+                if (n_ent[t] < 1) return fail(VRT_EINVAL, "an item needs at least one entry");
+                items[2 * ((t - b0) * 8 + (size_t)x)] = make_int4((int)t, n_ent[t], 0, 0);
+                items[2 * ((t - b0) * 8 + (size_t)x) + 1] = make_int4(nlev[t], 0, 0, 0);
+            }
+        }
+        PatchSplitRule rule;
+        rule.npair = npair; rule.quad = quad; rule.Q = Q; rule.cost = cost; rule.split = split; rule.target = target;
+        while ((1 << rule.lgB) < pair_block) rule.lgB++;
+        PatchWorkgroups wg;
+        if (!build_patch_workgroups(items.data(), (int64_t)slots, rule, wg))
+            return fail(VRT_EINVAL, "launch does not fit the workgroup record (levels <= 255, pair blocks <= 65535)");
+        const int64_t n = (int64_t)wg.est.size();
+        counts[0] = n; counts[1] = wg.budget; counts[2] = wg.nsplit;
+        if (!records && !est) return VRT_OK;
+        if (cap < n) return fail(VRT_EINVAL, "output arrays too short");
+        for (int64_t w = 0; w < n; w++) {
+            const int4 &r = wg.rec[2 * (size_t)w], &r2 = wg.rec[2 * (size_t)w + 1];
+            if (records) {
+                records[4 * w] = r.y > 0 ? r.x : -1;
+                records[4 * w + 1] = (r2.y >> 17) & 0x7F;
+                records[4 * w + 2] = r2.x & 0xFFFF;
+                records[4 * w + 3] = (int32_t)((uint32_t)r2.x >> 16);
+            }
+            if (est) est[w] = wg.est[(size_t)w];
+        }
+        return VRT_OK;
+    });
+}
+
+int vrt_plan_patch_timelog(vrt_plan *p, int64_t cap_launches, int64_t *launches, int64_t cap_rows, uint32_t *rows,
+                           int64_t counts[2])
+{
+    if (!p || !counts) return fail(VRT_EINVAL, "NULL argument");
+#ifndef VRT_DIAG
+    return fail(VRT_EINVAL, "the time log of the patch launches exists in the diagnostics build only (-DVRT_DIAG)");
+#endif
+    return guarded([&] {
+        std::lock_guard<std::mutex> lock(p->mu);
+        if (int rc = use_device(p->g->device)) return rc;
+        counts[0] = (int64_t)(p->patch_tlog_launch.size() / 5);
+        counts[1] = p->patch_tlog_used;
+        if (!launches && !rows) return VRT_OK;
+        if (cap_launches < counts[0] || cap_rows < counts[1]) return fail(VRT_EINVAL, "output arrays too short");
+        VRT_HIP_TRY(hipDeviceSynchronize());
+        if (launches) std::copy(p->patch_tlog_launch.begin(), p->patch_tlog_launch.end(), launches);
+        if (rows && counts[1] > 0)
+            VRT_HIP_TRY(hipMemcpy(rows, p->d_patch_tlog, sizeof(uint4) * 2 * (size_t)counts[1], hipMemcpyDeviceToHost));
+        return VRT_OK;
+    });
+}
+
+int vrt_plan_patch_records(vrt_plan *p, int npair, int cost, int64_t cap_offsets, int64_t *offsets, int64_t cap_records,
+                           int32_t *records, int64_t counts[2])
+{
+    if (!p || !counts) return fail(VRT_EINVAL, "NULL argument");
+    return guarded([&] {
+        std::lock_guard<std::mutex> lock(p->mu);
+        if (int rc = use_device(p->g->device)) return rc;
+        const vrt_plan::PatchWgSet *set = nullptr;
+        for (const auto &s : p->patch_wg_sets)
+            if (s.rule.npair == npair && (s.rule.cost != 0) == (cost != 0)) set = &s;
+        if (!set) return fail(VRT_EINVAL, "no per-layer patch launch of this plan has run with that pair count and split rule");
+        const int64_t n = set->off.back();
+        counts[0] = (int64_t)set->off.size();
+        counts[1] = n;
+        if (!offsets && !records) return VRT_OK;
+        if ((offsets && cap_offsets < counts[0]) || (records && cap_records < n)) return fail(VRT_EINVAL, "output arrays too short");
+        if (offsets) std::copy(set->off.begin(), set->off.end(), offsets);
+        if (records && n > 0) {
+            std::vector<int4> h(2 * (size_t)n);
+            VRT_HIP_TRY(hipDeviceSynchronize());
+            VRT_HIP_TRY(hipMemcpy(h.data(), set->d_rec, sizeof(int4) * h.size(), hipMemcpyDeviceToHost));
+            for (int64_t w = 0; w < n; w++) {
+                const int4 &r = h[2 * (size_t)w], &r2 = h[2 * (size_t)w + 1];
+                int32_t *o = records + 6 * w;
+                o[0] = r.x; o[1] = r.y;
+                o[2] = (r2.y >> 17) & 0x7F;
+                o[3] = r2.x & 0xFFFF;
+                o[4] = (int32_t)((uint32_t)r2.x >> 16);
+                o[5] = (int32_t)((uint32_t)r2.y >> 24);
+            }
+        }
+        return VRT_OK;
+    });
+}
+
 int vrt_grid_get_storage_order(const vrt_grid *g, int dir, int64_t *out)
 {
     if (!g || !out) return fail(VRT_EINVAL, "NULL argument");
diff --git a/voronoirt_amd/csrc/vrt_internal.h b/voronoirt_amd/csrc/vrt_internal.h
--- a/voronoirt_amd/csrc/vrt_internal.h
+++ b/voronoirt_amd/csrc/vrt_internal.h
@@ -171,6 +171,7 @@
     int chain_dataflag = 2;
     int patch_split = 0;
     int patch_target = 0;
+    int patch_split_cost = 1;
     int chain_static = 1;
     int lambda_native = 1;
     int debug_flags = 0, debug_skip_levels = 0, tile_debug = 0;
@@ -225,6 +226,38 @@
 namespace vrt {
 struct RasterLocator;
 void raster_locator_free(vrt_grid *g);
+}
+
+namespace vrt {
+struct PatchSplitRule {
+    int npair = 0, lgB = 0, quad = 0, Q = 1;
+    int cost = 0;
+    int split = 0, target = 0;
+    bool operator==(const PatchSplitRule &o) const
+    {
+        return npair == o.npair && lgB == o.lgB && quad == o.quad && Q == o.Q && cost == o.cost && split == o.split && target == o.target;
+    }
+};
+constexpr double kSplitStepBase = 3.32, kSplitStepPerLevel = 0.0885, kSplitStepPerEntry = 0.0, kSplitPrologue = 10.24;
+inline double patch_step_cost(int nlev, int n_ent)
+{
+    return kSplitStepBase + kSplitStepPerLevel * (double)nlev + kSplitStepPerEntry * (double)n_ent;
+}
+inline void split_blocks(int Q, int nsplit, int split, int nblock, int &b0, int &b1)
+{
+    const int nstep = (nblock + Q - 1) / Q;
+    const int base = nstep / nsplit, rem = nstep - base * nsplit;
+    const int s0 = split * base + (split < rem ? split : rem), s1 = s0 + base + (split < rem ? 1 : 0);
+    b0 = s0 * Q;
+    b1 = nblock < s1 * Q ? nblock : s1 * Q;
+}
+struct PatchWorkgroups {
+    std::vector<int4> rec;
+    std::vector<double> est;
+    int budget = 0;
+    int nsplit = 0;
+};
+bool build_patch_workgroups(const int4 *items, int64_t slots, const PatchSplitRule &rule, PatchWorkgroups &out);
 }
 
 struct vrt_grid {
@@ -353,9 +386,18 @@
     };
     std::vector<ChainSet> chain_cache;
     uint32_t chain_epoch = 0;
-    int4 *d_patch_work = nullptr;
+    std::vector<int4> h_patch_work;
     std::vector<int64_t> patch_work_off;
     int patch_work_groups = 0;
+    struct PatchWgSet {
+        vrt::PatchSplitRule rule;
+        int4 *d_rec = nullptr;
+        std::vector<int64_t> off;
+    };
+    std::vector<PatchWgSet> patch_wg_sets;
+    uint4 *d_patch_tlog = nullptr;
+    int64_t patch_tlog_cap = 0, patch_tlog_used = 0;
+    std::vector<int64_t> patch_tlog_launch;
     hipStream_t step_stream[4] = {nullptr, nullptr, nullptr, nullptr};
     hipEvent_t step_fork = nullptr, step_join[4] = {nullptr, nullptr, nullptr, nullptr};
     int last_path = 0;
@@ -504,6 +546,8 @@
 bool patch_shape_exists(int K, int Q, int NT);
 int launch_patch_entries(vrt_plan *p, int a, int64_t first, int64_t count);
 int ensure_patch_work(vrt_plan *p, int G, const std::vector<int32_t> &group_angles, const std::vector<int> &group_off);
+void free_patch_workgroups(vrt_plan *p);
+int patch_tlog_begin(vrt_plan *p, hipStream_t st);
 int launch_patch_layer(vrt_plan *p, const TileArgs &ta, int npair, int layer, int group, int Q, hipStream_t st,
                        bool f32, const PatchReduce *reduce);
 bool patch_chain_possible(const vrt_plan *p, int npair, bool f32);
diff --git a/voronoirt_amd/csrc/vrt_layers.hip b/voronoirt_amd/csrc/vrt_layers.hip
--- a/voronoirt_amd/csrc/vrt_layers.hip
+++ b/voronoirt_amd/csrc/vrt_layers.hip
@@ -192,7 +192,7 @@
     if (!p->d_step_angles && (rc = dev_alloc(&p->d_step_angles, (size_t)A))) return rc;
     VRT_HIP_TRY(hipMemcpy(p->d_step_angles, list.data(), sizeof(int32_t) * list.size(), hipMemcpyHostToDevice));
     p->h_step_angles = list;
-    dev_free(p->d_patch_work);
+    free_patch_workgroups(p);
     if (!p->step_fork) VRT_HIP_TRY(hipEventCreateWithFlags(&p->step_fork, hipEventDisableTiming));
     for (int gi = 0; gi < 4; gi++) {
         if (gi >= 1 && gi < G && !p->step_stream[gi]) {
@@ -686,6 +686,7 @@
         return k > 0;
     };
     const int Lmax = deepest_layer(r);
+    if ((rc = patch_tlog_begin(p, st))) return rc;
     if ((rc = fork_streams(p, st, G))) return rc;
     r.launches = 0;
     for (int layer = 2; layer <= Lmax; layer++)
diff --git a/voronoirt_amd/csrc/vrt_patch.cpp b/voronoirt_amd/csrc/vrt_patch.cpp
--- a/voronoirt_amd/csrc/vrt_patch.cpp
+++ b/voronoirt_amd/csrc/vrt_patch.cpp
@@ -2,6 +2,9 @@
 #include <atomic>
 #include <new>
 
+#include <cmath>
+
+#include "vrt_device.h"
 #include "vrt_internal.h"
 
 namespace vrt {
@@ -343,4 +346,129 @@
     }
 }
 
-}
+namespace {
+
+int uniform_split(int64_t items, int steps_all, const PatchSplitRule &r)
+{
+    if (r.split > 0) return std::min(steps_all, r.split);
+    if (r.target > 0) return (int)std::max<int64_t>(1, std::min<int64_t>(steps_all, (r.target + items - 1) / items));
+    const double T = std::min(900.0, 460.0 + 4100.0 / (double)steps_all);
+    const int s_min = (int)std::min<int64_t>(steps_all, std::max<int64_t>(1, (512 + items - 1) / items));
+    double dmin = 1e300;
+    for (int c = steps_all; c >= 1; c--) {
+        const int sc = (steps_all + c - 1) / c;
+        if (sc >= s_min) dmin = std::min(dmin, std::fabs(std::log((double)items * sc / T)));
+    }
+    int nsplit = s_min;
+    for (int c = steps_all; c >= 1; c--) {
+        const int sc = (steps_all + c - 1) / c;
+        if (sc >= s_min && std::fabs(std::log((double)items * sc / T)) <= dmin + 0.03) nsplit = sc;
+    }
+    return nsplit;
+}
+
+void workgroup_record(const int4 &it, const int4 &it2, int sib, int b0, int b1, int4 &r, int4 &r2)
+{
+    r = it;
+    const uint32_t blocks = (uint32_t)b0 | ((uint32_t)b1 << 16);
+    const uint32_t who = ((uint32_t)it2.y & 0x1FFFFu) | ((uint32_t)sib << 17) | ((uint32_t)it2.x << 24);
+    r2 = make_int4((int)blocks, (int)who, it2.z, it2.w);
+}
+
+}
+
+bool build_patch_workgroups(const int4 *items, int64_t slots, const PatchSplitRule &r, PatchWorkgroups &out)
+{
+    out = PatchWorkgroups();
+    const int lgS = r.lgB - r.quad, nsib = 1 << lgS;
+    const int nblock = pair_block_count(r.npair, r.lgB);
+    const int steps_all = (nblock + r.Q - 1) / r.Q;
+    if (nblock > 0xFFFF || lgS < 0 || lgS > 6 || slots <= 0 || steps_all < 1) return false;
+    for (int64_t t = 0; t < slots * 8; t++)
+        if (items[2 * t].y > 0 && (items[2 * t + 1].x < 0 || items[2 * t + 1].x > 255)) return false;
+    const bool per_item = r.cost != 0 && r.split <= 0 && r.target <= 0;
+    if (!per_item) {
+        const int nsplit = uniform_split(slots * 8 << lgS, steps_all, r);
+        const int ngrp = nsplit << lgS;
+        out.nsplit = nsplit;
+        out.rec.assign((size_t)slots * 8 * (size_t)ngrp * 2, make_int4(0, 0, 0, 0));
+        out.est.assign((size_t)slots * 8 * (size_t)ngrp, 0.0);
+        for (int64_t sj = 0; sj < slots; sj++)
+            for (int x = 0; x < 8; x++) {
+                const int4 &it = items[2 * (sj * 8 + x)], &it2 = items[2 * (sj * 8 + x) + 1];
+                if (it.y <= 0) continue;
+                for (int grp = 0; grp < ngrp; grp++) {
+                    int b0, b1;
+                    split_blocks(r.Q, nsplit, grp >> lgS, nblock, b0, b1);
+                    if (b0 >= b1) continue;
+                    const size_t w = (size_t)((sj * ngrp + grp) * 8 + x);
+                    workgroup_record(it, it2, grp & (nsib - 1), b0, b1, out.rec[2 * w], out.rec[2 * w + 1]);
+                    out.est[w] = kSplitPrologue + (double)((b1 - b0 + r.Q - 1) / r.Q) * patch_step_cost(it2.x, it.y);
+                }
+            }
+        return true;
+    }
+    std::vector<int64_t> live;
+    for (int64_t t = 0; t < slots * 8; t++)
+        if (items[2 * t].y > 0) live.push_back(t);
+    const int64_t m = (int64_t)live.size();
+    if (m == 0) return false;
+    int64_t W = (int64_t)std::min(900.0, 460.0 + 4100.0 / (double)steps_all);
+    W = std::max<int64_t>(W, 512);
+    W = std::min<int64_t>(W, (m << lgS) * steps_all);
+    W = std::max<int64_t>(W, m << lgS);
+    out.budget = (int)W;
+    std::vector<double> c((size_t)m);
+    double hi = 0.0;
+    for (int64_t i = 0; i < m; i++) {
+        c[(size_t)i] = patch_step_cost(items[2 * live[(size_t)i] + 1].x, items[2 * live[(size_t)i]].y);
+        hi = std::max(hi, c[(size_t)i] * steps_all);
+    }
+    auto count = [&](double T) -> int64_t {
+        int64_t sum = 0;
+        for (int64_t i = 0; i < m; i++) {
+            const int mi = (int)std::min<double>(steps_all, std::floor(T / c[(size_t)i]));
+            if (mi < 1) return -1;
+            sum += (steps_all + mi - 1) / mi;
+        }
+        return sum;
+    };
+    double lo = 0.0;
+    hi *= 1.0 + 1e-9;
+    for (int itn = 0; itn < 60; itn++) {
+        const double mid = 0.5 * (lo + hi);
+        const int64_t cnt = count(mid);
+        if (cnt >= 0 && (cnt << lgS) <= W) hi = mid;
+        else lo = mid;
+    }
+    struct Wg { double est; int64_t slot; int sib, b0, b1; };
+    std::vector<Wg> q[8];
+    for (int64_t i = 0; i < m; i++) {
+        const int64_t t = live[(size_t)i];
+        const int mi = (int)std::max(1.0, std::min<double>(steps_all, std::floor(hi / c[(size_t)i])));
+        const int s = (steps_all + mi - 1) / mi;
+        for (int sp = 0; sp < s; sp++) {
+            int b0, b1;
+            split_blocks(r.Q, s, sp, nblock, b0, b1);
+            const double est = kSplitPrologue + (double)((b1 - b0 + r.Q - 1) / r.Q) * c[(size_t)i];
+            for (int sib = 0; sib < nsib; sib++) q[t & 7].push_back({est, t, sib, b0, b1});
+        }
+    }
+    size_t len = 0;
+    for (int x = 0; x < 8; x++) {
+        std::stable_sort(q[x].begin(), q[x].end(), [](const Wg &a, const Wg &b) { return a.est > b.est; });
+        len = std::max(len, q[x].size());
+    }
+    out.rec.assign(len * 8 * 2, make_int4(0, 0, 0, 0));
+    out.est.assign(len * 8, 0.0);
+    for (int x = 0; x < 8; x++)
+        for (size_t k = 0; k < q[x].size(); k++) {
+            const Wg &w = q[x][k];
+            const size_t b = k * 8 + (size_t)x;
+            workgroup_record(items[2 * w.slot], items[2 * w.slot + 1], w.sib, w.b0, w.b1, out.rec[2 * b], out.rec[2 * b + 1]);
+            out.est[b] = w.est;
+        }
+    return true;
+}
+
+}
diff --git a/voronoirt_amd/csrc/vrt_patch.hip b/voronoirt_amd/csrc/vrt_patch.hip
--- a/voronoirt_amd/csrc/vrt_patch.hip
+++ b/voronoirt_amd/csrc/vrt_patch.hip
@@ -15,6 +15,7 @@
 enum : int {
     kDiagNoLevels = 1, kDiagCentreGathers = 2, kDiagNoWeights = 4, kDiagNoStores = 8, kDiagNoGatherI = 16, kDiagNoGatherAlpha = 32,
     kDiagNoGatherS = 64, kDiagNoReduce = 128, kDiagNoWait = 256, kDiagPlainLoadI = 512, kDiagPlainStoreI = 1024, kDiagNoPairLoop = 2048,
+    kDiagTimeLog = 4096,
 };
 __host__ __device__ __forceinline__ constexpr bool diag(int dbg, int flag) { return kDiag && (dbg & flag) != 0; }
 
@@ -22,8 +23,7 @@
     TileArgs ta;
     int npair;
     int layer;
-    int ngrp;
-    int nsplit, Q;
+    int Q;
     int lgB;
     int stride;
     int cap;
@@ -32,6 +32,7 @@
     int dbg;
     PatchReduce red;
     const int4 *wrec;
+    uint4 *tlog;
     const int32_t *e_pos, *e_u1, *e_u2;
     const uint32_t *e_vis, *e_loc;
     const double *e_w1, *e_w2, *e_r1, *e_r2;
@@ -75,15 +76,6 @@
 template <> struct Log2Size<double2> { static constexpr int value = 4; };
 template <> struct Log2Size<float2> { static constexpr int value = 3; };
 
-__host__ __device__ __forceinline__ void split_blocks(const PatchArgs &pa, int split, int nblock, int &b0, int &b1)
-{
-    const int nstep = (nblock + pa.Q - 1) / pa.Q;
-    const int base = nstep / pa.nsplit, rem = nstep - base * pa.nsplit;
-    const int s0 = split * base + (split < rem ? split : rem), s1 = s0 + base + (split < rem ? 1 : 0);
-    b0 = s0 * pa.Q;
-    b1 = nblock < s1 * pa.Q ? nblock : s1 * pa.Q;
-}
-
 #ifndef VRT_REDUCE_LAST
 #define VRT_REDUCE_LAST 1
 #endif
@@ -94,6 +86,17 @@
 __device__ __forceinline__ int patch_block_index(const PatchArgs &pa)
 {
     return VRT_REDUCE_LAST ? (int)blockIdx.x : (int)blockIdx.x - pa.red.nred;
+}
+__device__ __forceinline__ uint64_t tlog_start(const PatchArgs &pa)
+{
+    return kDiag && diag(pa.dbg, kDiagTimeLog) && pa.tlog ? wall_clock64() : 0;
+}
+__device__ __forceinline__ void tlog_end(const PatchArgs &pa, uint64_t t0, int item, int b0, int b1, int nlev, int a, int n_ent)
+{
+    if (!(kDiag && diag(pa.dbg, kDiagTimeLog) && pa.tlog) || threadIdx.x != 0) return;
+    const uint64_t t1 = wall_clock64();
+    pa.tlog[2 * blockIdx.x] = make_uint4((uint32_t)t0, (uint32_t)(t0 >> 32), (uint32_t)t1, (uint32_t)(t1 >> 32));
+    pa.tlog[2 * blockIdx.x + 1] = make_uint4((uint32_t)item, (uint32_t)(b0 | (b1 << 16)), (uint32_t)(nlev | (a << 8)), (uint32_t)n_ent);
 }
 template <typename T, int NT>
 __device__ __forceinline__ void patch_reduce_role(const PatchArgs &pa)
@@ -173,20 +176,17 @@
     extern __shared__ __attribute__((aligned(16))) double2 ptile[];
     const TileArgs &ta = pa.ta;
     const int tid = threadIdx.x;
+    const uint64_t t_start = tlog_start(pa);
     if (reduce_block_index(pa) >= 0) {
         patch_reduce_role<T, NT>(pa);
+        tlog_end(pa, t_start, -1, 0, 0, 0, 0, 0);
         return;
     }
     const int bid = patch_block_index(pa);
-    const int x = bid & 7, rr = bid >> 3;
-    const int grp = rr % pa.ngrp, sj = rr / pa.ngrp;
-    const int4 rec = pa.wrec[2 * (sj * 8 + x)], rec2 = pa.wrec[2 * (sj * 8 + x) + 1];
+    const int4 rec = pa.wrec[2 * bid], rec2 = pa.wrec[2 * bid + 1];
     if (rec.y <= 0) return;
-    const int sib = grp & ((1 << pa.lgB) - 1);
-    const int nblock = pair_block_count(pa.npair, pa.lgB);
-    int b0, b1;
-    split_blocks(pa, grp >> pa.lgB, nblock, b0, b1);
-    if (b0 >= b1) return;
+    const int sib = (rec2.y >> 17) & 0x7F;
+    const int b0 = rec2.x & 0xFFFF, b1 = (int)((uint32_t)rec2.x >> 16);
     {
         int k0, lw;
         pair_block_of(b0, pa.npair, pa.lgB, k0, lw);
@@ -194,8 +194,8 @@
     }
     const int ent_off = rec.x, n_ent = rec.y, own_lo = rec.z, own_cnt = rec.w;
     const int dbg = kDiag ? pa.dbg : 0;
-    const int nlev = diag(dbg, kDiagNoLevels) ? 0 : rec2.x, a = rec2.y & 0xFFFF;
-    const int d = rec2.y >> 16;
+    const int nlev = diag(dbg, kDiagNoLevels) ? 0 : (int)((uint32_t)rec2.y >> 24), a = rec2.y & 0xFFFF;
+    const int d = (rec2.y >> 16) & 1;
     const int lo = rec2.z, hi = rec2.w;
     const int64_t n = ta.n;
     const int stride = pa.stride;
@@ -329,6 +329,7 @@
             }
         }
     }
+    tlog_end(pa, t_start, bid, b0, b1, nlev, a, n_ent);
 }
 
 
@@ -336,19 +337,17 @@
     int sib, b0, b1;
     int ent_off, n_ent, own_lo, own_cnt, nlev, a, d, lo, hi;
 };
-__device__ __forceinline__ bool patch_item(const PatchArgs &pa, int lgS, PatchItem &it)
+__device__ __forceinline__ bool patch_item(const PatchArgs &pa, PatchItem &it)
 {
     const int bid = patch_block_index(pa);
-    const int x = bid & 7, rr = bid >> 3;
-    const int grp = rr % pa.ngrp, sj = rr / pa.ngrp;
-    const int4 rec = pa.wrec[2 * (sj * 8 + x)], rec2 = pa.wrec[2 * (sj * 8 + x) + 1];
+    const int4 rec = pa.wrec[2 * bid], rec2 = pa.wrec[2 * bid + 1];
     if (rec.y <= 0) return false;
-    it.sib = grp & ((1 << lgS) - 1);
-    split_blocks(pa, grp >> lgS, pair_block_count(pa.npair, pa.lgB), it.b0, it.b1);
-    if (it.b0 >= it.b1) return false;
+    it.b0 = rec2.x & 0xFFFF; it.b1 = (int)((uint32_t)rec2.x >> 16);
     it.ent_off = rec.x; it.n_ent = rec.y; it.own_lo = rec.z; it.own_cnt = rec.w;
-    it.nlev = rec2.x; it.a = rec2.y & 0xFFFF;
-    it.d = rec2.y >> 16;
+    it.a = rec2.y & 0xFFFF;
+    it.d = (rec2.y >> 16) & 1;
+    it.sib = (rec2.y >> 17) & 0x7F;
+    it.nlev = (int)((uint32_t)rec2.y >> 24);
     it.lo = rec2.z;
     it.hi = rec2.w;
     return true;
@@ -737,12 +736,14 @@
 {
     extern __shared__ __attribute__((aligned(16))) double2 ptile[];
     const int tid = threadIdx.x;
+    const uint64_t t_start = tlog_start(pa);
     if (reduce_block_index(pa) >= 0) {
         patch_reduce_role<T, NT>(pa);
+        tlog_end(pa, t_start, -1, 0, 0, 0, 0, 0);
         return;
     }
     PatchItem it;
-    if (!patch_item(pa, pa.lgB, it)) return;
+    if (!patch_item(pa, it)) return;
     if (diag(pa.dbg, kDiagNoPairLoop)) it.b1 = it.b0;
     const EntryTable<NT> tab(ptile, 1);
     tab.park(pa, it, tid);
@@ -750,6 +751,7 @@
     exp2_table_fill();
     __syncthreads();
     lean_pairs<T, AM, NT, 0>(pair_io<AM>(pa, it.d), it, tab, ptile);
+    tlog_end(pa, t_start, patch_block_index(pa), it.b0, it.b1, it.nlev, it.a, it.n_ent);
 }
 
 
@@ -881,12 +883,14 @@
 {
     extern __shared__ __attribute__((aligned(16))) double2 ptile[];
     const int tid = threadIdx.x;
+    const uint64_t t_start = tlog_start(pa);
     if (reduce_block_index(pa) >= 0) {
         patch_reduce_role<float, NT>(pa);
+        tlog_end(pa, t_start, -1, 0, 0, 0, 0, 0);
         return;
     }
     PatchItem it;
-    if (!patch_item(pa, pa.lgB - 1, it)) return;
+    if (!patch_item(pa, it)) return;
     const EntryTable<NT> tab(ptile, 2);
     tab.park(pa, it, tid);
     if (tid == 0) {
@@ -896,6 +900,7 @@
     exp2_table_fill();
     __syncthreads();
     quad_pairs<AM, NT, false>(pair_io<AM>(pa, it.d), it, tab, ptile);
+    tlog_end(pa, t_start, patch_block_index(pa), it.b0, it.b1, it.nlev, it.a, it.n_ent);
 }
 
 
@@ -1189,10 +1194,11 @@
 
 int ensure_patch_work(vrt_plan *p, int G, const std::vector<int32_t> &group_angles, const std::vector<int> &group_off)
 {
-    if (p->d_patch_work && p->patch_work_groups == G) return VRT_OK;
-    if (p->d_patch_work) { (void)hipFree(p->d_patch_work); p->d_patch_work = nullptr; }
+    if (!p->h_patch_work.empty() && p->patch_work_groups == G) return VRT_OK;
+    free_patch_workgroups(p);
     const int maxL = p->tile_max_layers;
-    std::vector<int4> work;
+    std::vector<int4> &work = p->h_patch_work;
+    work.clear();
     p->patch_work_off.assign((size_t)G * (size_t)(maxL + 2) + 1, 0);
     std::vector<std::pair<int64_t, int32_t>> items;
     for (int gi = 0; gi < G; gi++)
@@ -1226,9 +1232,45 @@
             }
         }
     p->patch_work_off.back() = (int64_t)(work.size() / 2);
-    if (int rc = dev_alloc(&p->d_patch_work, work.size())) return rc;
-    VRT_HIP_TRY(hipMemcpy(p->d_patch_work, work.data(), sizeof(int4) * work.size(), hipMemcpyHostToDevice));
     p->patch_work_groups = G;
+    return VRT_OK;
+}
+
+void free_patch_workgroups(vrt_plan *p)
+{
+    for (auto &s : p->patch_wg_sets) dev_free(s.d_rec);
+    p->patch_wg_sets.clear();
+    p->h_patch_work.clear();
+}
+
+static int ensure_patch_workgroups(vrt_plan *p, const PatchSplitRule &rule, const vrt_plan::PatchWgSet **out)
+{
+    for (const auto &s : p->patch_wg_sets)
+        if (s.rule == rule) { *out = &s; return VRT_OK; }
+    if (p->patch_wg_sets.size() >= 16) {
+        VRT_HIP_TRY(hipDeviceSynchronize());
+        dev_free(p->patch_wg_sets.front().d_rec);
+        p->patch_wg_sets.erase(p->patch_wg_sets.begin());
+    }
+    vrt_plan::PatchWgSet set;
+    set.rule = rule;
+    const size_t launches = p->patch_work_off.size() - 1;
+    set.off.assign(launches + 1, 0);
+    std::vector<int4> all;
+    PatchWorkgroups wg;
+    for (size_t l = 0; l < launches; l++) {
+        set.off[l] = (int64_t)(all.size() / 2);
+        const int64_t w0 = p->patch_work_off[l], w1 = p->patch_work_off[l + 1];
+        if (w1 <= w0) continue;
+        if (!build_patch_workgroups(p->h_patch_work.data() + 2 * w0, (w1 - w0) / 8, rule, wg))
+            return fail(VRT_EINVAL, "patch launch does not fit the workgroup record (levels <= 255, pair blocks <= 65535, siblings <= 64)");
+        all.insert(all.end(), wg.rec.begin(), wg.rec.end());
+    }
+    set.off[launches] = (int64_t)(all.size() / 2);
+    if (int rc = dev_alloc(&set.d_rec, std::max<size_t>(all.size(), 1))) return rc;
+    if (!all.empty()) VRT_HIP_TRY(hipMemcpy(set.d_rec, all.data(), sizeof(int4) * all.size(), hipMemcpyHostToDevice));
+    p->patch_wg_sets.push_back(std::move(set));
+    *out = &p->patch_wg_sets.back();
     return VRT_OK;
 }
 
@@ -1255,10 +1297,22 @@
     red.nred = (red.nred + 7) / 8 * 8;
 }
 
+int patch_tlog_begin(vrt_plan *p, hipStream_t st)
+{
+    if (!(kDiag && diag(p->tune.debug_flags, kDiagTimeLog))) return VRT_OK;
+    if (!p->d_patch_tlog) {
+        p->patch_tlog_cap = (int64_t)1 << 20;
+        if (int rc = dev_alloc(&p->d_patch_tlog, 2 * (size_t)p->patch_tlog_cap)) return rc;
+    }
+    p->patch_tlog_used = 0;
+    p->patch_tlog_launch.clear();
+    VRT_HIP_TRY(hipMemsetAsync(p->d_patch_tlog, 0, sizeof(uint4) * 2 * (size_t)p->patch_tlog_cap, st));
+    return VRT_OK;
+}
+
 int launch_patch_layer(vrt_plan *p, const TileArgs &ta, int npair, int layer, int group, int Q, hipStream_t st,
                        bool f32, const PatchReduce *reduce)
 {
-    const int target_wgs = p->tune.patch_target;
     const int maxL = p->tile_max_layers;
     const size_t wo = (size_t)group * (size_t)(maxL + 2) + (size_t)layer;
     const int64_t w0 = (layer >= 2 && layer <= maxL) ? p->patch_work_off[wo] : 0, w1 = (layer >= 2 && layer <= maxL) ? p->patch_work_off[wo + 1] : 0;
@@ -1275,42 +1329,32 @@
     pa.quad = (f32 && pa.lgB >= 1 && p->patch_K == 1 && p->tune.patch_quad != 0 && (npair & 1) == 0) ? 1 : 0;
     if (pa.quad) Q = 1;
     pa.lean = (p->tune.patch_lean != 0 && p->patch_K == 1 && Q == 1 && !pa.quad && npair >= 2) ? 1 : 0;
-    const int lgS = pa.lgB - pa.quad;
     pa.Q = Q;
-    pa.nsplit = 1;
-    pa.ngrp = 1 << lgS;
+    int64_t wgs = 0;
+    pa.wrec = nullptr;
     if (w1 > w0) {
-        const int64_t items = (w1 - w0) << lgS;
-        const int nblock = pair_block_count(npair, pa.lgB);
-        const int steps_all = (nblock + Q - 1) / Q;
-        int nsplit;
-        if (p->tune.patch_split > 0) nsplit = std::min(steps_all, p->tune.patch_split);
-        else if (target_wgs > 0) nsplit = (int)std::max<int64_t>(1, std::min<int64_t>(steps_all, (target_wgs + items - 1) / items));
-        else {
-            const double T = std::min(900.0, 460.0 + 4100.0 / (double)steps_all);
-            const int s_min = (int)std::min<int64_t>(steps_all, std::max<int64_t>(1, (512 + items - 1) / items));
-            double dmin = 1e300;
-            for (int c = steps_all; c >= 1; c--) {
-                const int sc = (steps_all + c - 1) / c;
-                if (sc >= s_min) dmin = std::min(dmin, std::fabs(std::log((double)items * sc / T)));
-            }
-            nsplit = s_min;
-            for (int c = steps_all; c >= 1; c--) {
-                const int sc = (steps_all + c - 1) / c;
-                if (sc >= s_min && std::fabs(std::log((double)items * sc / T)) <= dmin + 0.03) nsplit = sc;
-            }
-        }
-        pa.nsplit = nsplit;
-        pa.ngrp = nsplit << lgS;
+        PatchSplitRule rule;
+        rule.npair = npair; rule.lgB = pa.lgB; rule.quad = pa.quad; rule.Q = Q;
+        rule.cost = p->tune.patch_split_cost; rule.split = p->tune.patch_split; rule.target = p->tune.patch_target;
+        const vrt_plan::PatchWgSet *set = nullptr;
+        if (int rc = ensure_patch_workgroups(p, rule, &set)) return rc;
+        pa.wrec = set->d_rec + 2 * set->off[wo];
+        wgs = set->off[wo + 1] - set->off[wo];
     }
     pa.stride = p->patch_cap + 1;
     pa.cap = p->patch_cap;
     pa.dbg = kDiag ? p->tune.debug_flags : 0;
-    pa.wrec = p->d_patch_work + 2 * w0;
     pa.e_pos = p->e_pos; pa.e_u1 = p->e_u1; pa.e_u2 = p->e_u2;
     pa.e_vis = p->e_vis; pa.e_loc = p->e_loc;
     pa.e_w1 = p->e_w1; pa.e_w2 = p->e_w2; pa.e_r1 = p->e_r1; pa.e_r2 = p->e_r2;
-    const dim3 grid((unsigned)(pa.red.nred + (w1 - w0) * pa.ngrp));
+    const dim3 grid((unsigned)(pa.red.nred + wgs));
+    pa.tlog = nullptr;
+    if (kDiag && diag(pa.dbg, kDiagTimeLog) && p->d_patch_tlog && p->patch_tlog_used + (int64_t)grid.x <= p->patch_tlog_cap) {
+        pa.tlog = p->d_patch_tlog + 2 * p->patch_tlog_used;
+        const int64_t row[5] = {layer, group, p->patch_tlog_used, (int64_t)grid.x, pa.red.nred};
+        p->patch_tlog_launch.insert(p->patch_tlog_launch.end(), row, row + 5);
+        p->patch_tlog_used += grid.x;
+    }
     const size_t lds = (size_t)(pa.quad ? 2 : Q) * (size_t)pa.stride * sizeof(double2) + (size_t)pa.cap * (4 * sizeof(double) + 5 * sizeof(int32_t));
     const int rc = f32 ? launch_mode<float>(ta.alpha_mode, p->patch_K, Q, p->patch_NT, grid, lds, st, pa)
                        : launch_mode<double>(ta.alpha_mode, p->patch_K, Q, p->patch_NT, grid, lds, st, pa);
@@ -1386,13 +1430,10 @@
     const int64_t n = g->n, n_patches = p->n_patches;
     const int nblock = pair_block_count(npair, lgB);
     if ((int64_t)nsplit * n_patches >= ((int64_t)1 << 31)) return fail(VRT_EINVAL, "too many (split, patch) progress words");
-    PatchArgs sp;
-    sp.nsplit = nsplit;
-    sp.Q = 1;
     std::vector<int> steps((size_t)nsplit);
     for (int s = 0; s < nsplit; s++) {
         int b0, b1;
-        split_blocks(sp, s, nblock, b0, b1);
+        split_blocks(1, nsplit, s, nblock, b0, b1);
         steps[(size_t)s] = b1 - b0;
     }
     std::vector<int4> q[8];
```

After: 90.61 billion (median of 6 runs). 3.1% higher.
